# in5omnia/Image_Segmentation

Hardware: AMD Instinct MI355X
Metric: images/sec (fwd+bwd) U-Net 3-class 256x256; IoU parity vs CPU ref (higher is better)
Workload: dtype bf16; 1 GPU; unet(3,3) train step (fwd + ce + bwd + grad all-reduce + AdamW), B=32/GPU 3x256x256, BASELINE config 2; global_batch=32, parallelism=dp1, rccl_ranks=0, rehearsal=False

## Files before the change

image_segmentation_amd/_lib.py:

```python
import ctypes as C
import os

_HERE = os.path.dirname(os.path.abspath(__file__))
LIB_PATH = os.path.join(_HERE, "csrc", "libsegk.so")

F32, BF16 = 0, 1
ABI_VERSION = 318
MAX_CLASSES = 8
MAX_VIEWS = 16
MSE_PART_FLOATS = 1024

_vp, _fp, _i, _l, _f, _d = C.c_void_p, C.c_void_p, C.c_int, C.c_long, C.c_float, C.c_double

SIGNATURES = {
    "segk_version": (_i, []),
    "segk_entry_count": (_i, []),
    "segk_clock_probe": (_i, [_vp, _i, _i, _i, _vp]),
    "segk_debug_poison_tickets": (_i, [C.c_uint64, _vp]),
    "segk_build_id": (C.c_char_p, []),
    "segk_last_error": (C.c_char_p, []),
    "segk_nchw_to_nhwc": (_i, [_fp, _vp, _i, _i, _i, _i, _i, _i, _vp]),
    "segk_nhwc_to_nchw": (_i, [_vp, _fp, _i, _i, _i, _i, _i, _i, _vp]),
    "segk_pack_conv_weight": (_i, [_fp, _vp, _i, _i, _i, _i, _i, _i, _i, _i, _i, _vp]),
    "segk_pack_conv3x3_both": (_i, [_fp, _vp, _vp, _i, _i, _i, _i, _i, _i, _i, _vp]),
    "segk_pack_multi": (_i, [_vp, _i, _i, _i, _vp]),
    "segk_pack_convt_chunk": (_i, []),
    "segk_pack_convt_weight": (_i, [_fp, _vp, _i, _i, _i, _i, _i, _i, _vp]),
    "segk_conv_tiles": (_i, [_i, _i, _i, _i, _i, _i]),
    "segk_bn_stats_floats": (_i, [_i, _i]),
    "segk_conv3x3": (_i, [_vp, _vp, _vp, _fp, _fp, _fp, _vp, _vp, _fp, _i, _i, _i, _i, _i, _i, _i, _i, _vp]),
    "segk_conv_writes_act_q": (_i, [_i, _i, _i]),
    "segk_conv3x3_act": (_i, [_vp, _vp, _fp, _fp, _vp, _vp, _fp, _i, _i, _i, _i, _i, _i, _vp]),
    "segk_stem3x3_rows": (_i, [_i, _i, _i, _i, _i, _i]),
    "segk_stem3x3": (_i, [_fp, _fp, _vp, _vp, _fp, _i, _i, _i, _i, _i, _i, _vp]),
    "segk_stem3x3_wgrad_slabs": (_i, [_i, _i, _i, _i, _i, _i]),
    "segk_stem3x3_wgrad": (_i, [_fp, _vp, _fp, _i, _i, _i, _i, _i, _i, _vp]),
    "segk_conv1x1": (_i, [_vp, _vp, _fp, _vp, _i, _i, _i, _i, _i, _i, _vp]),
    "segk_convt2x2_fwd": (_i, [_vp, _vp, _fp, _vp, _i, _i, _i, _i, _i, _i, _vp]),
    "segk_convt2x2_dgrad": (_i, [_vp, _vp, _vp, _i, _i, _i, _i, _i, _i, _vp]),
    "segk_wgrad_tiles": (_i, [_i, _i, _i, _i, _i]),
    "segk_wgrad_split": (_i, [_i, _i, _i, _i, _i, _i]),
    "segk_wgrad": (_i, [_vp, _vp, _vp, _fp, _fp, _fp, _vp, _i, _i, _i, _i, _i, _i, _i, _i, _i, _vp]),
    "segk_wgrad_reduce": (_i, [_fp, _i, _fp, _i, _i, _i, _i, _i, _i, _i, _vp]),
    "segk_wgrad_reduce_multi": (_i, [_vp, _i, _vp]),
    "segk_bn_finalize": (_i, [_fp, _i, _i, _i, _d, _fp, _fp, _fp, _fp, _fp, _f, _f, _i, _fp, _fp, _fp, _fp, _vp]),
    "segk_bn_relu_apply": (_i, [_vp, _vp, _fp, _fp, _l, _i, _i, _vp]),
    "segk_bn_relu_apply_pool": (_i, [_vp, _vp, _vp, _fp, _fp, _i, _i, _i, _i, _i, _vp]),
    "segk_bn_bwd_blocks": (_i, [_l, _i, _i]),
    "segk_bn_relu_bwd": (_i, [_vp, _vp, _vp, _fp, _fp, _fp, _fp, _l, _i, _i, _fp, _fp, _fp, _fp, _i, _vp]),
    "segk_channel_sum": (_i, [_vp, _l, _i, _i, _fp, _fp, _i, _vp]),
    "segk_maxpool2x2_fwd": (_i, [_vp, _vp, _i, _i, _i, _i, _i, _vp]),
    "segk_maxpool2x2_bwd": (_i, [_vp, _vp, _vp, _i, _i, _i, _i, _i, _i, _vp]),
    "segk_maxpool_bwd_stat_blocks": (_i, [_i, _i, _i, _i, _i]),
    "segk_maxpool2x2_bwd_bnstat": (_i, [_vp, _vp, _vp, _i, _i, _i, _i, _i, _fp, _fp, _fp, _fp, _fp, _vp, _i, _vp]),
    "segk_bn_relu_bwd_from_part": (_i, [_vp, _vp, _vp, _fp, _fp, _fp, _fp, _l, _i, _i, _fp, _i, _fp, _fp, _fp, _i, _vp]),
    "segk_bilinear_fwd": (_i, [_vp, _vp, _i, _i, _i, _i, _i, _i, _i, _vp]),
    "segk_bilinear_bwd": (_i, [_vp, _vp, _fp, _i, _i, _i, _i, _i, _i, _i, _vp]),
    "segk_linear": (_i, [_vp, _vp, _fp, _vp, _l, _i, _i, _i, _i, _vp]),
    "segk_vit_patchify": (_i, [_fp, _vp, _i, _i, _i, _i, _i, _i, _i, _vp]),
    "segk_vit_embed_ln": (_i, [_vp, _fp, _fp, _fp, _fp, _f, _fp, _i, _i, _i, _i, _i, _vp]),
    "segk_add_layernorm": (_i, [_fp, _vp, _fp, _fp, _f, _vp, _l, _i, _i, _i, _vp]),
    "segk_linear_splitk": (_i, [_vp, _vp, _fp, _vp, _l, _i, _i, _i, _i, _vp]),
    "segk_add_layernorm_parts": (_i, [_fp, _vp, _i, _l, _fp, _fp, _f, _vp, _l, _i, _i, _i, _vp]),
    "segk_attention": (_i, [_vp, _vp, _i, _i, _i, _i, _i, _i, _f, _i, _vp]),
    "segk_vit_tokens_to_grid": (_i, [_fp, _vp, _i, _i, _i, _i, _i, _vp]),
    "segk_resize_pad": (_i, [_vp, _vp, _i, _i, _i, _i, _i, _i, _i, _i, _i, _i, _vp]),
    "segk_crop_resize": (_i, [_fp, _fp, _i, _i, _i, _i, _i, _i, _i, _i, _i, _vp]),
    "segk_resize_pad_u8": (_i, [_vp, _fp, _i, _i, _i, _i, _i, _i, _i, _i, _i, _vp]),
    "segk_predict_mask": (_i, [_vp, _vp, _vp, _vp, _vp, _vp, _vp, _i, _i, _i, _i, _i, _i, _i, _i, _i, _vp]),
    "segk_resize_pad_flip": (_i, [_vp, _vp, _i, _i, _i, _i, _i, _i, _i, _i, _i, _i, _i, _vp]),
    "segk_resize_pad_u8_flip": (_i, [_vp, _fp, _i, _i, _i, _i, _i, _i, _i, _i, _i, _i, _vp]),
    "segk_predict_merge": (_i, [_vp, _i, _i, _i, _i, _i, _i, _vp, _vp, _vp, _vp, _vp, _vp, _vp, _fp, _vp]),
    "segk_tile_gather_u8": (_i, [_vp, _fp, _i, _i, _i, _i, _i, _i, _i, _i, _vp]),
    "segk_tile_gather": (_i, [_fp, _fp, _i, _i, _i, _i, _i, _i, _i, _i, _vp]),
    "segk_predict_tiles": (_i, [_fp, _i, _i, _i, _i, _i, _i, _i, _i, _vp, _vp, _vp, _vp, _vp, _vp, _vp, _fp, _vp]),
    "segk_cc_label": (_i, [_vp, _vp, _vp, _vp, _vp, _vp, _vp, _vp, _i, _i, _i, _i, _i, _vp]),
    "segk_cc_clean": (_i, [_vp, _vp, _vp, _vp, _vp, _i, _i, _i, _i, _i, _vp]),
    "segk_mask_finish": (_i, [_vp, _vp, _vp, _vp, _vp, _vp, _i, _i, _i, _vp]),
    "segk_head_fwd": (_i, [_vp, _fp, _fp, _fp, _i, _i, _i, _i, _i, _i, _i, _vp]),
    "segk_head_fwd_bn": (_i, [_vp, _fp, _fp, _fp, _fp, _fp, _i, _i, _i, _i, _i, _i, _i, _vp]),
    "segk_head_bwd_bn": (_i, [_fp, _vp, _fp, _vp, _fp, _fp, _fp, _i, _i, _i, _i, _i, _i, _fp, _fp, _fp, _fp, _fp, _i, _vp]),
    "segk_head_part_floats": (_i, [_l, _i]),
    "segk_head_bwd": (_i, [_fp, _vp, _fp, _vp, _fp, _fp, _fp, _i, _i, _i, _i, _i, _i, _i, _vp]),
    "segk_head_bwd_blocks": (_i, [_l]),
    "segk_head_bwd_bnstat": (_i, [_fp, _vp, _fp, _vp, _fp, _fp, _fp, _i, _i, _i, _i, _i, _i, _fp, _fp, _fp, _fp, _fp, _i, _vp]),
    "segk_loss_part_floats": (_i, [_l]),
    "segk_loss_state_floats": (_i, []),
    "segk_loss_fwd": (_i, [_fp, _vp, _fp, _i, _i, _l, _i, _f, _f, _f, _fp, _fp, _fp, _vp]),
    "segk_loss_bwd": (_i, [_fp, _vp, _fp, _fp, _fp, _i, _i, _l, _i, _f, _f, _fp, _vp]),
    "segk_prompt_mix_fwd": (_i, [_fp, _fp, _fp, _i, _l, _vp]),
    "segk_prompt_mix_bwd": (_i, [_fp, _fp, _fp, _fp, _i, _l, _vp]),
    "segk_prob_loss_fwd": (_i, [_fp, _vp, _fp, _i, _i, _l, _i, _f, _f, _f, _i, _f, _fp, _fp, _fp, _vp]),
    "segk_prob_loss_bwd": (_i, [_fp, _vp, _fp, _fp, _fp, _i, _i, _l, _i, _f, _f, _i, _f, _fp, _vp]),
    "segk_confusion": (_i, [_fp, _vp, _i, _i, _l, _vp, _vp]),
    "segk_recon_head_fwd": (_i, [_vp, _fp, _fp, _fp, _i, _i, _i, _i, _i, _i, _i, _vp]),
    "segk_recon_sigmoid_bwd": (_i, [_fp, _fp, _vp, _i, _i, _i, _i, _i, _i, _vp]),
    "segk_mse_fwd": (_i, [_fp, _fp, _fp, _i, _fp, _l, _i, _vp]),
    "segk_mse_bwd": (_i, [_fp, _fp, _fp, _fp, _fp, _l, _i, _vp]),
    "segk_prompt_scores": (_i, [_vp, _vp, _vp, _vp, _i, _i, _vp, _vp, _i, _i, _i, _i, _vp]),
    "segk_prompt_make": (_i, [_vp, _vp, _vp, _vp, _vp, _i, _fp, _vp, _vp, _vp, _vp, _i, _i, _i, _i, _i, _vp]),
    "segk_prompt_heatmap": (_i, [_vp, _i, _vp, _i, _fp, _i, _i, _vp]),
    "segk_aug_prefilter": (_i, [_vp, _i, _i, _vp]),
    "segk_aug_resample": (_i, [_vp, _i, _i, _vp, _vp, _i, _vp, _i, _vp, _i, _vp, _fp, _vp, _vp, _vp]),
    "segk_aug_merge": (_i, [_vp, _vp, _i, _i, _vp, _fp, _vp, _vp, _vp]),
    "segk_label_hist": (_i, [_vp, _l, _i, _i, _i, _l, _vp, _vp]),
    "segk_rgb_label_to_classes": (_i, [_vp, _vp, _l, _vp]),
    "segk_perturb_point": (_i, [_vp, _i, _i, _i, _vp, _vp]),
    "segk_perturb_blur": (_i, [_vp, _i, _i, _i, _vp]),
}



class ReduceJob(C.Structure):
    _fields_ = [("src", C.c_void_p), ("dst", C.c_void_p), ("kind", C.c_int), ("S", C.c_int), ("N", C.c_int), ("CA", C.c_int),
                ("CB", C.c_int), ("Np", C.c_int), ("CAp", C.c_int), ("CBp", C.c_int), ("taps", C.c_int), ("pad_", C.c_int)]


_lib = None


def load():
    global _lib, LIB_PATH
    if _lib is None:
        if os.environ.get("SEGK_LIB"):
            LIB_PATH = os.path.abspath(os.environ["SEGK_LIB"])
        if not os.path.exists(LIB_PATH):
            raise RuntimeError(
                f"{LIB_PATH} not found: the HIP extension is required (no CPU/eager fallback exists). "
                "Build it with `python -m image_segmentation_amd.build`.")
        lib = C.CDLL(LIB_PATH)
        for name, (res, args) in SIGNATURES.items():
            try:
                fn = getattr(lib, name)
            except AttributeError:
                raise RuntimeError(f"{LIB_PATH} does not export {name}: it was built from another include/segk.h than "
                                   "this binding (rebuild with `python -m image_segmentation_amd.build`)") from None
            fn.restype = res
            fn.argtypes = args
        ver, nent = lib.segk_version(), lib.segk_entry_count()
        if ver != ABI_VERSION or nent != len(SIGNATURES):
            raise RuntimeError(f"{LIB_PATH}: ABI version {ver} with {nent} entries, this binding expects version "
                               f"{ABI_VERSION} with {len(SIGNATURES)} entries -- refusing to drive a library built from "
                               "another include/segk.h")
        _lib = lib
    return _lib


def call(name, *args):
    lib = load()
    rc = getattr(lib, name)(*args)
    if rc != 0:
        raise RuntimeError(f"{name} failed ({rc}): {lib.segk_last_error().decode()}")


def build_id():
    return load().segk_build_id().decode()


def query(name, *args):
    return getattr(load(), name)(*args)
```

image_segmentation_amd/build.py:

```python
import os
import subprocess
import sys
from concurrent.futures import ThreadPoolExecutor

CSRC = os.path.join(os.path.dirname(os.path.abspath(__file__)), "csrc")
SOURCES = ["api.hip", "conv_igemm.hip", "conv_rs.hip", "convt_stream.hip", "stem.hip", "wgrad.hip", "bn_pool.hip", "pack.hip", "head_loss.hip", "recon.hip", "prompt.hip", "augment.hip", "perturb.hip", "components.hip", "resize.hip", "tiles.hip", "vit.hip", "gemm.hip", "probe.hip"]
LIB = os.path.join(CSRC, "libsegk.so")
FLAGS = ["--offload-arch=gfx950", "-O3", "-fPIC", "-std=c++17", "-ffp-contract=off", "-Wall", "-Wno-unused-function"]


def _hipcc():
    for c in (os.environ.get("HIPCC"), "/opt/rocm/bin/hipcc", "hipcc"):
        if c and (os.path.isabs(c) and os.path.exists(c) or not os.path.isabs(c)):
            return c
    raise RuntimeError("hipcc not found")


def source_hash() -> str:
    import hashlib
    h = hashlib.sha256()
    files = sorted(f for f in os.listdir(CSRC) if f.endswith((".hip", ".hpp", ".h")))
    paths = [os.path.join(CSRC, f) for f in files] + \
            [os.path.join(os.path.dirname(os.path.dirname(CSRC)), "include", "segk.h")]
    for path in paths:
        h.update(os.path.basename(path).encode() + b"\0")
        h.update(open(path, "rb").read())
    return h.hexdigest()[:16]


def _stale(obj, src):
    if not os.path.exists(obj):
        return True
    t = os.path.getmtime(obj)
    deps = [src] + [os.path.join(CSRC, h) for h in ("common.hpp", "segk_internal.h")] + \
           [os.path.join(os.path.dirname(os.path.dirname(CSRC)), "include", "segk.h")]
    return any(os.path.getmtime(d) > t for d in deps)


def build(force: bool = False, verbose: bool = True) -> str:
    hipcc = _hipcc()
    objs, jobs = [], []
    bid = source_hash()
    stamp = os.path.join(CSRC, ".build_id")
    id_changed = not os.path.exists(stamp) or open(stamp).read().strip() != bid
    for s in SOURCES:
        src = os.path.join(CSRC, s)
        obj = os.path.join(CSRC, s.replace(".hip", ".o"))
        objs.append(obj)
        extra = [f'-DSEGK_BUILD_ID="{bid}"'] if s == "api.hip" else []
        if force or _stale(obj, src) or (extra and id_changed):
            jobs.append([hipcc, *FLAGS, *extra, "-c", src, "-o", obj])

    def run(cmd):
        if verbose:
            print(" ".join(cmd), flush=True)
        r = subprocess.run(cmd, capture_output=True, text=True)
        if r.returncode != 0:
            raise RuntimeError(f"hipcc failed: {' '.join(cmd)}\n{r.stdout}\n{r.stderr}")
        if verbose and r.stderr.strip():
            print(r.stderr, file=sys.stderr)

    with ThreadPoolExecutor(max_workers=6) as ex:
        list(ex.map(run, jobs))
    if jobs or not os.path.exists(LIB):
        run([hipcc, "--offload-arch=gfx950", "-shared", "-fPIC", "-o", LIB, *objs])
    with open(stamp, "w") as f:
        f.write(bid + "\n")
    return LIB


def build_sanitized(verbose: bool = False) -> str:
    hipcc = _hipcc()
    out = os.path.join(CSRC, ".asan")
    os.makedirs(out, exist_ok=True)
    lib = os.path.join(out, "libsegk_asan.so")
    stamp = os.path.join(out, ".build_id")
    bid = source_hash()
    if os.path.exists(lib) and os.path.exists(stamp) and open(stamp).read().strip() == bid:
        return lib
    flags = ["--offload-arch=gfx950", "-O1", "-g", "-fPIC", "-std=c++17", "-ffp-contract=off", "-fno-omit-frame-pointer",
             "-fsanitize=address,undefined", "-fno-sanitize-recover=undefined", "-fno-gpu-sanitize"]
    objs, jobs = [], []
    for s in SOURCES:
        obj = os.path.join(out, s.replace(".hip", ".o"))
        objs.append(obj)
        extra = [f'-DSEGK_BUILD_ID="{bid}"'] if s == "api.hip" else []
        jobs.append([hipcc, *flags, *extra, "-c", os.path.join(CSRC, s), "-o", obj])

    def run(cmd):
        if verbose:
            print(" ".join(cmd), flush=True)
        r = subprocess.run(cmd, capture_output=True, text=True)
        if r.returncode != 0:
            raise RuntimeError(f"hipcc failed: {' '.join(cmd)}\n{r.stdout}\n{r.stderr}")
    with ThreadPoolExecutor(max_workers=6) as ex:
        list(ex.map(run, jobs))
    run([hipcc, "--offload-arch=gfx950", "-shared", "-fPIC", "-fsanitize=address,undefined", "-shared-libsan", "-o", lib, *objs])
    with open(stamp, "w") as f:
        f.write(bid + "\n")
    return lib


def asan_runtime() -> str:
    import glob
    hits = sorted(glob.glob("/opt/rocm/lib/llvm/lib/clang/*/lib/linux/libclang_rt.asan-x86_64.so"))
    if not hits:
        raise RuntimeError("libclang_rt.asan-x86_64.so not found under /opt/rocm/lib/llvm")
    return hits[-1]


if __name__ == "__main__":
    print(build(force="--force" in sys.argv))
```

image_segmentation_amd/csrc/bn_pool.hip:

```cpp
#include <atomic>
#include "common.hpp"
#include "segk_internal.h"
#include "ticket.hpp"
#include "../../include/segk.h"

namespace {
__device__ unsigned g_tickets[TICKET_SLOTS * TICKET_GROUPS];

struct Lanes {
  int cx, ry, cv;
  bool active;
};
__device__ __forceinline__ Lanes lanes(int cvb, int cvec) {
  Lanes l;
  l.cx = threadIdx.x % cvb;
  l.ry = threadIdx.x / cvb;
  l.cv = blockIdx.y * cvb + l.cx;
  l.active = l.cv < cvec;
  return l;
}

constexpr int NCH = 32;
__device__ __forceinline__ void stats_chunk(const float* __restrict__ part, int MT, int C, double* __restrict__ out,
                                            double (&sh)[8][32][2]) {
// ... 459 lines not shown
        o[j] = accumulate ? o[j] + r : r;
        if (STAT) {
          const float gg = v[k][j] > 0.f ? o[j] : 0.f;
          sg[j] += gg;
          sgx[j] = fmaf(gg, fmaf(v[k][j], xa[j], xb[j]), sgx[j]);
        }
      }
      *(uint4*)(dx + off[k]) = pack16<T>(o);
    }
  }
  if (STAT) {
    __shared__ float red[256][2 * E::VEC + 1];
    if (from_z) {
#pragma unroll
      for (int j = 0; j < E::VEC; ++j) sgx[j] = 0.f;
      for (unsigned i = blockIdx.x * 256u + threadIdx.x; i < (unsigned)total; i += gridDim.x * 256u) {
        const Idx4 ix = split4(i, (unsigned)CV, (unsigned)Wc, (unsigned)Hc);
        const int cv = ix.cv, xo = ix.x, yo = ix.y, b = ix.b;
        for (int k = 0; k < 4; ++k) {
          const int yy = 2 * yo + (k >> 1), xx = 2 * xo + (k & 1);
          if (yy >= H || xx >= W) continue;
          const size_t off = (((size_t)(b * H + yy)) * W + xx) * C + cv * E::VEC;
          float fy[E::VEC], fd[E::VEC], fz[E::VEC];
          unpack16<T>(*(const uint4*)(x + off), fy);
          unpack16<T>(*(const uint4*)(dx + off), fd);
          unpack16<T>(*(const uint4*)(z + off), fz);
#pragma unroll
          for (int j = 0; j < E::VEC; ++j) {
            const int c = cv * E::VEC + j;
            const float gg = fy[j] > 0.f ? fd[j] : 0.f;
            sgx[j] = fmaf(gg, (fz[j] - mean[c]) * rstd[c], sgx[j]);
          }
        }
      }
    }
#pragma unroll
    for (int j = 0; j < E::VEC; ++j) { red[threadIdx.x][j] = sg[j]; red[threadIdx.x][E::VEC + j] = sgx[j]; }
    __syncthreads();
    for (int q = threadIdx.x; q < CV * E::VEC; q += 256) {
      const int cv = q / E::VEC, j = q - cv * E::VEC;
      float a = 0.f, bsum = 0.f;
      for (int t = cv; t < 256; t += CV) {
        a += red[t][j];
        bsum += red[t][E::VEC + j];
      }
      ((float2*)part)[(size_t)blockIdx.x * C + q] = make_float2(a, bsum);
    }
  }
}

template <typename T>
__global__ __launch_bounds__(256) void channel_sum_kernel(const T* __restrict__ x, long P, int C, int cvb, int rows,
                                                          float* part) {
  using E = ET<T>;
  extern __shared__ __attribute__((aligned(16))) char smem[];
  float* red = (float*)smem;
  const Lanes l = lanes(cvb, C / E::VEC);
  float s[E::VEC];
#pragma unroll
  for (int j = 0; j < E::VEC; ++j) s[j] = 0.f;
  if (l.active && l.ry < rows) {
    auto one = [&](const uint4 raw) {
      float f[E::VEC];
      unpack16<T>(raw, f);
#pragma unroll
      for (int j = 0; j < E::VEC; ++j) s[j] += f[j];
    };
    const long step = (long)gridDim.x * rows;
    const size_t cofs = (size_t)l.cv * E::VEC;
    long p = (long)blockIdx.x * rows + l.ry;
    for (; p + 3 * step < P; p += 4 * step) {
      uint4 r[4];
#pragma unroll
      for (int u = 0; u < 4; ++u) r[u] = *(const uint4*)(x + (size_t)(p + u * step) * C + cofs);
      __builtin_amdgcn_sched_barrier(0);
#pragma unroll
      for (int u = 0; u < 4; ++u) one(r[u]);
    }
    for (; p < P; p += step) one(*(const uint4*)(x + (size_t)p * C + cofs));
  }
  if (l.ry < rows) {
    float* r = red + ((size_t)l.ry * cvb + l.cx) * E::VEC;
#pragma unroll
    for (int j = 0; j < E::VEC; ++j) r[j] = s[j];
  }
  __syncthreads();
  if (l.ry == 0 && l.active)
#pragma unroll
    for (int j = 0; j < E::VEC; ++j) {
      float a = 0.f;
      for (int r = 0; r < rows; ++r) a += red[((size_t)r * cvb + l.cx) * E::VEC + j];
      part[(size_t)blockIdx.x * C + l.cv * E::VEC + j] = a;
    }
}
__global__ __launch_bounds__(1024) void channel_sum_finalize_kernel(const float* __restrict__ part, int NB, int C,
                                                                    int C_real, float* out) {
  __shared__ double sh[32][32];
  const int cx = threadIdx.x & 31, ry = threadIdx.x >> 5;
  const int c = blockIdx.x * 32 + cx;
  double s = 0.0;
  if (c < C) {
    for (int m = ry; m < NB; m += 512) {
      float v[16];
#pragma unroll
      for (int u = 0; u < 16; ++u) {
        const int r = m + 32 * u < NB ? m + 32 * u : NB - 1;
        v[u] = part[(unsigned)r * (unsigned)C + (unsigned)c];
      }
#pragma unroll
      for (int u = 0; u < 16; ++u) s += (m + 32 * u < NB) ? (double)v[u] : 0.0;
    }
  }
  sh[ry][cx] = s;
  __syncthreads();
  if (ry != 0 || c >= C_real) return;
  s = 0.0;
#pragma unroll 8
  for (int r = 0; r < 32; ++r) s += sh[r][cx];
  out[c] = (float)s;
}

static inline void lane_geometry(int C, int vec, int* cvb, int* rows, int* gy) {
  const int cvec = C / vec;
  *cvb = cvec < 128 ? cvec : 128;
  *rows = 256 / *cvb;
  *gy = cdiv(cvec, *cvb);
}

}

unsigned* segk_ticket_slot(int groups, hipStream_t st) {
  static std::atomic<unsigned> n{0};
  static unsigned* base[SEGK_MAX_DEVICES] = {};
  const int dev = segk_device_index();
  if (groups < 1 || groups > TICKET_GROUPS) return nullptr;
  if (!base[dev] && hipGetSymbolAddress((void**)&base[dev], HIP_SYMBOL(g_tickets)) != hipSuccess) return nullptr;
  unsigned* const p = base[dev] + (size_t)(n.fetch_add(1, std::memory_order_relaxed) % TICKET_SLOTS) * TICKET_GROUPS;
  if (hipMemsetAsync(p, 0, (size_t)groups * sizeof(unsigned), st) != hipSuccess) return nullptr;
  return p;
}

extern "C" int segk_debug_poison_tickets(uint64_t pattern, segk_stream_t s) {
  hipStream_t st = (hipStream_t)s;
  unsigned* base = nullptr;
  SEGK_REQUIRE(hipGetSymbolAddress((void**)&base, HIP_SYMBOL(g_tickets)) == hipSuccess, "poison_tickets: no ticket array");
  static unsigned host[TICKET_SLOTS * TICKET_GROUPS];
  for (int i = 0; i < TICKET_SLOTS * TICKET_GROUPS; ++i) host[i] = (unsigned)pattern;
  SEGK_REQUIRE(hipMemcpyAsync(base, host, sizeof(host), hipMemcpyHostToDevice, st) == hipSuccess, "poison_tickets: copy failed");
  SEGK_REQUIRE(hipStreamSynchronize(st) == hipSuccess, "poison_tickets: sync failed");
  return 0;
}

extern "C" int segk_bn_finalize(const float* part, int MT, int C, int C_real, double count, const float* conv_bias,
                                const float* gamma, const float* beta, float* rmean, float* rvar, float momentum, float eps,
                                int training, float* scale, float* shift, float* mean, float* rstd, segk_stream_t s) {
  hipStream_t st = (hipStream_t)s;
  SEGK_REQUIRE(C > 0 && C % 32 == 0 && C_real > 0 && C_real <= C, "bn_finalize: bad channels C=%d real=%d", C, C_real);
  SEGK_REQUIRE(gamma && beta && scale && shift, "bn_finalize: null pointer");
  if (training) SEGK_REQUIRE(part && MT > 0 && count > 0 && mean && rstd, "bn_finalize: training needs partials");
  else SEGK_REQUIRE(rmean && rvar, "bn_finalize: eval needs running statistics");
  double* scratch = part ? (double*)(const_cast<float*>(part) + (size_t)MT * C * 2) : nullptr;
  if (training && MT <= 1024) {
    hipLaunchKernelGGL(bn_stats_finalize_small_kernel, dim3(C / 32), dim3(1024), 0, st, part, MT, C, C_real, count, conv_bias,
                       gamma, beta, rmean, rvar, momentum, eps, scale, shift, mean, rstd);
    SEGK_CHECK_LAUNCH("bn_stats_finalize_small");
    return 0;
  }
  if (training) {
    SEGK_REQUIRE(C / 32 <= TICKET_GROUPS, "bn_finalize: at most %d channels", 32 * TICKET_GROUPS);
    unsigned* const tickets = segk_ticket_slot(C / 32, st);
    SEGK_REQUIRE(tickets != nullptr, "bn_finalize: no ticket array");
    hipLaunchKernelGGL(bn_stats_finalize_kernel, dim3(C / 32, NCH), dim3(256), 0, st, part, MT, C, C_real, count, conv_bias,
                       gamma, beta, rmean, rvar, momentum, eps, scale, shift, mean, rstd, scratch, tickets);
    SEGK_CHECK_LAUNCH("bn_stats_finalize");
    return 0;
  }
  hipLaunchKernelGGL(bn_finalize_kernel, dim3(C / 32), dim3(256), 0, st, scratch, NCH, C, C_real, count, conv_bias,
                     gamma, beta, rmean, rvar, momentum, eps, training, scale, shift, mean, rstd);
  SEGK_CHECK_LAUNCH("bn_finalize");
  return 0;
}
int segk_bn_stats_floats(int tiles, int Cp) {
  if (tiles <= 0 || Cp <= 0) return 0;
  const long long n = (long long)tiles * Cp * 2 + (long long)NCH * Cp * 4;
  return n > 0x7fffffffLL ? 0 : (int)n;
}

template <typename T>
static int bn_relu_apply_t(const void* z, void* y, const float* scale, const float* shift, long P, int C, hipStream_t st) {
  int cvb, rows, gy;
  lane_geometry(C, ET<T>::VEC, &cvb, &rows, &gy);
  long gx = (P + rows - 1) / rows;
  if (gx > 4096) gx = 4096;
  hipLaunchKernelGGL(bn_relu_apply_kernel<T>, dim3((int)gx, gy), dim3(256), 0, st, (const T*)z, (T*)y, scale, shift, P,
                     C, cvb, rows);
  SEGK_CHECK_LAUNCH("bn_relu_apply");
  return 0;
}
extern "C" int segk_bn_relu_apply(const void* z, void* y, const float* scale, const float* shift, long P, int C, int dtype,
                                  segk_stream_t s) {
  SEGK_REQUIRE_DTYPE("bn_relu_apply", dtype);
  hipStream_t st = (hipStream_t)s;
  SEGK_REQUIRE(z && y && scale && shift && P > 0 && C > 0 && C % 32 == 0, "bn_relu_apply: bad arguments");
  return dtype == SEGK_DT_BF16 ? bn_relu_apply_t<bf16_t>(z, y, scale, shift, P, C, st)
                               : bn_relu_apply_t<float>(z, y, scale, shift, P, C, st);
}

extern "C" int segk_bn_relu_apply_pool(const void* z, void* y, void* pooled, const float* scale, const float* shift, int B,
                                       int H, int W, int C, int dtype, segk_stream_t s) {
  SEGK_REQUIRE_DTYPE("bn_relu_apply_pool", dtype);
  hipStream_t st = (hipStream_t)s;
  SEGK_REQUIRE(z && y && pooled && scale && shift && B > 0 && H >= 2 && W >= 2 && C > 0 && C % 32 == 0,
               "bn_relu_apply_pool: bad arguments");
  const int vec = dtype == SEGK_DT_BF16 ? 8 : 4;
  long total = (long)B * ((H + 1) / 2) * ((W + 1) / 2) * (C / vec);
  SEGK_REQUIRE(total < (1L << 31), "bn_relu_apply_pool: more than 2^31 windows x channel vectors");
  long g = (total + 255) / 256;
  if (g > 8192) g = 8192;
  if (dtype == SEGK_DT_BF16)
    hipLaunchKernelGGL(bn_relu_apply_pool_kernel<bf16_t>, dim3((int)g), dim3(256), 0, st, (const bf16_t*)z, (bf16_t*)y,
                       (bf16_t*)pooled, scale, shift, B, H, W, C);
  else
    hipLaunchKernelGGL(bn_relu_apply_pool_kernel<float>, dim3((int)g), dim3(256), 0, st, (const float*)z, (float*)y,
                       (float*)pooled, scale, shift, B, H, W, C);
  SEGK_CHECK_LAUNCH("bn_relu_apply_pool");
  return 0;
}

int segk_bn_bwd_blocks(long P, int C, int dtype) {
  if (P <= 0 || C <= 0 || C % 32 != 0) return 0;
  const int vec = dtype == SEGK_DT_BF16 ? 8 : 4;
  int cvb, rows, gy;
  lane_geometry(C, vec, &cvb, &rows, &gy);
  long gx = (P + rows - 1) / rows;
  if (gx > 512) gx = 512;
  return (int)gx;
}

template <typename T>
static int bn_bwd_t(const void* dy, const void* z, void* dz, const float* scale, const float* shift, const float* mean,
                    const float* rstd, long P, int C, int C_real, float* part, float* dgamma, float* dbeta,
                    float* coef, hipStream_t st) {
  using E = ET<T>;
  int cvb, rows, gy;
  lane_geometry(C, E::VEC, &cvb, &rows, &gy);
  const int gx = segk_bn_bwd_blocks(P, C, sizeof(T) == 2 ? SEGK_DT_BF16 : SEGK_DT_F32);
  const size_t lds = (size_t)rows * cvb * 2 * E::VEC * sizeof(float);
  hipLaunchKernelGGL(bn_bwd_reduce_kernel<T>, dim3(gx, gy), dim3(256), lds, st, (const T*)dy, (const T*)z, scale, shift,
                     mean, rstd, P, C, cvb, rows, part);
  SEGK_CHECK_LAUNCH("bn_bwd_reduce");
  hipLaunchKernelGGL(bn_bwd_finalize_kernel, dim3(C / 32), dim3(1024), 0, st, part, gx, C, C_real, (double)P, dgamma,
                     dbeta, coef);
  SEGK_CHECK_LAUNCH("bn_bwd_finalize");
  long ga = (P + rows - 1) / rows;
  if (ga > 4096) ga = 4096;
  hipLaunchKernelGGL(bn_bwd_apply_kernel<T>, dim3((int)ga, gy), dim3(256), 0, st, (const T*)dy, (const T*)z, (T*)dz,
                     scale, shift, mean, rstd, coef, P, C, cvb, rows);
  SEGK_CHECK_LAUNCH("bn_bwd_apply");
  return 0;
}
template <typename T>
static int bn_bwd_from_part_t(const void* dy, const void* z, void* dz, const float* scale, const float* shift, const float* mean,
                              const float* rstd, long P, int C, int C_real, const float* part, int nb, float* dgamma,
                              float* dbeta, float* coef, hipStream_t st) {
  using E = ET<T>;
  int cvb, rows, gy;
  lane_geometry(C, E::VEC, &cvb, &rows, &gy);
  hipLaunchKernelGGL(bn_bwd_finalize_kernel, dim3(C / 32), dim3(1024), 0, st, part, nb, C, C_real, (double)P, dgamma,
                     dbeta, coef);
  SEGK_CHECK_LAUNCH("bn_bwd_finalize");
  long ga = (P + rows - 1) / rows;
  if (ga > 4096) ga = 4096;
  hipLaunchKernelGGL(bn_bwd_apply_kernel<T>, dim3((int)ga, gy), dim3(256), 0, st, (const T*)dy, (const T*)z, (T*)dz,
                     scale, shift, mean, rstd, coef, P, C, cvb, rows);
  SEGK_CHECK_LAUNCH("bn_bwd_apply");
  return 0;
}
extern "C" int segk_bn_relu_bwd_from_part(const void* dy, const void* z, void* dz, const float* scale, const float* shift,
                                          const float* mean, const float* rstd, long P, int C, int C_real, const float* part,
                                          int nb, float* dgamma, float* dbeta, float* coef, int dtype, segk_stream_t s) {
  SEGK_REQUIRE_DTYPE("bn_relu_bwd_from_part", dtype);
  hipStream_t st = (hipStream_t)s;
  SEGK_REQUIRE(dy && z && dz && scale && shift && mean && rstd && part && dgamma && dbeta && coef && nb > 0,
               "bn_bwd_from_part: bad arguments");
  SEGK_REQUIRE(P > 0 && C > 0 && C % 32 == 0 && C_real > 0 && C_real <= C, "bn_bwd_from_part: bad shape");
  return dtype == SEGK_DT_BF16
             ? bn_bwd_from_part_t<bf16_t>(dy, z, dz, scale, shift, mean, rstd, P, C, C_real, part, nb, dgamma, dbeta, coef, st)
             : bn_bwd_from_part_t<float>(dy, z, dz, scale, shift, mean, rstd, P, C, C_real, part, nb, dgamma, dbeta, coef, st);
}

extern "C" int segk_bn_relu_bwd(const void* dy, const void* z, void* dz, const float* scale, const float* shift,
                                const float* mean, const float* rstd, long P, int C, int C_real, float* part, float* dgamma,
                                float* dbeta, float* coef, int dtype, segk_stream_t s) {
  SEGK_REQUIRE_DTYPE("bn_relu_bwd", dtype);
  hipStream_t st = (hipStream_t)s;
  SEGK_REQUIRE(dy && z && dz && scale && shift && mean && rstd && part && dgamma && dbeta && coef,
               "bn_bwd: null pointer");
  SEGK_REQUIRE(P > 0 && C > 0 && C % 32 == 0 && C_real > 0 && C_real <= C, "bn_bwd: bad shape");
  return dtype == SEGK_DT_BF16
             ? bn_bwd_t<bf16_t>(dy, z, dz, scale, shift, mean, rstd, P, C, C_real, part, dgamma, dbeta, coef, st)
             : bn_bwd_t<float>(dy, z, dz, scale, shift, mean, rstd, P, C, C_real, part, dgamma, dbeta, coef, st);
}

extern "C" int segk_maxpool2x2_fwd(const void* x, void* y, int B, int H, int W, int C, int dtype, segk_stream_t s) {
  SEGK_REQUIRE_DTYPE("maxpool2x2_fwd", dtype);
  hipStream_t st = (hipStream_t)s;
  SEGK_REQUIRE(x && y && B > 0 && H >= 2 && W >= 2 && C > 0 && C % 32 == 0, "maxpool_fwd: bad arguments");
  const int vec = dtype == SEGK_DT_BF16 ? 8 : 4;
  long total = (long)B * (H / 2) * (W / 2) * (C / vec);
  SEGK_REQUIRE(total < (1L << 31), "maxpool_fwd: more than 2^31 windows x channel vectors");
  long g = (total + 255) / 256;
  if (g > 8192) g = 8192;
  if (dtype == SEGK_DT_BF16)
    hipLaunchKernelGGL(maxpool_fwd_kernel<bf16_t>, dim3((int)g), dim3(256), 0, st, (const bf16_t*)x, (bf16_t*)y, B, H, W, C);
  else
    hipLaunchKernelGGL(maxpool_fwd_kernel<float>, dim3((int)g), dim3(256), 0, st, (const float*)x, (float*)y, B, H, W, C);
  SEGK_CHECK_LAUNCH("maxpool_fwd");
  return 0;
}

extern "C" int segk_maxpool2x2_bwd(const void* x, const void* dy, void* dx, int B, int H, int W, int C, int accumulate,
                                   int dtype, segk_stream_t s) {
  SEGK_REQUIRE_DTYPE("maxpool2x2_bwd", dtype);
  hipStream_t st = (hipStream_t)s;
  SEGK_REQUIRE(x && dy && dx && B > 0 && H >= 2 && W >= 2 && C > 0 && C % 32 == 0, "maxpool_bwd: bad arguments");
  const int vec = dtype == SEGK_DT_BF16 ? 8 : 4;
  long total = (long)B * ((H + 1) / 2) * ((W + 1) / 2) * (C / vec);
  SEGK_REQUIRE(total < (1L << 31), "maxpool_bwd: more than 2^31 windows x channel vectors");
  long g = (total + 255) / 256;
  if (g > 8192) g = 8192;
  if (dtype == SEGK_DT_BF16)
    hipLaunchKernelGGL((maxpool_bwd_kernel<bf16_t, false>), dim3((int)g), dim3(256), 0, st, (const bf16_t*)x, (const bf16_t*)dy,
                       (bf16_t*)dx, B, H, W, C, accumulate, nullptr, nullptr, nullptr, nullptr, nullptr, nullptr);
  else
    hipLaunchKernelGGL((maxpool_bwd_kernel<float, false>), dim3((int)g), dim3(256), 0, st, (const float*)x, (const float*)dy,
                       (float*)dx, B, H, W, C, accumulate, nullptr, nullptr, nullptr, nullptr, nullptr, nullptr);
  SEGK_CHECK_LAUNCH("maxpool_bwd");
  return 0;
}

int segk_maxpool_bwd_stat_blocks(int B, int H, int W, int C, int dtype) {
  const int vec = dtype == SEGK_DT_BF16 ? 8 : 4;
  if (B <= 0 || H < 2 || W < 2 || C <= 0 || C % 32 != 0) return 0;
  const int cv = C / vec;
  if ((cv & (cv - 1)) != 0 || cv > 256) return 0;
  long total = (long)B * ((H + 1) / 2) * ((W + 1) / 2) * cv;
  if (total >= (1L << 31)) return 0;
  long g = (total + 255) / 256;
  return (int)(g > 1024 ? 1024 : g);
}

extern "C" int segk_maxpool2x2_bwd_bnstat(const void* x, const void* dy, void* dx, int B, int H, int W, int C, int accumulate,
                                          const float* scale, const float* shift, const float* mean, const float* rstd,
                                          float* part, const void* z, int dtype, segk_stream_t s) {
  SEGK_REQUIRE_DTYPE("maxpool2x2_bwd_bnstat", dtype);
  hipStream_t st = (hipStream_t)s;
  SEGK_REQUIRE(x && dy && dx && scale && shift && mean && rstd && part, "maxpool_bwd_bnstat: null pointer");
  const int g = segk_maxpool_bwd_stat_blocks(B, H, W, C, dtype);
  SEGK_REQUIRE(g > 0, "maxpool_bwd_bnstat: shape not served (channel vectors must be a power of two)");
  if (dtype == SEGK_DT_BF16)
    hipLaunchKernelGGL((maxpool_bwd_kernel<bf16_t, true>), dim3(g), dim3(256), 0, st, (const bf16_t*)x, (const bf16_t*)dy,
                       (bf16_t*)dx, B, H, W, C, accumulate, scale, shift, mean, rstd, part, (const bf16_t*)z);
  else
    hipLaunchKernelGGL((maxpool_bwd_kernel<float, true>), dim3(g), dim3(256), 0, st, (const float*)x, (const float*)dy,
                       (float*)dx, B, H, W, C, accumulate, scale, shift, mean, rstd, part, (const float*)z);
  SEGK_CHECK_LAUNCH("maxpool_bwd_bnstat");
  return 0;
}

extern "C" int segk_channel_sum(const void* x, long P, int C, int C_real, float* part, float* out, int dtype, segk_stream_t s) {
  SEGK_REQUIRE_DTYPE("channel_sum", dtype);
  hipStream_t st = (hipStream_t)s;
  SEGK_REQUIRE(x && part && out && P > 0 && C > 0 && C % 32 == 0 && C_real > 0 && C_real <= C, "channel_sum: bad arguments");
  const int vec = dtype == SEGK_DT_BF16 ? 8 : 4;
  int cvb, rows, gy;
  lane_geometry(C, vec, &cvb, &rows, &gy);
  const int gx = segk_bn_bwd_blocks(P, C, dtype);
  const size_t lds = (size_t)rows * cvb * vec * sizeof(float);
  if (dtype == SEGK_DT_BF16)
    hipLaunchKernelGGL(channel_sum_kernel<bf16_t>, dim3(gx, gy), dim3(256), lds, st, (const bf16_t*)x, P, C, cvb, rows, part);
  else
    hipLaunchKernelGGL(channel_sum_kernel<float>, dim3(gx, gy), dim3(256), lds, st, (const float*)x, P, C, cvb, rows, part);
  SEGK_CHECK_LAUNCH("channel_sum");
  hipLaunchKernelGGL(channel_sum_finalize_kernel, dim3(C / 32), dim3(1024), 0, st, part, gx, C, C_real, out);
  SEGK_CHECK_LAUNCH("channel_sum_finalize");
  return 0;
}
```

image_segmentation_amd/csrc/head_loss.hip:

```cpp
#include <type_traits>
#include "common.hpp"
#include "segk_internal.h"
#include "ticket.hpp"
#include "../../include/segk.h"

namespace {
constexpr int MAXC = 8;
constexpr int HT = 256;
constexpr int HCH = 64;

__device__ __forceinline__ void split_hw(long p, long HW, long& b, long& r) {
  const unsigned bb = (unsigned)p / (unsigned)HW;
  b = (long)bb;
  r = p - (long)bb * HW;
}

template <typename T, int NC>
__global__ __launch_bounds__(256) void head_fwd_kernel(const T* __restrict__ y, const float* __restrict__ w,
                                                       const float* __restrict__ bias, float* __restrict__ logits,
                                                       long P, long HW, int Cp, int C, int ncls,
                                                       const float* __restrict__ zsc, const float* __restrict__ zsh) {
  using E = ET<T>;
  constexpr int PITCH = HCH * E::ES + 16;
  extern __shared__ __attribute__((aligned(16))) char tile[];
// ... 303 lines not shown
      v[u] = part[(unsigned)r * LP + cx];
    }
#pragma unroll
    for (int u = 0; u < FL; ++u) acc += (ry + RG * u < NB) ? (double)v[u] : 0.0;
  }
  sh[ry][cx] = acc;
  __syncthreads();
  if (t < LP) {
    double s = 0.0;
    for (int r = 0; r < RG; ++r) s += sh[r][t];
    tot[t] = s;
  }
  __syncthreads();
  if (t != 0) return;
  const double ce = tot[1] > 0.0 ? tot[0] / tot[1] : NAN;
  double wsum = 0.0, dsum = 0.0;
  int nvalid = 0;
  for (int k = 0; k < C; ++k) {
    const double den_raw = tot[2 + MAXC + k] + tot[2 + 2 * MAXC + k] + (double)smooth;
    const double den = den_raw < 1e-8 ? 1e-8 : den_raw;
    const double dc = (2.0 * tot[2 + k] + (double)smooth) / den;
    state[4 + k] = (float)dc;
    state[4 + MAXC + k] = (float)den_raw;
    const bool valid = !(ignore_index >= 0 && ignore_index < C && k == ignore_index);
    if (valid) {
      const double wk = cw ? (double)cw[k] : 1.0;
      wsum += wk; dsum += dc * wk; ++nvalid;
    }
  }
  if (cw && wsum < 1e-8) wsum = 1e-8;
  const double dice = -(dsum / wsum);
  for (int k = 0; k < C; ++k) {
    const bool valid = !(ignore_index >= 0 && ignore_index < C && k == ignore_index);
    state[4 + 2 * MAXC + k] = valid ? (float)((cw ? (double)cw[k] : 1.0) / wsum) : 0.f;
  }
  state[0] = (float)((double)dice_weight * dice + (ce_weight != 0.f ? (double)ce_weight * ce : 0.0));
  if (loss_out) *loss_out = state[0];
  state[1] = (float)ce;
  state[2] = (float)dice;
  state[3] = (float)tot[1];
  (void)nvalid;
}

template <bool PROB, int NC>
__global__ __launch_bounds__(LT) void loss_fwd_kernel(const float* __restrict__ logits,
                                                       const long long* __restrict__ labels,
                                                       const float* __restrict__ cw, long P, long HW, int C,
                                                       int ignore_index, float* __restrict__ part, int nll_log, float eps,
                                                       float smooth, float dice_weight, float ce_weight,
                                                       float* __restrict__ state, float* __restrict__ loss_out,
                                                       unsigned* __restrict__ ticket) {
  __shared__ float sh[LT / 64][LP];
  __shared__ int last;
  float a0 = 0.f, a1 = 0.f, aI[NC], aP[NC], aG[NC];
#pragma unroll
  for (int k = 0; k < NC; ++k) { aI[k] = 0.f; aP[k] = 0.f; aG[k] = 0.f; }
  auto fetch = [&](long p, float (&raw)[NC], long long& y) {
    long b, r; split_hw(p, HW, b, r);
#pragma unroll
    for (int k = 0; k < NC; ++k) {
      const float v = logits[(b * C + (k < C ? k : C - 1)) * HW + r];
      raw[k] = (k < C) ? v : -INFINITY;
    }
    y = labels[p];
  };
  auto pixel = [&](const float (&raw)[NC], const long long y) {
    float l[NC], m = -INFINITY;
#pragma unroll
    for (int k = 0; k < NC; ++k) m = fmaxf(m, raw[k]);
    float se = 0.f;
#pragma unroll
    for (int k = 0; k < NC; ++k) {
      if constexpr (PROB) l[k] = (k < C) ? raw[k] : 0.f;
      else l[k] = (k < C) ? expf(raw[k] - m) : 0.f;
      se += l[k];
    }
    const float inv = PROB ? 1.f : 1.f / se, lse = PROB ? 0.f : logf(se);
#pragma unroll
    for (int k = 0; k < NC; ++k) {
      const float pk = l[k] * inv;
      const float oh = (y == k) ? 1.f : 0.f;
      aI[k] += pk * oh;
      aP[k] += pk;
      aG[k] += oh;
      if (y == k && k < C && y != ignore_index) {
        const float wy = cw ? cw[k] : 1.f;
        if constexpr (PROB) a0 += wy * (nll_log ? -logf(raw[k] + eps) : -raw[k]);
        else a0 += wy * (lse - (raw[k] - m));
        a1 += wy;
      }
    }
  };
  const long step = (long)gridDim.x * LT;
  long p = (long)blockIdx.x * LT + threadIdx.x;
  for (; p + 3 * step < P; p += 4 * step) {
    float r0[NC], r1[NC], r2[NC], r3[NC];
    long long y0, y1, y2, y3;
    fetch(p, r0, y0);
    fetch(p + step, r1, y1);
    fetch(p + 2 * step, r2, y2);
    fetch(p + 3 * step, r3, y3);
    pixel(r0, y0);
    pixel(r1, y1);
    pixel(r2, y2);
    pixel(r3, y3);
  }
  for (; p < P; p += step) {
    float r0[NC];
    long long y0;
    fetch(p, r0, y0);
    pixel(r0, y0);
  }
  float v[LP];
#pragma unroll
  for (int i = 0; i < LP; ++i) v[i] = 0.f;
  v[0] = a0; v[1] = a1;
#pragma unroll
  for (int k = 0; k < NC; ++k) { v[2 + k] = aI[k]; v[2 + MAXC + k] = aP[k]; v[2 + 2 * MAXC + k] = aG[k]; }
#pragma unroll
  for (int i = 0; i < LP; ++i) {
    if (i >= 2 && ((i - 2) % MAXC) >= NC) continue;
#pragma unroll
    for (int o = 32; o > 0; o >>= 1) v[i] += __shfl_xor(v[i], o);
  }
  if ((threadIdx.x & 63) == 0) {
#pragma unroll
    for (int i = 0; i < LP; ++i) sh[threadIdx.x >> 6][i] = v[i];
  }
  __syncthreads();
  if (threadIdx.x < LP) {
    const int i = threadIdx.x;
    float s2 = 0.f;
#pragma unroll
    for (int w = 0; w < LT / 64; ++w) s2 += sh[w][i];
    part[(size_t)blockIdx.x * LP + i] = s2;
  }
  if (last_arriver(ticket, gridDim.x, &last))
    loss_finalize_block(part, (int)gridDim.x, C, cw, ignore_index, smooth, dice_weight, ce_weight, state, loss_out);
}


template <bool PROB, int NC>
__global__ __launch_bounds__(256) void loss_bwd_kernel(const float* __restrict__ logits,
                                                       const long long* __restrict__ labels,
                                                       const float* __restrict__ cw, const float* __restrict__ state,
                                                       const float* __restrict__ gout, long P, long HW, int C,
                                                       int ignore_index, float dice_weight, float ce_weight,
                                                       float* __restrict__ dlogits, int nll_log, float eps) {
  const float go = gout[0];
  const float ce_den = state[3];
  float G0[NC], G1[NC];
#pragma unroll
  for (int k = 0; k < NC; ++k) {
    G0[k] = 0.f; G1[k] = 0.f;
    if (k < C) {
      const float dc = state[4 + k], den_raw = state[4 + MAXC + k], ak = state[4 + 2 * MAXC + k];
      if (den_raw < 1e-8f) { G1[k] = -ak * 2.f / 1e-8f; }
      else { G0[k] = ak * dc / den_raw; G1[k] = -ak * 2.f / den_raw; }
    }
  }
  for (long p = (long)blockIdx.x * 256 + threadIdx.x; p < P; p += (long)gridDim.x * 256) {
    long b, r; split_hw(p, HW, b, r);
    float l[NC], m = -INFINITY;
#pragma unroll
    for (int k = 0; k < NC; ++k) {
      const float v = logits[(b * C + (k < C ? k : C - 1)) * HW + r];
      l[k] = (k < C) ? v : -INFINITY;
      m = fmaxf(m, l[k]);
    }
    const long long y = labels[p];
    const bool ce_valid = (ce_weight != 0.f && y >= 0 && y < C && y != ignore_index);
    float wy = 0.f;
    if (ce_valid) wy = (cw ? cw[y] : 1.f) / ce_den;
    if constexpr (PROB) {
#pragma unroll
      for (int k = 0; k < NC; ++k)
        if (k < C) {
          const bool hit = (y == k);
          const float dd = G0[k] + (hit ? G1[k] : 0.f);
          const float dn = hit ? (nll_log ? -wy / (l[k] + eps) : -wy) : 0.f;
          dlogits[(b * C + k) * HW + r] = go * (dice_weight * dd + ce_weight * dn);
        }
      continue;
    }
    float se = 0.f;
#pragma unroll
    for (int k = 0; k < NC; ++k) { l[k] = (k < C) ? expf(l[k] - m) : 0.f; se += l[k]; }
    const float inv = 1.f / se;
    float dot = 0.f;
#pragma unroll
    for (int k = 0; k < NC; ++k) {
      l[k] *= inv;
      dot += l[k] * (G0[k] + ((y == k) ? G1[k] : 0.f));
    }
#pragma unroll
    for (int k = 0; k < NC; ++k)
      if (k < C) {
        const float gk = G0[k] + ((y == k) ? G1[k] : 0.f);
        const float dd = l[k] * (gk - dot);
        const float dce = wy * (l[k] - ((y == k) ? 1.f : 0.f));
        dlogits[(b * C + k) * HW + r] = go * (dice_weight * dd + ce_weight * dce);
      }
  }
}

__global__ __launch_bounds__(256) void confusion_kernel(const float* __restrict__ logits,
                                                        const long long* __restrict__ labels, long P, long HW, int C,
                                                        unsigned long long* __restrict__ M) {
  __shared__ unsigned int hist[MAXC * MAXC];
  if (threadIdx.x < MAXC * MAXC) hist[threadIdx.x] = 0;
  __syncthreads();
  for (long p = (long)blockIdx.x * 256 + threadIdx.x; p < P; p += (long)gridDim.x * 256) {
    long b, r; split_hw(p, HW, b, r);
    int best = 0;
    float bv = logits[(b * C) * HW + r];
    for (int k = 1; k < C; ++k) {
      const float v = logits[(b * C + k) * HW + r];
      if (v > bv || (v != v && bv == bv)) { bv = v; best = k; }
    }
    const long long y = labels[p];
    if (y >= 0 && y < C) atomicAdd(&hist[best * MAXC + (int)y], 1u);
  }
  __syncthreads();
  if (threadIdx.x < MAXC * MAXC && hist[threadIdx.x])
    atomicAdd(&M[threadIdx.x], (unsigned long long)hist[threadIdx.x]);
}

}

template <typename T> static size_t head_lds() { return (size_t)HT * (HCH * ET<T>::ES + 16); }

#ifndef SEGK_HEAD_BLOCKS_CAP
#define SEGK_HEAD_BLOCKS_CAP 1024
#endif
int segk_head_blocks(long P) {
  if (P <= 0) return 0;
  long g = (P + 31) / 32;
  return (int)(g > SEGK_HEAD_BLOCKS_CAP ? SEGK_HEAD_BLOCKS_CAP : g);
}
int segk_head_part_floats(long P, int Cp) {
  if (P <= 0 || Cp <= 0) return 0;
  const long long n = (long long)segk_head_blocks(P) * MAXC * ((long long)Cp + 1);
  return n > 0x7fffffffLL ? 0 : (int)n;
}

static int head_fwd(const void* y, const float* w, const float* bias, float* logits, int B, int H, int W, int Cp, int C, int ncls,
                    const float* zsc, const float* zsh, int dtype, hipStream_t st) {
  SEGK_REQUIRE(y && w && bias && logits && B > 0 && H > 0 && W > 0, "head_fwd: bad arguments");
  SEGK_REQUIRE((zsc == nullptr) == (zsh == nullptr), "head_fwd: scale and shift come together");
  SEGK_REQUIRE_DTYPE("head_fwd", dtype);
  SEGK_REQUIRE(ncls >= 1 && ncls <= MAXC, "head_fwd: 1..%d classes supported, got %d", MAXC, ncls);
  SEGK_REQUIRE(Cp % 32 == 0 && C > 0 && C <= Cp, "head_fwd: bad channels");
  const long P = (long)B * H * W, HW = (long)H * W;
  SEGK_REQUIRE(P < (1L << 31), "head / loss kernels index pixels with 32 bits: %ld pixels", P);
  long g = (P + HT - 1) / HT;
  if (g > 4096) g = 4096;
  auto launch = [&](auto Tc, auto NCc) {
    using T = decltype(Tc);
    constexpr int NC = decltype(NCc)::value;
    return segk_launch_lds<head_fwd_kernel<T, NC>>("head_fwd", 96 * 1024, dim3((int)g), dim3(256), head_lds<T>(), st, (const T*)y, w,
                                                   bias, logits, P, HW, Cp, C, ncls, zsc, zsh);
  };
  auto by_nc = [&](auto Tc) {
    if (ncls <= 2) return launch(Tc, std::integral_constant<int, 2>{});
    if (ncls == 3) return launch(Tc, std::integral_constant<int, 3>{});
    if (ncls == 4) return launch(Tc, std::integral_constant<int, 4>{});
    return launch(Tc, std::integral_constant<int, MAXC>{});
  };
  return dtype == SEGK_DT_BF16 ? by_nc(bf16_t{}) : by_nc(float{});
}
extern "C" int segk_head_fwd(const void* y, const float* w, const float* bias, float* logits, int B, int H, int W, int Cp, int C,
                             int ncls, int dtype, segk_stream_t s) {
  SEGK_REQUIRE_DTYPE("head_fwd", dtype);
  return head_fwd(y, w, bias, logits, B, H, W, Cp, C, ncls, nullptr, nullptr, dtype, (hipStream_t)s);
}
extern "C" int segk_head_fwd_bn(const void* z, const float* scale, const float* shift, const float* w, const float* bias,
                                float* logits, int B, int H, int W, int Cp, int C, int ncls, int dtype, segk_stream_t s) {
  SEGK_REQUIRE(scale && shift, "head_fwd_bn: null scale/shift");
  return head_fwd(z, w, bias, logits, B, H, W, Cp, C, ncls, scale, shift, dtype, (hipStream_t)s);
}

template <typename T>
static int head_bwd_t(const float* dlog, const void* y, const float* w, void* dy, float* part, float* dw, float* db,
                      long P, long HW, int Cp, int C, int ncls, const float* const* bn, float* bnpart, bool zin,
                      hipStream_t st) {
  constexpr int HV = HeadVec<T>::HV;
  const int cvec = Cp / HV;
  const int cvb = cvec < 64 ? cvec : 64;
  const int rows = 256 / cvb, gy = cdiv(cvec, cvb);
  const int nb = segk_head_blocks(P);
  const size_t lds = (size_t)rows * cvb * (MAXC * HV + MAXC) * sizeof(float);
  auto launch_z = [&](auto NCc, auto ZINc) {
    constexpr int NC = decltype(NCc)::value;
    return segk_launch_lds<head_bwd_kernel<T, NC, decltype(ZINc)::value>>(
        "head_bwd", 96 * 1024, dim3(nb, gy), dim3(256), lds, st, dlog, (const T*)y, w, (T*)dy, part, P, HW, Cp, C, ncls, cvb, rows,
        bn ? bn[0] : nullptr, bn ? bn[1] : nullptr, bn ? bn[2] : nullptr, bn ? bn[3] : nullptr, bnpart);
  };
  auto launch = [&](auto NCc) { return zin ? launch_z(NCc, std::true_type{}) : launch_z(NCc, std::false_type{}); };
  const int rc = ncls <= 2 ? launch(std::integral_constant<int, 2>{})
               : ncls == 3 ? launch(std::integral_constant<int, 3>{})
               : ncls == 4 ? launch(std::integral_constant<int, 4>{})
                           : launch(std::integral_constant<int, MAXC>{});
  if (rc) return rc;
  hipLaunchKernelGGL(head_bwd_finalize_kernel, dim3(cdiv(ncls * (C + 1), 4)), dim3(256), 0, st, part, nb, Cp, C, ncls, dw, db);
  SEGK_CHECK_LAUNCH("head_bwd_finalize");
  return 0;
}

static int head_bwd(const float* dlog, const void* y, const float* w, void* dy, float* part, float* dw, float* db, int B, int H,
                    int W, int Cp, int C, int ncls, const float* bn_scale, const float* bn_shift, const float* bn_mean,
                    const float* bn_rstd, float* bnpart, int zin, int dtype, hipStream_t st) {
  SEGK_REQUIRE(dlog && y && w && dy && part && dw && db && B > 0 && H > 0 && W > 0, "head_bwd: bad arguments");
  SEGK_REQUIRE(ncls >= 1 && ncls <= MAXC && Cp % 32 == 0 && C > 0 && C <= Cp, "head_bwd: bad channels/classes");
  SEGK_REQUIRE_DTYPE("head_bwd", dtype);
  SEGK_REQUIRE(!(bnpart || zin) || (bn_scale && bn_shift && bn_mean && bn_rstd),
               "head_bwd: BatchNorm reductions / a pre-activation input need scale, shift, mean and rstd");
  const long P = (long)B * H * W, HW = (long)H * W;
  SEGK_REQUIRE(P < (1L << 31), "head / loss kernels index pixels with 32 bits: %ld pixels", P);
  const float* bn[4] = {bn_scale, bn_shift, bn_mean, bn_rstd};
  const float* const* bnp = (bnpart || zin) ? bn : nullptr;
  return dtype == SEGK_DT_BF16 ? head_bwd_t<bf16_t>(dlog, y, w, dy, part, dw, db, P, HW, Cp, C, ncls, bnp, bnpart, zin != 0, st)
                               : head_bwd_t<float>(dlog, y, w, dy, part, dw, db, P, HW, Cp, C, ncls, bnp, bnpart, zin != 0, st);
}
extern "C" int segk_head_bwd(const float* dlogits, const void* y, const float* w, void* dy, float* part, float* dw, float* db,
                             int B, int H, int W, int Cp, int C, int ncls, int dtype, segk_stream_t s) {
  SEGK_REQUIRE_DTYPE("head_bwd", dtype);
  return head_bwd(dlogits, y, w, dy, part, dw, db, B, H, W, Cp, C, ncls, nullptr, nullptr, nullptr, nullptr, nullptr, 0, dtype,
                  (hipStream_t)s);
}
extern "C" int segk_head_bwd_blocks(long P) { return segk_head_blocks(P); }
extern "C" int segk_head_bwd_bnstat(const float* dlogits, const void* y, const float* w, void* dy, float* part, float* dw,
                                    float* db, int B, int H, int W, int Cp, int C, int ncls, const float* scale,
                                    const float* shift, const float* mean, const float* rstd, float* bnpart, int dtype,
                                    segk_stream_t s) {
  SEGK_REQUIRE_DTYPE("head_bwd_bnstat", dtype);
  SEGK_REQUIRE(bnpart, "head_bwd_bnstat: null partials");
  return head_bwd(dlogits, y, w, dy, part, dw, db, B, H, W, Cp, C, ncls, scale, shift, mean, rstd, bnpart, 0, dtype,
                  (hipStream_t)s);
}
extern "C" int segk_head_bwd_bn(const float* dlogits, const void* z, const float* w, void* dy, float* part, float* dw, float* db,
                                int B, int H, int W, int Cp, int C, int ncls, const float* scale, const float* shift,
                                const float* mean, const float* rstd, float* bnpart, int dtype, segk_stream_t s) {
  SEGK_REQUIRE(scale && shift && mean && rstd, "head_bwd_bn: null BatchNorm vectors");
  return head_bwd(dlogits, z, w, dy, part, dw, db, B, H, W, Cp, C, ncls, scale, shift, mean, rstd, bnpart, 1, dtype,
                  (hipStream_t)s);
}

__global__ __launch_bounds__(256) void prompt_mix_fwd_kernel(const float* __restrict__ clip, const float* __restrict__ mask,
                                                             float* __restrict__ out, long P, long HW) {
  for (long p = (long)blockIdx.x * 256 + threadIdx.x; p < P; p += (long)gridDim.x * 256) {
    long b, r; split_hw(p, HW, b, r);
    float l[4], mx = -INFINITY;
#pragma unroll
    for (int k = 0; k < 4; ++k) { l[k] = clip[(b * 4 + k) * HW + r]; mx = fmaxf(mx, l[k]); }
    float se = 0.f;
#pragma unroll
    for (int k = 0; k < 4; ++k) { l[k] = expf(l[k] - mx); se += l[k]; }
    const float inv = 1.f / se;
    const float m = 1.f / (1.f + expf(-mask[p]));
    float sel[4];
#pragma unroll
    for (int k = 0; k < 4; ++k) sel[k] = m * (l[k] * inv);
    out[(b * 4 + 0) * HW + r] = 1.0f - m;
    out[(b * 4 + 1) * HW + r] = sel[0] + sel[3];
    out[(b * 4 + 2) * HW + r] = sel[1];
    out[(b * 4 + 3) * HW + r] = sel[2];
  }
}
__global__ __launch_bounds__(256) void prompt_mix_bwd_kernel(const float* __restrict__ clip, const float* __restrict__ mask,
                                                             const float* __restrict__ dout, float* __restrict__ dmask,
                                                             long P, long HW) {
  for (long p = (long)blockIdx.x * 256 + threadIdx.x; p < P; p += (long)gridDim.x * 256) {
    long b, r; split_hw(p, HW, b, r);
    float l[4], mx = -INFINITY;
#pragma unroll
    for (int k = 0; k < 4; ++k) { l[k] = clip[(b * 4 + k) * HW + r]; mx = fmaxf(mx, l[k]); }
    float se = 0.f;
#pragma unroll
    for (int k = 0; k < 4; ++k) { l[k] = expf(l[k] - mx); se += l[k]; }
    const float inv = 1.f / se;
    const float m = 1.f / (1.f + expf(-mask[p]));
    const float d0 = dout[(b * 4 + 0) * HW + r], d1 = dout[(b * 4 + 1) * HW + r];
    const float d2 = dout[(b * 4 + 2) * HW + r], d3 = dout[(b * 4 + 3) * HW + r];
    const float dm = -d0 + d1 * ((l[0] + l[3]) * inv) + d2 * (l[1] * inv) + d3 * (l[2] * inv);
    dmask[p] = dm * m * (1.f - m);
  }
}

static int prompt_mix(const float* clip, const float* mask, const float* dout, float* out, int N, long HW, hipStream_t st) {
  SEGK_REQUIRE(clip && mask && out && N > 0 && HW > 0, "prompt_mix: bad arguments");
  const long P = (long)N * HW;
  SEGK_REQUIRE(P < (1L << 31), "head / loss kernels index pixels with 32 bits: %ld pixels", P);
  long g = (P + 255) / 256;
  if (g > 4096) g = 4096;
  if (dout) hipLaunchKernelGGL(prompt_mix_bwd_kernel, dim3((int)g), dim3(256), 0, st, clip, mask, dout, out, P, HW);
  else hipLaunchKernelGGL(prompt_mix_fwd_kernel, dim3((int)g), dim3(256), 0, st, clip, mask, out, P, HW);
  SEGK_CHECK_LAUNCH("prompt_mix");
  return 0;
}
extern "C" int segk_prompt_mix_fwd(const float* clip_logits, const float* mask_logit, float* final_probs, int N, long HW,
                                   segk_stream_t s) {
  return prompt_mix(clip_logits, mask_logit, nullptr, final_probs, N, HW, (hipStream_t)s);
}
extern "C" int segk_prompt_mix_bwd(const float* clip_logits, const float* mask_logit, const float* dfinal, float* dmask_logit,
                                   int N, long HW, segk_stream_t s) {
  SEGK_REQUIRE(dfinal, "prompt_mix_bwd: null gradient");
  return prompt_mix(clip_logits, mask_logit, dfinal, dmask_logit, N, HW, (hipStream_t)s);
}

int segk_loss_blocks(long P) {
  if (P <= 0) return 0;
  long g = (P + 4 * LT - 1) / (4 * LT);
  return (int)(g > LROWS ? LROWS : g < 1 ? 1 : g);
}
int segk_loss_part_floats(long P) { return segk_loss_blocks(P) * LP; }
int segk_loss_state_floats(void) { return LS; }

static int loss_fwd(const float* logits, const int64_t* labels64, const float* cw, int N, int C, long HW, int ignore_index,
                    float smooth, float dice_weight, float ce_weight, float* part, float* state, float* loss_out, int prob,
                    int nll_log, float eps, segk_stream_t s) {
  const long long* labels = (const long long*)labels64;
  hipStream_t st = (hipStream_t)s;
  SEGK_REQUIRE(logits && labels && part && state && N > 0 && HW > 0, "loss_fwd: bad arguments");
  SEGK_REQUIRE(C >= 1 && C <= MAXC, "loss_fwd: 1..%d classes supported, got %d", MAXC, C);
  const long P = (long)N * HW;
  SEGK_REQUIRE(P < (1L << 31), "head / loss kernels index pixels with 32 bits: %ld pixels", P);
  const int nb = segk_loss_blocks(P);
  unsigned* const ticket = segk_ticket_slot(1, st);
  SEGK_REQUIRE(ticket != nullptr, "loss_fwd: no ticket array");
  auto launch = [&](auto PROBc, auto NCc) {
    constexpr bool PR = decltype(PROBc)::value;
    constexpr int NC = decltype(NCc)::value;
    hipLaunchKernelGGL((loss_fwd_kernel<PR, NC>), dim3(nb), dim3(LT), 0, st, logits, labels, cw, P, HW, C, ignore_index, part,
                       PR ? nll_log : 0, PR ? eps : 0.f, smooth, dice_weight, ce_weight, state, loss_out, ticket);
  };
  auto by_nc = [&](auto PROBc) {
    if (C <= 2) launch(PROBc, std::integral_constant<int, 2>{});
    else if (C <= 4) launch(PROBc, std::integral_constant<int, 4>{});
    else launch(PROBc, std::integral_constant<int, MAXC>{});
  };
  if (prob) by_nc(std::true_type{});
  else by_nc(std::false_type{});
  SEGK_CHECK_LAUNCH("loss_fwd");
  return 0;
}
extern "C" int segk_loss_fwd(const float* logits, const int64_t* labels, const float* cw, int N, int C, long HW, int ignore_index,
                             float smooth, float dice_weight, float ce_weight, float* part, float* state, float* loss_out,
                             segk_stream_t s) {
  return loss_fwd(logits, labels, cw, N, C, HW, ignore_index, smooth, dice_weight, ce_weight, part, state, loss_out, 0, 0, 0.f, s);
}
extern "C" int segk_prob_loss_fwd(const float* probs, const int64_t* labels, const float* cw, int N, int C, long HW,
                                  int ignore_index, float smooth, float dice_weight, float nll_weight, int nll_log, float eps,
                                  float* part, float* state, float* loss_out, segk_stream_t s) {
  return loss_fwd(probs, labels, cw, N, C, HW, ignore_index, smooth, dice_weight, nll_weight, part, state, loss_out, 1, nll_log,
                  eps, s);
}

static int loss_bwd(const float* logits, const int64_t* labels64, const float* cw, const float* state, const float* gout, int N,
                    int C, long HW, int ignore_index, float dice_weight, float ce_weight, float* dlogits, int prob, int nll_log,
                    float eps, segk_stream_t s) {
  const long long* labels = (const long long*)labels64;
  hipStream_t st = (hipStream_t)s;
  SEGK_REQUIRE(logits && labels && state && gout && dlogits && N > 0 && HW > 0 && C >= 1 && C <= MAXC, "loss_bwd: bad arguments");
  const long P = (long)N * HW;
  SEGK_REQUIRE(P < (1L << 31), "head / loss kernels index pixels with 32 bits: %ld pixels", P);
  long g = (P + 255) / 256;
  if (g > 4096) g = 4096;
  auto launch = [&](auto PROBc, auto NCc) {
    constexpr bool PR = decltype(PROBc)::value;
    constexpr int NC = decltype(NCc)::value;
    hipLaunchKernelGGL((loss_bwd_kernel<PR, NC>), dim3((int)g), dim3(256), 0, st, logits, labels, cw, state, gout, P, HW, C,
                       ignore_index, dice_weight, ce_weight, dlogits, PR ? nll_log : 0, PR ? eps : 0.f);
  };
  auto by_nc = [&](auto PROBc) {
    if (C <= 2) launch(PROBc, std::integral_constant<int, 2>{});
    else if (C <= 4) launch(PROBc, std::integral_constant<int, 4>{});
    else launch(PROBc, std::integral_constant<int, MAXC>{});
  };
  if (prob) by_nc(std::true_type{});
  else by_nc(std::false_type{});
  SEGK_CHECK_LAUNCH("loss_bwd");
  return 0;
}
extern "C" int segk_loss_bwd(const float* logits, const int64_t* labels, const float* cw, const float* state, const float* gout,
                             int N, int C, long HW, int ignore_index, float dice_weight, float ce_weight, float* dlogits,
                             segk_stream_t s) {
  return loss_bwd(logits, labels, cw, state, gout, N, C, HW, ignore_index, dice_weight, ce_weight, dlogits, 0, 0, 0.f, s);
}
extern "C" int segk_prob_loss_bwd(const float* probs, const int64_t* labels, const float* cw, const float* state,
                                  const float* gout, int N, int C, long HW, int ignore_index, float dice_weight,
                                  float nll_weight, int nll_log, float eps, float* dprobs, segk_stream_t s) {
  return loss_bwd(probs, labels, cw, state, gout, N, C, HW, ignore_index, dice_weight, nll_weight, dprobs, 1, nll_log, eps, s);
}

extern "C" int segk_confusion(const float* logits, const int64_t* labels, int N, int C, long HW, uint64_t* M, segk_stream_t s) {
  hipStream_t st = (hipStream_t)s;
  SEGK_REQUIRE(logits && labels && M && N > 0 && HW > 0 && C >= 1 && C <= MAXC, "confusion: bad arguments");
  const long P = (long)N * HW;
  SEGK_REQUIRE(P < (1L << 31), "head / loss kernels index pixels with 32 bits: %ld pixels", P);
  long g = (P + 255) / 256;
  if (g > 1024) g = 1024;
  hipLaunchKernelGGL(confusion_kernel, dim3((int)g), dim3(256), 0, st, logits, (const long long*)labels, P, HW, C, (unsigned long long*)M);
  SEGK_CHECK_LAUNCH("confusion");
  return 0;
}
```

image_segmentation_amd/csrc/segk_internal.h:

```cpp
#pragma once
#include <hip/hip_runtime.h>
#include <stdint.h>
#include "common.hpp"

struct ConvArgs {
  const void* srcA;
  const void* srcB;
  const void* w;
  const float* bias;
  const float* scale;
  const float* shift;
  void* out;
  void* out2;
  float* stats;
  void* act_out;
  int B, H, W;
  int CA, CB;
  int Ntot, CO1, CO2;
  int twl, tiles_x, tiles_y;
  int unshuf, shuffle;
  int persistent;
  int act;
};
int segk_conv_igemm_launch(const ConvArgs& a, int geo, int dtype, hipStream_t st);

#define SEGK_MAX_DEVICES 64
int segk_device_index();
int segk_num_cus();

int segk_conv_use_rs(int cin_p, int n_p, int dtype, int W);
int segk_conv_rs_rows(int B, int H, int W, int n_p);
void segk_conv_rs_grid(int MT, int NT, int* gw_out, int* GW_out);
struct ConvPlan;
int segk_conv_rs_launch(const ConvArgs& a, const ConvPlan& p, hipStream_t st);
int segk_stem_rows(int B, int H, int W, int Cin, int Cout, int dtype);
int segk_stem_launch(const float* x, const float* w, void* z, void* xn, float* stats, int B, int H, int W, int Cin, int Cout,
                     hipStream_t st);
int segk_stem_wgrad_slabs(int B, int H, int W, int Cin, int Cout, int dtype);
int segk_stem_wgrad_launch(const float* x, const void* dz, float* slabs, int B, int H, int W, int Cin, int Cout,
                           hipStream_t st);
int segk_convt_stream_ok(int B, int H, int W, int Cin, int Cout, int dtype);
int segk_convt_stream_launch(const void* x, const void* wp, const float* bias4, void* out, int B, int H, int W, int Cin,
                             int Cout, hipStream_t st);
int segk_convt_stream_dgrad_ok(int B, int H, int W, int Cin, int Cout, int dtype);
int segk_convt_stream_dgrad_launch(const void* dout, const void* wd, void* din, int B, int H, int W, int Cin, int Cout,
                                   hipStream_t st);
int segk_conv_writes_act(int cin_p, int n_p, int dtype);

enum ConvForm {
  CONV_RS,
  CONV_WS,
  CONV_PIPE,
  CONV_GEMM_DMA,
  CONV_GENERIC,
};
struct ConvPlan {
  ConvForm form;
  bool wide;
  int bm, twl;
  int bn;
  int wm, wn, mf, nf, pbuf;
  int unit;
  bool rs_rows;
};
ConvPlan segk_conv_plan(int geo, int dtype, int cin_p, int n_p, int W, bool has_bias, bool gemm_dma);

template <auto Kern>
int segk_raise_lds(const char* name, int limit) {
  static bool attr_set[SEGK_MAX_DEVICES] = {};
  const int dev = segk_device_index();
  if (!attr_set[dev]) {
    if (hipFuncSetAttribute((const void*)Kern, hipFuncAttributeMaxDynamicSharedMemorySize, limit) != hipSuccess)
      SEGK_FAIL(-3, "%s: cannot raise dynamic LDS limit", name);
    attr_set[dev] = true;
  }
  return 0;
}
template <auto Kern, typename... Args>
int segk_launch_lds(const char* name, int limit, dim3 grid, dim3 block, size_t lds, hipStream_t st, Args... args) {
  if (const int rc = segk_raise_lds<Kern>(name, limit)) return rc;
  hipLaunchKernelGGL(Kern, grid, block, lds, st, args...);
  SEGK_CHECK_LAUNCH(name);
  return 0;
}

struct SegkPackEntry {
  const float* w;
  void* dst_fwd;
  void* dst_dgrad;
  int Cout, CA, CB, Coutp, CAp, CBp;
  int block0;
  int kind;
  int pad_[2];
};
static_assert(sizeof(SegkPackEntry) == 64, "SegkPackEntry is 64 bytes");

struct WgradArgs {
  const void* dz;
  const void* srcA;
  const void* srcB;
  const float* scale;
  const float* shift;
  float* slabs;
  const void* zeros;
  int B, H, W;
  int CD, CA, CB;
  int S;
};
int segk_wgrad_launch(const WgradArgs& a, int geo, int dtype, hipStream_t st);
int segk_wgrad_wc(int CD, int CA, int CB, int geo, int dtype);

struct GemmArgs {
  const void* A;
  const char* w;
  const float* bias;
  void* out;
  long M;
  int N;
  int nchunks;
  int nchA;
  int lda;
  int H, W;
  int Cout;
  int act;
  int ksplit;
  long split_stride;
};
int segk_gemm_dma_ok(long M, int nchunks, int nchA, int N, int cout_shuffle, int lda, int mode);
int segk_gemm_dma_launch(const GemmArgs& g, int mode, hipStream_t st);
```

image_segmentation_amd/ops.py:

```python
import os
import sys
import weakref

import torch

from . import _lib

_DT = {torch.float32: _lib.F32, torch.bfloat16: _lib.BF16}
_compute_dtype = torch.bfloat16


def set_compute_dtype(dtype):
    global _compute_dtype
    if dtype not in _DT:
        raise ValueError("compute dtype must be torch.float32 or torch.bfloat16")
    _compute_dtype = dtype


def get_compute_dtype():
    return _compute_dtype


def pad32(c):
    return (c + 31) // 32 * 32


_raw_stream = getattr(torch._C, "_cuda_getCurrentRawStream", None)
_raw_device = getattr(torch._C, "_cuda_getDevice", None)


def _stream():
    if _raw_stream is not None and _raw_device is not None:
        return _raw_stream(_raw_device())
    return torch.cuda.current_stream().cuda_stream


def _require_cuda(t, what):
    if not t.is_cuda:
        raise RuntimeError(f"{what}: expected a CUDA/HIP tensor -- image_segmentation_amd has no CPU path "
                           "(the CPU oracle lives in oracle/ and is test infrastructure only)")


def _p(t):
    return 0 if t is None else t.data_ptr()


def new_act(B, C, H, W, dtype, device):
    Cp = pad32(C)
    buf = torch.empty((B, H, W, Cp), dtype=dtype, device=device)
    if Cp != C:
        buf[..., C:].zero_()
    return buf.permute(0, 3, 1, 2)[:, :C]


def act_view(buf, C):
    return buf.permute(0, 3, 1, 2)[:, :C]


def act_info(t, dtype):
    if t.dim() != 4 or t.dtype != dtype or not t.is_cuda:
        return None
    B, C, H, W = t.shape
    sb, sc, sh, sw = t.stride()
    Cp = sw if W > 1 else (sh if H > 1 else pad32(C))
    if sc != 1 or Cp < C or Cp % 32 != 0 or Cp != pad32(C):
        return None
    if (W > 1 and sw != Cp) or (H > 1 and sh != W * Cp) or (B > 1 and sb != H * W * Cp):
        return None
    if (t.storage_offset() * t.element_size()) % 16 != 0:
        return None
    return t.data_ptr(), Cp


def to_act(x, dtype):
    _require_cuda(x, "to_act")
    if act_info(x, dtype) is not None:
        return x
    B, C, H, W = x.shape
    src = x.detach()
    if C % 32 == 0 and src.stride(1) == 1 and src.permute(0, 2, 3, 1).is_contiguous():
        return act_view(src.permute(0, 2, 3, 1).to(dtype), C)
    if src.dtype != torch.float32 or not src.is_contiguous():
        src = src.float().contiguous()
    out = torch.empty((B, H, W, pad32(C)), dtype=dtype, device=x.device)
    _lib.call("segk_nchw_to_nhwc", src.data_ptr(), out.data_ptr(), B, C, H, W, pad32(C), _DT[dtype], _stream())
    return act_view(out, C)


def act_to_nchw(t):
    info = act_info(t, t.dtype)
    if info is None:
        return t.float().contiguous()
    B, C, H, W = t.shape
    out = torch.empty((B, C, H, W), dtype=torch.float32, device=t.device)
    _lib.call("segk_nhwc_to_nchw", info[0], out.data_ptr(), B, C, H, W, info[1], _DT[t.dtype], _stream())
    return out


def _private_act_copy(t, dtype):
    ptr, Cp = act_info(t, dtype)
    B, C, H, W = t.shape
    n = B * H * W * Cp
    out = torch.empty((B, H, W, Cp), dtype=dtype, device=t.device)
    out.view(-1).copy_(torch.as_strided(t, (n,), (1,), t.storage_offset()))
    return out


def _raw(t, dtype):
    t = to_act(t, dtype)
    ptr, Cp = act_info(t, dtype)
    return t, ptr, Cp


INPLACE_SKIP_GRAD = True
FUSE_BN_REDUCE = True
HEAD_ON_Z = os.environ.get("SEGK_HEAD_ON_Z", "1") != "0"
_OPT_EPOCH = [0]


def _on_optimizer_step(optimizer, args, kwargs):
    _OPT_EPOCH[0] += 1


from torch.optim.optimizer import register_optimizer_step_post_hook as _register_step_hook

_register_step_hook(_on_optimizer_step)


def invalidate_packed_weights():
    _OPT_EPOCH[0] += 1


class PackCache:

    def __init__(self):
        self._c = {}
        self.multi = {}

    def get_pair(self, key_a, key_b, param, builder, meta=None):
        ver = (param._version, param.data_ptr(), param.device, _OPT_EPOCH[0] if param.requires_grad else -1)
        hit = self._c.get(key_a)
        if hit is None or hit[0] != ver:
            a, b = builder()
            hit = (ver, a)
            self._c[key_a] = hit
            self._c[key_b] = (ver, b)
            if meta is not None:
                self.multi[key_a] = (meta[0], key_b, param) + tuple(meta[1:])
        return hit[1]

    def get_registered(self, key, param, builder, meta):
        self.multi[key] = (meta[0], None, param) + tuple(meta[1:])
        return self.get(key, param, builder)

    def get(self, key, param, builder):
        ver = (param._version, param.data_ptr(), param.device, _OPT_EPOCH[0] if param.requires_grad else -1)
        hit = self._c.get(key)
        if hit is None or hit[0] != ver:
            hit = (ver, builder())
            self._c[key] = hit
        return hit[1]


def pack_conv(w, CA, CB, dtype, mode, taps=9):
    Cout = w.shape[0]
    Coutp, CAp, CBp = pad32(Cout), pad32(CA), (pad32(CB) if CB else 0)
    dst = torch.empty(((CAp + CBp) * taps * Coutp,), dtype=dtype, device=w.device)
    wf = w.detach()
    if wf.dtype != torch.float32 or not wf.is_contiguous():
        wf = wf.float().contiguous()
    _lib.call("segk_pack_conv_weight", wf.data_ptr(), dst.data_ptr(), Cout, CA, CB, Coutp, CAp, CBp, taps, mode,
              _DT[dtype], _stream())
    return dst


def pack_conv_both(w, CA, CB, dtype):
    Cout = w.shape[0]
    Coutp, CAp, CBp = pad32(Cout), pad32(CA), (pad32(CB) if CB else 0)
    n = (CAp + CBp) * 9 * Coutp
    both = torch.empty((2 * n,), dtype=dtype, device=w.device)
    wf = w.detach()
    if wf.dtype != torch.float32 or not wf.is_contiguous():
        wf = wf.float().contiguous()
    _lib.call("segk_pack_conv3x3_both", wf.data_ptr(), both.data_ptr(), both[n:].data_ptr(), Cout, CA, CB, Coutp, CAp, CBp,
              _DT[dtype], _stream())
    return both[:n], both[n:]


_PACK_CONVT_CHUNK = [0]


def _entry_geometry(kind, param, d0, d1):
    if kind == 0:
        Cout = param.shape[0]
        Coutp, CAp, CBp = pad32(Cout), pad32(d0), (pad32(d1) if d1 else 0)
        return (CAp + CBp) * 9 * Coutp, (Cout, d0, d1, Coutp, CAp, CBp), (CAp + CBp) // 32 * (Coutp // 32)
    if kind == 1:
        Cin, Cout = param.shape[0], param.shape[1]
        Cinp, Coutp = pad32(Cin), pad32(Cout)
        if not _PACK_CONVT_CHUNK[0]:
            _PACK_CONVT_CHUNK[0] = _lib.query("segk_pack_convt_chunk")
        n = Cinp * 4 * Coutp
        return n, (Cout, Cin, 0, Coutp, Cinp, 0), (n + _PACK_CONVT_CHUNK[0] - 1) // _PACK_CONVT_CHUNK[0]
    if kind == 3:
        Cout = param.shape[0]
        Coutp, CAp = pad32(Cout), pad32(d0)
        if not _PACK_CONVT_CHUNK[0]:
            _PACK_CONVT_CHUNK[0] = _lib.query("segk_pack_convt_chunk")
        n = CAp * Coutp
        return n, (Cout, d0, 0, Coutp, CAp, 0), (n + _PACK_CONVT_CHUNK[0] - 1) // _PACK_CONVT_CHUNK[0]
    Cout = param.shape[0]
    reps = d0 if d0 > 0 else 4
    return reps * pad32(Cout), (Cout, d0, 0, pad32(Cout), 0, 0), 1


def _pack_caches(model):
    seen, out, stack = set(), [], list(model.modules())
    while stack:
        m = stack.pop()
        if id(m) in seen:
            continue
        seen.add(id(m))
        c = getattr(m, "cache", None)
        if isinstance(c, PackCache):
            out.append(c)
        for v in vars(m).values():
            if isinstance(v, torch.nn.Module) and id(v) not in seen:
                stack.extend(v.modules())
    return out


def repack_stale(model):
    st = model.__dict__.get("_segk_pack_state")
    if st is None:
        st = model.__dict__["_segk_pack_state"] = {"epoch": _OPT_EPOCH[0], "caches": None, "tables": {}}
        return
    if st["epoch"] == _OPT_EPOCH[0]:
        return
    st["epoch"] = _OPT_EPOCH[0]
    if st["caches"] is None:
        st["caches"] = _pack_caches(model)
    groups = {}
    for cache in st["caches"]:
        for key_a, (kind, key_b, param, d0, d1, dtype) in cache.multi.items():
            ha = cache._c.get(key_a)
            hb = cache._c.get(key_b) if key_b is not None else None
            if ha is None or (key_b is not None and hb is None):
                continue
            if not param.is_cuda or param.dtype != torch.float32 or not param.is_contiguous():
                continue
            ver = (param._version, param.data_ptr(), param.device, _OPT_EPOCH[0] if param.requires_grad else -1)
            if ha[0] == ver and (hb is None or hb[0] == ver):
                continue
            n, _, _ = _entry_geometry(kind, param, d0, d1)
            want = torch.float32 if kind == 2 else dtype
            if ha[1].numel() != n or ha[1].dtype != want or not ha[1].is_contiguous():
                continue
            if hb is not None and (hb[1].numel() != n or hb[1].dtype != want or not hb[1].is_contiguous()):
                continue
            groups.setdefault((dtype, param.device), []).append(
                (cache, key_a, key_b, ver, param, ha[1], None if hb is None else hb[1], kind, d0, d1))
    for (dtype, dev), items in groups.items():
        if len(items) < 2:
            continue
        for c0 in range(0, len(items), 64):
            chunk = items[c0:c0 + 64]
            sig = tuple((it[4].data_ptr(), it[5].data_ptr(), 0 if it[6] is None else it[6].data_ptr(), it[7], it[8], it[9])
                        for it in chunk)
            tab = st["tables"].get((dtype, dev, c0))
            if tab is None or tab[0] != sig:
                import numpy as np
                words = np.zeros((len(chunk), 8), dtype=np.int64)
                ints = words.view(np.int32).reshape(len(chunk), 16)
                blk = 0
                for i, (_, _, _, _, param, a, b, kind, d0, d1) in enumerate(chunk):
                    _, dims, nblk = _entry_geometry(kind, param, d0, d1)
                    words[i, 0], words[i, 1], words[i, 2] = param.data_ptr(), a.data_ptr(), 0 if b is None else b.data_ptr()
                    ints[i, 6:12] = dims
                    ints[i, 12], ints[i, 13] = blk, kind
                    blk += nblk
                tab = (sig, torch.from_numpy(words).to(dev), blk)
                st["tables"][(dtype, dev, c0)] = tab
            with torch.cuda.device(dev):
                _lib.call("segk_pack_multi", tab[1].data_ptr(), len(chunk), tab[2], _DT[dtype], _stream())
            for cache, key_a, key_b, ver, _, a, b, _, _, _ in chunk:
                cache._c[key_a] = (ver, a)
                if key_b is not None:
                    cache._c[key_b] = (ver, b)


def pack_convt(w, dtype, mode):
    Cin, Cout = w.shape[0], w.shape[1]
    dst = torch.empty((pad32(Cin) * 4 * pad32(Cout),), dtype=dtype, device=w.device)
    wf = w.detach()
    if wf.dtype != torch.float32 or not wf.is_contiguous():
        wf = wf.float().contiguous()
    _lib.call("segk_pack_convt_weight", wf.data_ptr(), dst.data_ptr(), Cin, Cout, pad32(Cin), pad32(Cout), mode,
              _DT[dtype], _stream())
    return dst


class KernelTimer:

    def __init__(self):
        self.rows = {}
        self.levels = {}

    def span(self, tag, flops=0.0, nbytes=0.0):
        return _Span(self, tag, flops, nbytes)

    @staticmethod
    def _sum(rows):
        out = {}
        for key, r in rows.items():
            ms = sum(a.elapsed_time(b) for a, b in r["ev"])
            out[key] = {"launches": len(r["ev"]), "ms": ms, "flops": r["flops"], "bytes": r["bytes"]}
        return out

    def summary(self):
        torch.cuda.synchronize()
        return self._sum(self.rows)

    def level_summary(self):
        torch.cuda.synchronize()
        return self._sum(self.levels)


class _Span:
    def __init__(self, timer, tag, flops, nbytes):
        self.t, self.tag, self.flops, self.nbytes = timer, tag, flops, nbytes

    def __enter__(self):
        self.a = torch.cuda.Event(enable_timing=True)
        self.a.record()

    def __exit__(self, *exc):
        b = torch.cuda.Event(enable_timing=True)
        b.record()
        r = self.t.rows.setdefault(self.tag, {"ev": [], "flops": 0.0, "bytes": 0.0})
        r["ev"].append((self.a, b))
        r["flops"] += self.flops
        r["bytes"] += self.nbytes
        if _LEVEL is not None:
            phase = {"conv3x3_igemm": "dgrad" if _LEVEL[1] else "fwd", "wgrad3x3": "wgrad"}.get(self.tag, "other")
            r = self.t.levels.setdefault((_LEVEL[0], phase), {"ev": [], "flops": 0.0, "bytes": 0.0})
            r["ev"].append((self.a, b))
            r["flops"] += self.flops
            r["bytes"] += self.nbytes


class _NoSpan:
    def __enter__(self):
        return None

    def __exit__(self, *exc):
        return False


_NOSPAN = _NoSpan()
TIMER = None
_LEVEL = None


def name_levels(model):
    for name, m in model.named_modules():
        if hasattr(m, "bn_modules") and hasattr(m, "cache"):
            m.__dict__["_segk_level"] = name or "block"


class _level_scope:
    def __init__(self, mod, backward):
        self.v = (mod.__dict__.get("_segk_level"), backward) if TIMER is not None else None

    def __enter__(self):
        global _LEVEL
        self.prev = _LEVEL
        if self.v is not None and self.v[0] is not None:
            _LEVEL = self.v

    def __exit__(self, *exc):
        global _LEVEL
        _LEVEL = self.prev
        return False


def clock_probe(launches=4, blocks=256, iters=20000, device=None):
    dev = torch.device("cuda", torch.cuda.current_device()) if device is None else torch.device(device)
    res = {"method": f"s_memtime / s_memrealtime (100 MHz) around {iters} rounds of 16 v_mfma_f32_32x32x16_bf16 (or 32 "
                     f"v_mfma_f32_16x16x32_bf16: the same matrix work) per wave, one wave per SIMD on {blocks} workgroups, "
                     f"launch {launches} of {launches} back to back; pseudo-random register operands"}
    for shape, name in ((0, "mfma_32x32x16"), (1, "mfma_16x16x32")):
        out = torch.zeros((blocks * 4 * 2,), dtype=torch.int64, device=dev)
        with torch.cuda.device(dev):
            for _ in range(launches):
                _lib.call("segk_clock_probe", out.data_ptr(), blocks, iters, shape, _stream())
            torch.cuda.synchronize(dev)
        t = out.view(-1, 2).double().cpu()
        ghz = (t[:, 0] / t[:, 1].clamp(min=1.0)) * 0.1
        ms = float(t[:, 1].median()) / 1e5
        res[name] = {"median_ghz": round(float(ghz.median()), 4), "min_ghz": round(float(ghz.min()), 4),
                     "max_ghz": round(float(ghz.max()), 4), "probe_ms": round(ms, 3),
                     "probe_pflops": round(blocks * 4 * iters * 16 * 32768.0 / (ms * 1e-3) / 1e15, 3)}
    res["median_ghz"] = res["mfma_32x32x16"]["median_ghz"]
    return res


def _span(tag, flops=0.0, nbytes=0.0):
    return _NOSPAN if TIMER is None else TIMER.span(tag, flops, nbytes)


def _es(dtype):
    return 2 if dtype == torch.bfloat16 else 4


def _f32(n, dev):
    return torch.empty((n,), dtype=torch.float32, device=dev)


_ZERO_PAGES = {}


def _zero_page(dev):
    key = torch.device(dev)
    if key.type == "cuda" and key.index is None:
        key = torch.device("cuda", torch.cuda.current_device())
    z = _ZERO_PAGES.get(key)
    if z is None:
        z = torch.zeros(256, dtype=torch.uint8, device=key)
        _ZERO_PAGES[key] = z
    return z


def conv3x3(srcA, ptrA, CAp, ptrB, CBp, wpacked, out_ptr, CO1p, out2_ptr, CO2p, B, H, W, dtype, scale=None,
            shift=None, stats=None, alg=None, tag="conv3x3_igemm"):
    cin, cout = alg if alg else (CAp + CBp, CO1p + CO2p)
    P, e = B * H * W, _es(dtype)
    with _span(tag, 2.0 * P * 9 * cin * cout, P * (cin + cout) * e + 9.0 * cin * cout * e):
        _lib.call("segk_conv3x3", ptrA, ptrB, wpacked.data_ptr(), 0, _p(scale), _p(shift), out_ptr, out2_ptr,
                  _p(stats), B, H, W, CAp, CBp, CO1p, CO2p, _DT[dtype], _stream())


def wgrad(dz_ptr, CDp, ptrA, CAp, ptrB, CBp, B, H, W, geo, dtype, dev, scale=None, shift=None, alg=None):
    taps = {0: 9, 1: 1, 2: 4}[geo]
    cd, ck = alg if alg else (CDp, CAp + CBp)
    P, e = B * H * W, _es(dtype)
    pk = P * (4 if geo == 2 else 1)
    tiles = _lib.query("segk_wgrad_tiles", B, H, W, geo, _DT[dtype])
    S = _lib.query("segk_wgrad_split", tiles, CDp, CAp, CBp, geo, _DT[dtype])
    slabs = _f32(S * CDp * taps * (CAp + CBp), dev)
    tag = {0: "wgrad3x3", 1: "wgrad1x1", 2: "wgrad_convt"}[geo]
    with _span(tag, 2.0 * P * taps * cd * ck, (P * cd + pk * ck) * e + 4.0 * taps * cd * ck):
        _lib.call("segk_wgrad", dz_ptr, ptrA, ptrB, _p(scale), _p(shift), slabs.data_ptr(), _zero_page(dev).data_ptr(),
                  S, B, H, W, CDp, CAp, CBp, geo, _DT[dtype], _stream())
    return slabs, S


_GRAD_DEST = None
_GRAD_DEST_USED = set()


def grad_destination_begin(callback):
    global _GRAD_DEST
    _GRAD_DEST = callback
    _GRAD_DEST_USED.clear()


def grad_destination_end():
    global _GRAD_DEST
    _GRAD_DEST = None
    _GRAD_DEST_USED.clear()


def _grad_buffer(param, shape, dev):
    if _GRAD_DEST is not None and param is not None and param.data_ptr() not in _GRAD_DEST_USED:
        d = _GRAD_DEST(param)
        if d is not None and tuple(d.shape) == tuple(shape) and d.dtype == torch.float32:
            _GRAD_DEST_USED.add(param.data_ptr())
            return d
    return torch.empty(shape, dtype=torch.float32, device=dev)


def wgrad_to_param(slabs, S, shape, N, CA, CB, taps, dev, param=None):
    grad = _grad_buffer(param, shape, dev)
    with _span("wgrad_reduce", 0.0, 4.0 * (S + 1) * grad.numel()):
        _lib.call("segk_wgrad_reduce", slabs.data_ptr(), S, grad.data_ptr(), N, CA, CB, pad32(N), pad32(CA),
                  pad32(CB) if CB else 0, taps, _stream())
    return grad


class ReduceBatch:

    def __init__(self, dev):
        self.dev, self.jobs, self.keep, self.nbytes = dev, [], [], 0.0

    def add_weight(self, slabs, S, shape, N, CA, CB, taps, param=None):
        grad = _grad_buffer(param, shape, self.dev)
        self.jobs.append(_lib.ReduceJob(slabs.data_ptr(), grad.data_ptr(), 0, S, N, CA, CB, pad32(N), pad32(CA),
                                        pad32(CB) if CB else 0, taps, 0))
        self.keep.append(slabs)
        self.nbytes += 4.0 * (S + 1) * grad.numel()
        return grad

    def add_colsum(self, part, rows, ntot, col0, ncols):
        out = _f32(ncols, self.dev)
        self.jobs.append(_lib.ReduceJob(part.data_ptr(), out.data_ptr(), 1, rows, ntot, col0, ncols, 0, 0, 0, 0, 0))
        self.keep.append(part)
        self.nbytes += 8.0 * rows * ncols
        return out

    def flush(self):
        for i in range(0, len(self.jobs), 4):
            chunk = self.jobs[i:i + 4]
            arr = (_lib.ReduceJob * len(chunk))(*chunk)
            with _span("wgrad_reduce", 0.0, self.nbytes * len(chunk) / len(self.jobs)):
                _lib.call("segk_wgrad_reduce_multi", arr, len(chunk), _stream())
        self.jobs, self.keep, self.nbytes = [], [], 0.0


def bn_finalize(stats, tiles, C, count, conv_bias, bn_w, bn_b, rmean, rvar, momentum, eps, training, dev):
    Cp = pad32(C)
    scale, shift = _f32(Cp, dev), _f32(Cp, dev)
    mean, rstd = _f32(Cp, dev), _f32(Cp, dev)
    with _span("bn_finalize", 0.0, 8.0 * tiles * Cp if training else 0.0):
        _lib.call("segk_bn_finalize", _p(stats), tiles, Cp, C, float(count), _p(conv_bias), bn_w.data_ptr(),
                  bn_b.data_ptr(), _p(rmean), _p(rvar), float(momentum), float(eps), int(training), scale.data_ptr(),
                  shift.data_ptr(), mean.data_ptr(), rstd.data_ptr(), _stream())
    return scale, shift, mean, rstd


def bn_relu_bwd(dy_ptr, z_ptr, dz_ptr, scale, shift, mean, rstd, P, C, dtype, dev, ready=None, frozen=False):
    Cp = pad32(C)
    dgamma, dbeta = _f32(C, dev), _f32(C, dev)
    if frozen:
        nb = _lib.query("segk_bn_bwd_blocks", P, Cp, _DT[dtype])
        part, coef = _f32(nb * Cp * 2, dev), _f32(2 * Cp, dev)
        scratch = torch.empty((P * Cp,), dtype=dtype, device=dev)
        _lib.call("segk_bn_relu_bwd", dy_ptr, z_ptr, scratch.data_ptr(), scale.data_ptr(), shift.data_ptr(), mean.data_ptr(),
                  rstd.data_ptr(), P, Cp, C, part.data_ptr(), dgamma.data_ptr(), dbeta.data_ptr(), coef.data_ptr(),
                  _DT[dtype], _stream())
        zero_part = torch.zeros((Cp * 2,), dtype=torch.float32, device=dev)
        unused_g, unused_b = _f32(C, dev), _f32(C, dev)
        _lib.call("segk_bn_relu_bwd_from_part", dy_ptr, z_ptr, dz_ptr, scale.data_ptr(), shift.data_ptr(),
                  mean.data_ptr(), rstd.data_ptr(), P, Cp, C, zero_part.data_ptr(), 1, unused_g.data_ptr(), unused_b.data_ptr(),
                  coef.data_ptr(), _DT[dtype], _stream())
        return dgamma, dbeta
    if ready is not None:
        part, nb = ready
        coef = _f32(2 * Cp, dev)
        with _span("bn_relu_bwd", 0.0, 3.0 * P * C * _es(dtype)):
            _lib.call("segk_bn_relu_bwd_from_part", dy_ptr, z_ptr, dz_ptr, scale.data_ptr(), shift.data_ptr(),
                      mean.data_ptr(), rstd.data_ptr(), P, Cp, C, part.data_ptr(), nb, dgamma.data_ptr(), dbeta.data_ptr(),
                      coef.data_ptr(), _DT[dtype], _stream())
        return dgamma, dbeta
    nb = _lib.query("segk_bn_bwd_blocks", P, Cp, _DT[dtype])
    part, coef = _f32(nb * Cp * 2, dev), _f32(2 * Cp, dev)
    with _span("bn_relu_bwd", 0.0, 5.0 * P * C * _es(dtype)):
        _lib.call("segk_bn_relu_bwd", dy_ptr, z_ptr, dz_ptr, scale.data_ptr(), shift.data_ptr(), mean.data_ptr(),
                  rstd.data_ptr(), P, Cp, C, part.data_ptr(), dgamma.data_ptr(), dbeta.data_ptr(), coef.data_ptr(),
                  _DT[dtype], _stream())
    return dgamma, dbeta


def channel_sum(ptr, P, C, dtype, dev):
    Cp = pad32(C)
    nb = _lib.query("segk_bn_bwd_blocks", P, Cp, _DT[dtype])
    part, out = _f32(nb * Cp, dev), _f32(C, dev)
    _lib.call("segk_channel_sum", ptr, P, Cp, C, part.data_ptr(), out.data_ptr(), _DT[dtype], _stream())
    return out


_ZERO_POOL = {}


def _zero_grad_like(n, dev):
    key = torch.device(dev)
    if key.type == "cuda" and key.index is None:
        key = torch.device("cuda", torch.cuda.current_device())
    pool = _ZERO_POOL.get(key)
    if pool is None or pool[0] != _OPT_EPOCH[0] or pool[2] + n > pool[1].numel():
        pool = [_OPT_EPOCH[0], torch.zeros(max(16384, 4 * n), dtype=torch.float32, device=key), 0]
        _ZERO_POOL[key] = pool
    off = pool[2]
    pool[2] = off + (n + 3) // 4 * 4
    return pool[1][off:off + n]


_NBT_DEFER = None


class defer_batch_counters:

    def __enter__(self):
        global _NBT_DEFER
        self.prev, _NBT_DEFER = _NBT_DEFER, []
        return self

    def __exit__(self, *exc):
        global _NBT_DEFER
        pending, _NBT_DEFER = _NBT_DEFER, self.prev
        if pending and exc[0] is None:
            torch._foreach_add_(pending, 1)
        return False


def _bump_batch_counters(*bns):
    for bn in bns:
        if bn.num_batches_tracked is None:
            continue
        if _NBT_DEFER is not None:
            _NBT_DEFER.append(bn.num_batches_tracked)
        else:
            bn.num_batches_tracked.add_(1)


def _param_f32(p):
    t = p.detach()
    if t.dtype != torch.float32 or not t.is_contiguous():
        t = t.float().contiguous()
    return t


def _bn_momentum(bn):
    if bn.momentum is None:
        raise NotImplementedError("BatchNorm2d(momentum=None) (cumulative moving average) is not supported by the fused "
                                  "DoubleConv kernels; the reference uses the default momentum 0.1 (unet/unet.py:17,20)")
    return bn.momentum


def _convt_fwd(mod, x_t, px, w, b, B, H, W, Cin, Cout, dtype, dev, both=False):
    Cinp, Coutp = pad32(Cin), pad32(Cout)
    if both:
        wp = mod.cache.get_pair(("tf", dtype), ("td", dtype), w, lambda: (pack_convt(w, dtype, 0), pack_convt(w, dtype, 1)),
                                meta=(1, 0, 0, dtype))
    else:
        wp = mod.cache.get(("tf", dtype), w, lambda: pack_convt(w, dtype, 0))

    def bias4():
        t = torch.zeros((4, Coutp), dtype=torch.float32, device=dev)
        t[:, :Cout] = _param_f32(b)
        return t
    b4 = None if b is None else mod.cache.get_registered(("tb", dtype), b, bias4, meta=(2, 0, 0, dtype))
    out = torch.empty((B, 2 * H, 2 * W, Coutp), dtype=dtype, device=dev)
    with _span("convt_fwd", 2.0 * B * H * W * Cin * 4 * Cout, B * H * W * (Cin + 4 * Cout) * _es(dtype)):
        _lib.call("segk_convt2x2_fwd", px, wp.data_ptr(), _p(b4), out.data_ptr(), B, H, W, Cinp, Coutp, _DT[dtype],
                  _stream())
    return out


def _convt_bwd(mod, x_t, w, pd, B, H, W, Cin, Cout, dtype, dev, need_dx, has_bias, chan_sum=None, batch=None):
    Cinp, Coutp = pad32(Cin), pad32(Cout)
    px = act_info(x_t, dtype)[0]
    dx = None
    if need_dx:
        wd = mod.cache.get(("td", dtype), w, lambda: pack_convt(w, dtype, 1))
        dxb = torch.empty((B, H, W, Cinp), dtype=dtype, device=dev)
        with _span("convt_dgrad", 2.0 * B * H * W * Cin * 4 * Cout, B * H * W * (Cin + 4 * Cout) * _es(dtype)):
            _lib.call("segk_convt2x2_dgrad", pd, wd.data_ptr(), dxb.data_ptr(), B, H, W, Cinp, Coutp, _DT[dtype],
                      _stream())
        dx = act_view(dxb, Cin)
    slabs, S = wgrad(px, Cinp, pd, Coutp, 0, 0, B, H, W, 2, dtype, dev, alg=(Cin, Cout))
    if batch is not None:
        dw = batch.add_weight(slabs, S, w.shape, Cin, Cout, 0, 4, param=w)
    else:
        dw = wgrad_to_param(slabs, S, w.shape, Cin, Cout, 0, 4, dev, param=w)
    db = None
    if has_bias:
        db = chan_sum if chan_sum is not None else channel_sum(pd, B * 4 * H * W, Cout, dtype, dev)
    return dx, dw, db


def _head_fwd(px, Cp, w, b, B, C, H, W, dtype, dev, bn=None):
    ncls = w.shape[0]
    if ncls > _lib.MAX_CLASSES:
        raise RuntimeError(f"output head supports up to {_lib.MAX_CLASSES} classes, got {ncls}")
    w2 = _param_f32(w).reshape(ncls, C)
    logits = torch.empty((B, ncls, H, W), dtype=torch.float32, device=dev)
    with _span("head_fwd", 2.0 * B * H * W * C * ncls, B * H * W * (C * _es(dtype) + 4 * ncls)):
        if bn is not None:
            _lib.call("segk_head_fwd_bn", px, bn[0].data_ptr(), bn[1].data_ptr(), w2.data_ptr(), _param_f32(b).data_ptr(),
                      logits.data_ptr(), B, H, W, Cp, C, ncls, _DT[dtype], _stream())
        else:
            _lib.call("segk_head_fwd", px, w2.data_ptr(), _param_f32(b).data_ptr(), logits.data_ptr(), B, H, W, Cp, C,
                      ncls, _DT[dtype], _stream())
    return logits


def _head_bwd(dlogits, px, Cp, w, B, C, H, W, dtype, dev, bn=None, on_z=False):
    ncls = w.shape[0]
    dl = dlogits
    if dl.dtype != torch.float32 or not dl.is_contiguous():
        dl = dl.float().contiguous()
    w2 = _param_f32(w).reshape(ncls, C)
    dy = torch.empty((B, H, W, Cp), dtype=dtype, device=dev)
    part = _f32(_lib.query("segk_head_part_floats", B * H * W, Cp), dev)
    dw = _grad_buffer(w, w.shape, dev)
    db = _f32(ncls, dev)
    ready = None
    with _span("head_bwd", 4.0 * B * H * W * C * ncls, B * H * W * (2 * C * _es(dtype) + 4 * ncls)):
        if on_z:
            sc, sh, mu, rs = bn
            bnpart, nb = None, 0
            if FUSE_BN_REDUCE:
                nb = _lib.query("segk_head_bwd_blocks", B * H * W)
                bnpart = _f32(nb * Cp * 2, dev)
                ready = (bnpart, nb)
            _lib.call("segk_head_bwd_bn", dl.data_ptr(), px, w2.data_ptr(), dy.data_ptr(), part.data_ptr(),
                      dw.data_ptr(), db.data_ptr(), B, H, W, Cp, C, ncls, sc.data_ptr(), sh.data_ptr(), mu.data_ptr(),
                      rs.data_ptr(), _p(bnpart), _DT[dtype], _stream())
        elif bn is not None and FUSE_BN_REDUCE:
            sc, sh, mu, rs = bn
            nb = _lib.query("segk_head_bwd_blocks", B * H * W)
            bnpart = _f32(nb * Cp * 2, dev)
            _lib.call("segk_head_bwd_bnstat", dl.data_ptr(), px, w2.data_ptr(), dy.data_ptr(), part.data_ptr(),
                      dw.data_ptr(), db.data_ptr(), B, H, W, Cp, C, ncls, sc.data_ptr(), sh.data_ptr(), mu.data_ptr(),
                      rs.data_ptr(), bnpart.data_ptr(), _DT[dtype], _stream())
            ready = (bnpart, nb)
        else:
            _lib.call("segk_head_bwd", dl.data_ptr(), px, w2.data_ptr(), dy.data_ptr(), part.data_ptr(), dw.data_ptr(),
                      db.data_ptr(), B, H, W, Cp, C, ncls, _DT[dtype], _stream())
    return dy, dw, db, ready


class BlockCfg:
    __slots__ = ("mod", "up_mod", "emit_pool")

    def __init__(self, mod, up_mod=None, emit_pool=False):
        self.mod, self.up_mod, self.emit_pool = mod, up_mod, emit_pool


class DoubleConvFn(torch.autograd.Function):

    @staticmethod
    def forward(ctx, cfg, xa, xb, w1, b1, g1, be1, w2, b2, g2, be2, up_x, up_w, up_b, head_w, head_b):
        with _level_scope(cfg.mod, False):
            return DoubleConvFn._forward(ctx, cfg, xa, xb, w1, b1, g1, be1, w2, b2, g2, be2, up_x, up_w, up_b, head_w, head_b)

    @staticmethod
    def _forward(ctx, cfg, xa, xb, w1, b1, g1, be1, w2, b2, g2, be2, up_x, up_w, up_b, head_w, head_b):
        mod = cfg.mod
        dtype = mod.compute_dtype or _compute_dtype
        _require_cuda(xa, "DoubleConvReLU")
        dev = xa.device
        B, CA, H, W = xa.shape
        up_t, up_dims = None, None
        if up_x is not None:
            if xb is not None:
                raise ValueError("DoubleConvFn: give either xb or up_x")
            _require_cuda(up_x, "ConvTranspose2d")
            Bu, Cin_u, Hu, Wu = up_x.shape
            Cout_u = up_w.shape[1]
            if (2 * Hu, 2 * Wu) != (H, W):
                raise RuntimeError(f"Sizes of tensors must match except in dimension 1: {tuple(xa.shape)} vs "
                                   f"{(Bu, Cout_u, 2 * Hu, 2 * Wu)} (H and W must be multiples of 16)")
            up_t, pux, _ = _raw(up_x, dtype)
            ubuf = _convt_fwd(cfg.up_mod, up_t, pux, up_w, up_b, Bu, Hu, Wu, Cin_u, Cout_u, dtype, dev,
                              both=any(ctx.needs_input_grad))
            xb = act_view(ubuf, Cout_u)
            up_dims = (Bu, Hu, Wu, Cin_u, Cout_u)
        CB = 0 if xb is None else xb.shape[1]
        Cout = w1.shape[0]
        Coutp = pad32(Cout)
        training = mod.training
        bn1, bn2 = mod.bn_modules()
        want_grad = any(ctx.needs_input_grad)
        stem_rows = 0
        if (xb is None and act_info(xa, dtype) is None and xa.dtype == torch.float32 and xa.is_contiguous()
                and w1.dtype == torch.float32 and w1.is_contiguous()):
            stem_rows = _lib.query("segk_stem3x3_rows", B, H, W, CA, Cout, _DT[dtype])
        stem_raw = False
        if stem_rows:
            xa_t, pA, CAp = None, 0, pad32(CA)
            if want_grad and _lib.query("segk_stem3x3_wgrad_slabs", B, H, W, CA, Cout, _DT[dtype]):
                xa_t, stem_raw = xa.detach(), True
            elif want_grad:
                xbuf = torch.empty((B, H, W, CAp), dtype=dtype, device=dev)
                xa_t, pA = act_view(xbuf, CA), xbuf.data_ptr()
        else:
            xa_t, pA, CAp = _raw(xa, dtype)
        xb_t, pB, CBp = (None, 0, 0) if xb is None else _raw(xb, dtype)
        if training and want_grad:
            w1p = mod.cache.get_pair(("w1f", dtype), ("w1d", dtype), w1, lambda: pack_conv_both(w1, CA, CB, dtype),
                                     meta=(0, CA, CB, dtype))
            w2p = mod.cache.get_pair(("w2f", dtype), ("w2d", dtype), w2, lambda: pack_conv_both(w2, Cout, 0, dtype),
                                     meta=(0, Cout, 0, dtype))
        else:
            w1p = mod.cache.get(("w1f", dtype), w1, lambda: pack_conv(w1, CA, CB, dtype, 0))
            w2p = mod.cache.get(("w2f", dtype), w2, lambda: pack_conv(w2, Cout, 0, dtype, 0))
        tiles1 = stem_rows or _lib.query("segk_conv_tiles", B, H, W, CAp + CBp, Coutp, _DT[dtype])
        tiles2 = _lib.query("segk_conv_tiles", B, H, W, Coutp, Coutp, _DT[dtype])
        P = B * H * W

        z1 = torch.empty((B, H, W, Coutp), dtype=dtype, device=dev)
        st1 = _f32(_lib.query("segk_bn_stats_floats", tiles1, Coutp), dev) if training else None
        if stem_rows:
            e = _es(dtype)
            with _span("conv3x3_igemm", 2.0 * P * 9 * CA * Cout, P * (4 * CA + Cout * e) + 9.0 * CA * Cout * 4):
                _lib.call("segk_stem3x3", xa.data_ptr(), w1.data_ptr(), z1.data_ptr(), pA, _p(st1), B, H, W, CA, Cout,
                          _DT[dtype], _stream())
        else:
            conv3x3(xa_t, pA, CAp, pB, CBp, w1p, z1.data_ptr(), Coutp, 0, 0, B, H, W, dtype, stats=st1, alg=(CA + CB, Cout))
        sc1, sh1, mu1, rs1 = bn_finalize(st1, tiles1, Cout, P, None if b1 is None else _param_f32(b1), _param_f32(g1),
                                         _param_f32(be1), bn1.running_mean, bn1.running_var, _bn_momentum(bn1), bn1.eps,
                                         training, dev)
        z2 = torch.empty((B, H, W, Coutp), dtype=dtype, device=dev)
        st2 = _f32(_lib.query("segk_bn_stats_floats", tiles2, Coutp), dev) if training else None
        a1 = None
        if training and want_grad and _lib.query("segk_conv_writes_act_q", Coutp, Coutp, _DT[dtype]):
            a1 = torch.empty((B, H, W, Coutp), dtype=dtype, device=dev)
            with _span("conv3x3_igemm", 2.0 * P * 9 * Cout * Cout, (P * 2 * Cout + 9.0 * Cout * Cout) * _es(dtype)):
                _lib.call("segk_conv3x3_act", z1.data_ptr(), w2p.data_ptr(), sc1.data_ptr(), sh1.data_ptr(), z2.data_ptr(),
                          a1.data_ptr(), _p(st2), B, H, W, Coutp, Coutp, _DT[dtype], _stream())
        else:
            conv3x3(z1, z1.data_ptr(), Coutp, 0, 0, w2p, z2.data_ptr(), Coutp, 0, 0, B, H, W, dtype, scale=sc1,
                    shift=sh1, stats=st2, alg=(Cout, Cout))
        sc2, sh2, mu2, rs2 = bn_finalize(st2, tiles2, Cout, P, None if b2 is None else _param_f32(b2), _param_f32(g2),
                                         _param_f32(be2), bn2.running_mean, bn2.running_var, _bn_momentum(bn2), bn2.eps,
                                         training, dev)
        if training:
            _bump_batch_counters(bn1, bn2)
        head_on_z = head_w is not None and HEAD_ON_Z
        y = None if head_on_z else torch.empty((B, H, W, Coutp), dtype=dtype, device=dev)
        pooled = None
        if head_on_z:
            pass
        elif cfg.emit_pool:
            if H < 2 or W < 2:
                raise RuntimeError("MaxPool2d(2,2): input smaller than the window")
            pooled = torch.empty((B, H // 2, W // 2, Coutp), dtype=dtype, device=dev)
            with _span("bn_relu_apply", 0.0, 2.25 * P * Cout * _es(dtype)):
                _lib.call("segk_bn_relu_apply_pool", z2.data_ptr(), y.data_ptr(), pooled.data_ptr(), sc2.data_ptr(),
                          sh2.data_ptr(), B, H, W, Coutp, _DT[dtype], _stream())
        else:
            with _span("bn_relu_apply", 0.0, 2.0 * P * Cout * _es(dtype)):
                _lib.call("segk_bn_relu_apply", z2.data_ptr(), y.data_ptr(), sc2.data_ptr(), sh2.data_ptr(), P, Coutp,
                          _DT[dtype], _stream())
        logits = None
        if head_on_z:
            logits = _head_fwd(z2.data_ptr(), Coutp, head_w, head_b, B, Cout, H, W, dtype, dev, bn=(sc2, sh2))
        elif head_w is not None:
            logits = _head_fwd(y.data_ptr(), Coutp, head_w, head_b, B, Cout, H, W, dtype, dev)

        ctx.cfg, ctx.dtype, ctx.dims = cfg, dtype, (B, H, W, CA, CB, Cout)
        ctx.training = training
        ctx.has_bias = (b1 is not None, b2 is not None)
        ctx.up_dims = up_dims
        ctx.has_head = head_w is not None
        ctx.head_on_z = head_on_z
        ctx.stem_raw = stem_raw
        ctx.save_for_backward(xa_t, xb_t, z1, z2, sc1, sh1, mu1, rs1, sc2, sh2, mu2, rs2, w1, w2, a1,
                              y if (cfg.emit_pool or head_w is not None) else None, up_t, up_w, head_w)
        if logits is not None:
            return logits
        if pooled is not None:
            y_out = act_view(y, Cout)
            ctx.y_ref = weakref.ref(y_out)
            return y_out, act_view(pooled, Cout)
        return act_view(y, Cout)

    @staticmethod
    def backward(ctx, *grads):
        with _level_scope(ctx.cfg.mod, True):
            return DoubleConvFn._backward(ctx, *grads)

    @staticmethod
    def _backward(ctx, *grads):
        frozen = not ctx.training
        (xa_t, xb_t, z1, z2, sc1, sh1, mu1, rs1, sc2, sh2, mu2, rs2, w1, w2, a1, y, up_t, up_w, head_w) = ctx.saved_tensors
        cfg, dtype = ctx.cfg, ctx.dtype
        mod = cfg.mod
        B, H, W, CA, CB, Cout = ctx.dims
        dev = z1.device
        Coutp, CAp, CBp = pad32(Cout), pad32(CA), (pad32(CB) if CB else 0)
        P = B * H * W
        pA = 0 if ctx.stem_raw else act_info(xa_t, dtype)[0]
        pB = 0 if xb_t is None else act_info(xb_t, dtype)[0]
        need = ctx.needs_input_grad

        ready = None
        d_head_w = d_head_b = None
        keep = None
        if ctx.has_head:
            src = z2 if ctx.head_on_z else y
            dy_buf, d_head_w, d_head_b, ready = _head_bwd(grads[0], src.data_ptr(), Coutp, head_w, B, Cout, H, W, dtype, dev,
                                                          bn=(sc2, sh2, mu2, rs2), on_z=ctx.head_on_z)
            pdy, keep = dy_buf.data_ptr(), dy_buf
        elif cfg.emit_pool:
            dy, dpool = grads
            rc_skip, rc_pool = sys.getrefcount(dy), sys.getrefcount(dpool)
            if dpool is None:
                keep, pdy, _ = _raw(dy, dtype)
            else:
                dp_t, pdp, _ = _raw(dpool, dtype)
                if dy is None:
                    keep = torch.empty((B, H, W, Coutp), dtype=dtype, device=dev)
                    pdy, acc, nbytes = keep.data_ptr(), 0, 2.25
                else:
                    yo = getattr(ctx, "y_ref", lambda: None)()
                    uc = getattr(dy, "_use_count", None)
                    shared = uc is None or uc() > 2 or rc_skip > rc_pool
                    hooked = INPLACE_SKIP_GRAD is False or shared or (yo is not None and bool(yo._backward_hooks))
                    keep, pdy, _ = _raw(dy, dtype)
                    if hooked and keep.data_ptr() == dy.data_ptr():
                        keep = _private_act_copy(keep, dtype)
                        pdy = keep.data_ptr()
                    acc, nbytes = 1, 3.25
                nb = _lib.query("segk_maxpool_bwd_stat_blocks", B, H, W, Coutp, _DT[dtype]) if FUSE_BN_REDUCE else 0
                with _span("maxpool_bwd", 0.0, nbytes * P * Cout * _es(dtype)):
                    if nb > 0:
                        part = _f32(nb * Coutp * 2, dev)
                        _lib.call("segk_maxpool2x2_bwd_bnstat", y.data_ptr(), pdp, pdy, B, H, W, Coutp, acc,
                                  sc2.data_ptr(), sh2.data_ptr(), mu2.data_ptr(), rs2.data_ptr(), part.data_ptr(),
                                  z2.data_ptr(), _DT[dtype], _stream())
                        ready = (part, nb)
                    else:
                        _lib.call("segk_maxpool2x2_bwd", y.data_ptr(), pdp, pdy, B, H, W, Coutp, acc, _DT[dtype],
                                  _stream())
        else:
            keep, pdy, _ = _raw(grads[0], dtype)

        dz2 = torch.empty((B, H, W, Coutp), dtype=dtype, device=dev)
        dg2, dbe2 = bn_relu_bwd(pdy, z2.data_ptr(), dz2.data_ptr(), sc2, sh2, mu2, rs2, P, Cout, dtype, dev, ready=ready,
                                frozen=frozen)
        del keep
        w2d = mod.cache.get(("w2d", dtype), w2, lambda: pack_conv(w2, Cout, 0, dtype, 1))
        da1 = torch.empty((B, H, W, Coutp), dtype=dtype, device=dev)
        conv3x3(dz2, dz2.data_ptr(), Coutp, 0, 0, w2d, da1.data_ptr(), Coutp, 0, 0, B, H, W, dtype, alg=(Cout, Cout))
        if a1 is not None:
            slabs, S = wgrad(dz2.data_ptr(), Coutp, a1.data_ptr(), Coutp, 0, 0, B, H, W, 0, dtype, dev, alg=(Cout, Cout))
        else:
            slabs, S = wgrad(dz2.data_ptr(), Coutp, z1.data_ptr(), Coutp, 0, 0, B, H, W, 0, dtype, dev, scale=sc1,
                             shift=sh1, alg=(Cout, Cout))
        dw2 = wgrad_to_param(slabs, S, w2.shape, Cout, Cout, 0, 9, dev, param=w2)
        rb = ReduceBatch(dev)
        del slabs, dz2

        dg1, dbe1 = bn_relu_bwd(da1.data_ptr(), z1.data_ptr(), da1.data_ptr(), sc1, sh1, mu1, rs1, P, Cout, dtype, dev,
                                frozen=frozen)
        dz1 = da1
        dxa = dxb = None
        dxb_buf, chan_sum = None, None
        has_up = ctx.up_dims is not None
        if need[1] or need[2] or has_up:
            w1d = mod.cache.get(("w1d", dtype), w1, lambda: pack_conv(w1, CA, CB, dtype, 1))
            dxa_buf = torch.empty((B, H, W, CAp), dtype=dtype, device=dev)
            dxb_buf = torch.empty((B, H, W, CBp), dtype=dtype, device=dev) if CB else None
            std = None
            if has_up:
                tiles_d = _lib.query("segk_conv_tiles", B, H, W, Coutp, CAp + CBp, _DT[dtype])
                std = _f32(_lib.query("segk_bn_stats_floats", tiles_d, CAp + CBp), dev)
            conv3x3(dz1, dz1.data_ptr(), Coutp, 0, 0, w1d, dxa_buf.data_ptr(), CAp, _p(dxb_buf), CBp, B, H, W, dtype,
                    stats=std, alg=(Cout, CA + CB))
            dxa = act_view(dxa_buf, CA)
            dxb = act_view(dxb_buf, CB) if CB else None
            if has_up:
                chan_sum = rb.add_colsum(std, tiles_d, CAp + CBp, CAp, CB)
        if ctx.stem_raw:
            S = _lib.query("segk_stem3x3_wgrad_slabs", B, H, W, CA, Cout, _DT[dtype])
            slabs = _f32(S * 64 * 32, dev)
            with _span("wgrad3x3", 2.0 * P * 9 * CA * Cout, P * (Cout * _es(dtype) + 4 * CA) + 4.0 * 9 * CA * Cout):
                _lib.call("segk_stem3x3_wgrad", xa_t.data_ptr(), dz1.data_ptr(), slabs.data_ptr(), B, H, W, CA, Cout,
                          _DT[dtype], _stream())
            dw1 = wgrad_to_param(slabs, S, w1.shape, Cout, 9 * CA, 0, 1, dev, param=w1)
        else:
            slabs, S = wgrad(dz1.data_ptr(), Coutp, pA, CAp, pB, CBp, B, H, W, 0, dtype, dev, alg=(Cout, CA + CB))
            dw1 = wgrad_to_param(slabs, S, w1.shape, Cout, CA, CB, 9, dev, param=w1)
        del slabs
        if frozen:
            db1 = sc1[:Cout] * dbe1 if ctx.has_bias[0] else None
            db2 = sc2[:Cout] * dbe2 if ctx.has_bias[1] else None
        else:
            db1 = _zero_grad_like(Cout, dev) if ctx.has_bias[0] else None
            db2 = _zero_grad_like(Cout, dev) if ctx.has_bias[1] else None

        d_up_x = d_up_w = d_up_b = None
        if has_up:
            Bu, Hu, Wu, Cin_u, Cout_u = ctx.up_dims
            d_up_x, d_up_w, d_up_b = _convt_bwd(cfg.up_mod, up_t, up_w, dxb_buf.data_ptr(), Bu, Hu, Wu, Cin_u, Cout_u, dtype,
                                                dev, need[11], cfg.up_mod.upsample.bias is not None, chan_sum=chan_sum,
                                                batch=rb)
            dxb = None
        rb.flush()
        return (None, dxa, dxb, dw1, db1, dg1, dbe1, dw2, db2, dg2, dbe2, d_up_x, d_up_w, d_up_b, d_head_w, d_head_b)


def double_conv(mod, xa, xb, params, emit_pool=False, head=None, up_mod=None, up_x=None):
    cfg = BlockCfg(mod, up_mod, emit_pool and head is None)
    uw = ub = None
    if up_mod is not None:
        uw, ub = up_mod.upsample.weight, up_mod.upsample.bias
    hw = hb = None
    if head is not None:
        hw, hb = head.weight, head.bias
    return DoubleConvFn.apply(cfg, xa, xb, *params, up_x, uw, ub, hw, hb)


class MaxPoolFn(torch.autograd.Function):

    @staticmethod
    def forward(ctx, x, dtype):
        _require_cuda(x, "MaxPool2d")
        x_t, px, Cp = _raw(x, dtype)
        B, C, H, W = x.shape
        y = torch.empty((B, H // 2, W // 2, Cp), dtype=dtype, device=x.device)
        with _span("maxpool_fwd", 0.0, 1.25 * B * H * W * C * _es(dtype)):
            _lib.call("segk_maxpool2x2_fwd", px, y.data_ptr(), B, H, W, Cp, _DT[dtype], _stream())
        ctx.save_for_backward(x_t)
        ctx.dtype = dtype
        return act_view(y, C)

    @staticmethod
    def backward(ctx, dy):
        (x_t,) = ctx.saved_tensors
        dtype = ctx.dtype
        B, C, H, W = x_t.shape
        px, Cp = act_info(x_t, dtype)
        dy_t, pdy, _ = _raw(dy, dtype)
        dx = torch.empty((B, H, W, Cp), dtype=dtype, device=x_t.device)
        with _span("maxpool_bwd", 0.0, 2.25 * B * H * W * C * _es(dtype)):
            _lib.call("segk_maxpool2x2_bwd", px, pdy, dx.data_ptr(), B, H, W, Cp, 0, _DT[dtype], _stream())
        return act_view(dx, C), None


class ConvT2x2Fn(torch.autograd.Function):

    @staticmethod
    def forward(ctx, mod, x, w, b):
        dtype = mod.compute_dtype or _compute_dtype
        _require_cuda(x, "ConvTranspose2d")
        B, Cin, H, W = x.shape
        Cout = w.shape[1]
        x_t, px, _ = _raw(x, dtype)
        out = _convt_fwd(mod, x_t, px, w, b, B, H, W, Cin, Cout, dtype, x.device, both=any(ctx.needs_input_grad))
        ctx.mod, ctx.dtype, ctx.dims = mod, dtype, (B, H, W, Cin, Cout)
        ctx.has_bias = b is not None
        ctx.save_for_backward(x_t, w)
        return act_view(out, Cout)

    @staticmethod
    def backward(ctx, dout):
        x_t, w = ctx.saved_tensors
        B, H, W, Cin, Cout = ctx.dims
        d_t, pd, _ = _raw(dout, ctx.dtype)
        dx, dw, db = _convt_bwd(ctx.mod, x_t, w, pd, B, H, W, Cin, Cout, ctx.dtype, x_t.device, ctx.needs_input_grad[1],
                                ctx.has_bias)
        return None, dx, dw, db


class Conv1x1Fn(torch.autograd.Function):

    @staticmethod
    def forward(ctx, mod, x, w, b):
        dtype = mod.compute_dtype or _compute_dtype
        _require_cuda(x, "Conv2d 1x1")
        dev = x.device
        B, Cin, H, W = x.shape
        Cout = w.shape[0]
        Cinp, Coutp = pad32(Cin), pad32(Cout)
        x_t, px, _ = _raw(x, dtype)
        wp = mod.cache.get_registered(("cf", dtype), w, lambda: pack_conv(w, Cin, 0, dtype, 0, taps=1), meta=(3, Cin, 0, dtype))

        def biasp():
            t = torch.zeros((Coutp,), dtype=torch.float32, device=dev)
            t[:Cout] = _param_f32(b)
            return t
        bp = None if b is None else mod.cache.get_registered(("cb", dtype), b, biasp, meta=(2, 1, 0, dtype))
        out = torch.empty((B, H, W, Coutp), dtype=dtype, device=dev)
        _lib.call("segk_conv1x1", px, wp.data_ptr(), _p(bp), out.data_ptr(), B, H, W, Cinp, Coutp, _DT[dtype], _stream())
        ctx.mod, ctx.dtype, ctx.dims = mod, dtype, (B, H, W, Cin, Cout)
        ctx.has_bias = b is not None
        ctx.save_for_backward(x_t, w)
        return act_view(out, Cout)

    @staticmethod
    def backward(ctx, dout):
        x_t, w = ctx.saved_tensors
        mod, dtype = ctx.mod, ctx.dtype
        B, H, W, Cin, Cout = ctx.dims
        dev = x_t.device
        Cinp, Coutp = pad32(Cin), pad32(Cout)
        d_t, pd, _ = _raw(dout, dtype)
        px = act_info(x_t, dtype)[0]
        dx = None
        if ctx.needs_input_grad[1]:
            wd = mod.cache.get(("cd", dtype), w, lambda: pack_conv(w, Cin, 0, dtype, 1, taps=1))
            dxb = torch.empty((B, H, W, Cinp), dtype=dtype, device=dev)
            _lib.call("segk_conv1x1", pd, wd.data_ptr(), 0, dxb.data_ptr(), B, H, W, Coutp, Cinp, _DT[dtype], _stream())
            dx = act_view(dxb, Cin)
        slabs, S = wgrad(pd, Coutp, px, Cinp, 0, 0, B, H, W, 1, dtype, dev)
        dw = wgrad_to_param(slabs, S, w.shape, Cout, Cin, 0, 1, dev, param=w)
        db = channel_sum(pd, B * H * W, Cout, dtype, dev) if ctx.has_bias else None
        return None, dx, dw, db


class ReconHeadFn(torch.autograd.Function):

    @staticmethod
    def forward(ctx, mod, x, w, b):
        dtype = mod.compute_dtype or _compute_dtype
        _require_cuda(x, "reconstruction head")
        dev = x.device
        B, Cin, H, W = x.shape
        Cout = w.shape[0]
        x_t, px, Cp = _raw(x, dtype)
        rec = torch.empty((B, Cout, H, W), dtype=torch.float32, device=dev)
        P = B * H * W
        with _span("recon_head_fwd", 2.0 * P * 9 * Cin * Cout, P * (Cin * _es(dtype) + 4 * Cout)):
            _lib.call("segk_recon_head_fwd", px, _param_f32(w).data_ptr(), 0 if b is None else _param_f32(b).data_ptr(),
                      rec.data_ptr(), B, H, W, Cp, Cin, Cout, _DT[dtype], _stream())
        ctx.mod, ctx.dtype, ctx.dims = mod, dtype, (B, H, W, Cin, Cout)
        ctx.has_bias = b is not None
        ctx.save_for_backward(x_t, w, rec)
        return rec

    @staticmethod
    def backward(ctx, drec):
        x_t, w, rec = ctx.saved_tensors
        mod, dtype = ctx.mod, ctx.dtype
        B, H, W, Cin, Cout = ctx.dims
        dev = x_t.device
        Cinp, Coutp = pad32(Cin), pad32(Cout)
        g = drec.detach()
        if g.dtype != torch.float32 or not g.is_contiguous():
            g = g.float().contiguous()
        dzb = torch.empty((B, H, W, Coutp), dtype=dtype, device=dev)
        P = B * H * W
        with _span("recon_sigmoid_bwd", 0.0, P * (8.0 * Cout + Coutp * _es(dtype))):
            _lib.call("segk_recon_sigmoid_bwd", g.data_ptr(), rec.data_ptr(), dzb.data_ptr(), B, H, W, Cout, Coutp,
                      _DT[dtype], _stream())
        pd = dzb.data_ptr()
        px = act_info(x_t, dtype)[0]
        dx = dw = db = None
        if ctx.needs_input_grad[1]:
            wd = mod.cache.get(("c3d", dtype), w, lambda: pack_conv(w, Cin, 0, dtype, 1))
            dxb = torch.empty((B, H, W, Cinp), dtype=dtype, device=dev)
            conv3x3(dzb, pd, Coutp, 0, 0, wd, dxb.data_ptr(), Cinp, 0, 0, B, H, W, dtype, alg=(Cout, Cin))
            dx = act_view(dxb, Cin)
        if ctx.needs_input_grad[2]:
            slabs, S = wgrad(pd, Coutp, px, Cinp, 0, 0, B, H, W, 0, dtype, dev, alg=(Cout, Cin))
            dw = wgrad_to_param(slabs, S, w.shape, Cout, Cin, 0, 9, dev, param=w)
        if ctx.has_bias and ctx.needs_input_grad[3]:
            db = channel_sum(pd, P, Cout, dtype, dev)
        return None, dx, dw, db


def _mse_operand(t, what):
    _require_cuda(t, what)
    t = t.detach()
    if t.dtype != torch.float32 or not t.is_contiguous():
        t = t.float().contiguous()
    return t


class MSELossFn(torch.autograd.Function):

    @staticmethod
    def forward(ctx, input, target, mean):
        if input.shape != target.shape:
            raise ValueError(f"MSELoss: input {tuple(input.shape)} and target {tuple(target.shape)} differ in shape")
        a, b = _mse_operand(input, "MSELoss input"), _mse_operand(target, "MSELoss target")
        n = a.numel()
        if n == 0:
            raise ValueError("MSELoss of empty tensors")
        dev = a.device
        part, out = _f32(_lib.MSE_PART_FLOATS, dev), _f32(1, dev)
        with _span("mse_fwd", 0.0, 8.0 * n):
            _lib.call("segk_mse_fwd", a.data_ptr(), b.data_ptr(), part.data_ptr(), part.numel(), out.data_ptr(), n, int(mean),
                      _stream())
        ctx.mean = int(mean)
        ctx.save_for_backward(a, b)
        return out.view(())

    @staticmethod
    def backward(ctx, gout):
        a, b = ctx.saved_tensors
        go = gout.detach().float().reshape(1).contiguous()
        da = torch.empty_like(a)
        db = torch.empty_like(b) if ctx.needs_input_grad[1] else None
        n = a.numel()
        with _span("mse_bwd", 0.0, (12.0 if db is None else 16.0) * n):
            _lib.call("segk_mse_bwd", a.data_ptr(), b.data_ptr(), go.data_ptr(), da.data_ptr(), _p(db), n, ctx.mean,
                      _stream())
        return da, db, None


class BilinearFn(torch.autograd.Function):

    @staticmethod
    def forward(ctx, x, size, dtype):
        _require_cuda(x, "bilinear resize")
        x_t, px, Cp = _raw(x, dtype)
        B, C, IH, IW = x.shape
        OH, OW = int(size[0]), int(size[1])
        y = torch.empty((B, OH, OW, Cp), dtype=dtype, device=x.device)
        with _span("bilinear_fwd", 0.0, B * (IH * IW + OH * OW) * C * _es(dtype)):
            _lib.call("segk_bilinear_fwd", px, y.data_ptr(), B, IH, IW, OH, OW, Cp, _DT[dtype], _stream())
        ctx.cfg = (B, C, IH, IW, OH, OW, Cp, dtype)
        return act_view(y, C)

    @staticmethod
    def backward(ctx, dy):
        B, C, IH, IW, OH, OW, Cp, dtype = ctx.cfg
        d_t, pd, _ = _raw(dy, dtype)
        dx = torch.empty((B, IH, IW, Cp), dtype=dtype, device=dy.device)
        with _span("bilinear_bwd", 0.0, B * (IH * IW + OH * OW) * C * _es(dtype)):
            tmp = _f32(B * OH * IW * Cp, dy.device) if OH * OW > 4 * IH * IW else None
            _lib.call("segk_bilinear_bwd", pd, dx.data_ptr(), _p(tmp), B, IH, IW, OH, OW, Cp, _DT[dtype], _stream())
        return act_view(dx, C), None, None


class HeadFn(torch.autograd.Function):

    @staticmethod
    def forward(ctx, mod, x, w, b):
        dtype = mod.compute_dtype or _compute_dtype
        _require_cuda(x, "output Conv2d")
        B, C, H, W = x.shape
        x_t, px, Cp = _raw(x, dtype)
        logits = _head_fwd(px, Cp, w, b, B, C, H, W, dtype, x.device)
        ctx.dtype, ctx.dims = dtype, (B, C, H, W)
        ctx.save_for_backward(x_t, w)
        return logits

    @staticmethod
    def backward(ctx, dlogits):
        x_t, w = ctx.saved_tensors
        dtype = ctx.dtype
        B, C, H, W = ctx.dims
        px, Cp = act_info(x_t, dtype)
        dy, dw, db, _ = _head_bwd(dlogits, px, Cp, w, B, C, H, W, dtype, x_t.device)
        return None, act_view(dy, C), dw, db


class SegLossFn(torch.autograd.Function):

    @staticmethod
    def forward(ctx, logits, target, class_weights, ignore_index, smooth, dice_weight, ce_weight):
        _require_cuda(logits, "segmentation loss")
        if logits.dim() != 4:
            raise ValueError(f"expected logits [N,C,H,W], got {tuple(logits.shape)}")
        N, C, H, W = logits.shape
        if C > _lib.MAX_CLASSES:
            raise RuntimeError(f"fused loss supports up to {_lib.MAX_CLASSES} classes, got {C}")
        lg = logits.detach()
        if lg.dtype != torch.float32 or not lg.is_contiguous():
            lg = lg.float().contiguous()
        tg = target.detach()
        if tg.dtype != torch.int64 or not tg.is_contiguous():
            tg = tg.long().contiguous()
        if tg.numel() != N * H * W:
            raise ValueError(f"target shape {tuple(target.shape)} does not match logits {tuple(logits.shape)}")
        dev = logits.device
        cw = None
        if class_weights is not None:
            cw = class_weights.detach().to(device=dev, dtype=torch.float32).contiguous()
            if cw.numel() != C:
                raise ValueError("class_weights must have one entry per class")
        ign = -1 if ignore_index is None else int(ignore_index)
        part = _f32(_lib.query("segk_loss_part_floats", N * H * W), dev)
        state = _f32(_lib.query("segk_loss_state_floats"), dev)
        out = _f32(1, dev)
        with _span("loss_fwd", 0.0, N * H * W * (4.0 * C + 8)):
            _lib.call("segk_loss_fwd", lg.data_ptr(), tg.data_ptr(), _p(cw), N, C, H * W, ign, float(smooth),
                      float(dice_weight), float(ce_weight), part.data_ptr(), state.data_ptr(), out.data_ptr(), _stream())
        ctx.cfg = (N, C, H, W, ign, float(dice_weight), float(ce_weight))
# ... 113 lines not shown
```

include/segk.h:

```cpp
#ifndef SEGK_H
#define SEGK_H
#include <stddef.h>
#include <stdint.h>
#ifdef __cplusplus
extern "C" {
#endif

#define SEGK_F32 0
#define SEGK_BF16 1
#define SEGK_MAX_CLASSES 8

typedef void* segk_stream_t;

#define SEGK_ABI_VERSION 318
#define SEGK_ENTRY_COUNT 94
int segk_version(void);
int segk_entry_count(void);
const char* segk_build_id(void);
const char* segk_last_error(void);

int segk_nchw_to_nhwc(const float* src, void* dst, int B, int C, int H, int W, int Cp, int dtype, segk_stream_t s);
int segk_nhwc_to_nchw(const void* src, float* dst, int B, int C, int H, int W, int Cp, int dtype, segk_stream_t s);

int segk_pack_conv_weight(const float* w, void* dst, int Cout, int CA, int CB, int Coutp, int CAp, int CBp,
                          int taps, int mode, int dtype, segk_stream_t s);
int segk_pack_conv3x3_both(const float* w, void* dst_fwd, void* dst_dgrad, int Cout, int CA, int CB, int Coutp, int CAp,
                           int CBp, int dtype, segk_stream_t s);
int segk_pack_multi(const void* table, int n, int total_blocks, int dtype, segk_stream_t s);
int segk_pack_convt_chunk(void);
int segk_pack_convt_weight(const float* w, void* dst, int Cin, int Cout, int Cinp, int Coutp, int mode, int dtype,
                           segk_stream_t s);

int segk_conv_writes_act_q(int Cin, int Cout, int dtype);
int segk_conv3x3_act(const void* srcA, const void* wpacked, const float* scale, const float* shift, void* out,
                     void* act_out, float* stats, int B, int H, int W, int CA, int CO, int dtype, segk_stream_t s);

int segk_stem3x3_rows(int B, int H, int W, int Cin, int Cout, int dtype);
int segk_stem3x3(const float* x_nchw, const float* w_oihw, void* z, void* x_nhwc, float* stats, int B, int H, int W, int Cin,
                 int Cout, int dtype, segk_stream_t s);
int segk_stem3x3_wgrad_slabs(int B, int H, int W, int Cin, int Cout, int dtype);
int segk_stem3x3_wgrad(const float* x_nchw, const void* dz, float* slabs, int B, int H, int W, int Cin, int Cout, int dtype,
                       segk_stream_t s);
int segk_conv_tiles(int B, int H, int W, int Cin, int Cout, int dtype);
int segk_bn_stats_floats(int tiles, int Cp);
int segk_conv3x3(const void* srcA, const void* srcB, const void* wpacked, const float* bias, const float* scale,
                 const float* shift, void* out, void* out2, float* stats, int B, int H, int W, int CA, int CB,
                 int CO1, int CO2, int dtype, segk_stream_t s);
int segk_conv1x1(const void* srcA, const void* wpacked, const float* bias, void* out, int B, int H, int W, int CA,
                 int CO, int dtype, segk_stream_t s);
int segk_convt2x2_fwd(const void* in, const void* wpacked, const float* bias4, void* out, int B, int H, int W,
                      int Cin, int Cout, int dtype, segk_stream_t s);
int segk_convt2x2_dgrad(const void* dout, const void* wpacked, void* din, int B, int H, int W, int Cin, int Cout,
                        int dtype, segk_stream_t s);

int segk_wgrad_tiles(int B, int H, int W, int geo, int dtype);
int segk_wgrad_split(int tiles, int CD, int CA, int CB, int geo, int dtype);
int segk_wgrad(const void* dz, const void* srcA, const void* srcB, const float* scale, const float* shift,
               float* slabs, const void* zeros64, int S, int B, int H, int W, int CD, int CA, int CB, int geo,
               int dtype, segk_stream_t s);
int segk_wgrad_reduce(const float* slabs, int S, float* grad, int N, int CA, int CB, int Np, int CAp, int CBp,
                      int taps, segk_stream_t s);
typedef struct segk_reduce_job {
  const float* src;
  float* dst;
  int kind, S, N, CA, CB, Np, CAp, CBp, taps, pad_;
} segk_reduce_job;
int segk_wgrad_reduce_multi(const segk_reduce_job* jobs, int n, segk_stream_t s);

int segk_bn_finalize(const float* stats, int tiles, int Cp, int C, double count, const float* conv_bias,
                     const float* gamma, const float* beta, float* running_mean, float* running_var, float momentum,
                     float eps, int training, float* scale, float* shift, float* mean, float* rstd, segk_stream_t s);
int segk_bn_relu_apply(const void* z, void* y, const float* scale, const float* shift, long P, int Cp, int dtype,
                       segk_stream_t s);
int segk_bn_relu_apply_pool(const void* z, void* y, void* pooled, const float* scale, const float* shift, int B, int H, int W,
                            int Cp, int dtype, segk_stream_t s);
int segk_bn_bwd_blocks(long P, int Cp, int dtype);
int segk_bn_relu_bwd(const void* dy, const void* z, void* dz, const float* scale, const float* shift,
                     const float* mean, const float* rstd, long P, int Cp, int C, float* part, float* dgamma,
                     float* dbeta, float* coef, int dtype, segk_stream_t s);

int segk_channel_sum(const void* x, long P, int Cp, int C, float* part, float* out, int dtype, segk_stream_t s);

int segk_maxpool2x2_fwd(const void* x, void* y, int B, int H, int W, int Cp, int dtype, segk_stream_t s);
int segk_maxpool2x2_bwd(const void* x, const void* dy, void* dx, int B, int H, int W, int Cp, int accumulate,
                        int dtype, segk_stream_t s);

int segk_maxpool_bwd_stat_blocks(int B, int H, int W, int Cp, int dtype);
int segk_maxpool2x2_bwd_bnstat(const void* x, const void* dy, void* dx, int B, int H, int W, int Cp, int accumulate,
                               const float* scale, const float* shift, const float* mean, const float* rstd, float* part,
                               const void* z, int dtype, segk_stream_t s);
int segk_bn_relu_bwd_from_part(const void* dy, const void* z, void* dz, const float* scale, const float* shift,
                               const float* mean, const float* rstd, long P, int Cp, int C, const float* part, int nb,
                               float* dgamma, float* dbeta, float* coef, int dtype, segk_stream_t s);

int segk_bilinear_fwd(const void* x, void* y, int B, int IH, int IW, int OH, int OW, int Cp, int dtype,
                      segk_stream_t s);
int segk_bilinear_bwd(const void* dy, void* dx, float* scratch, int B, int IH, int IW, int OH, int OW, int Cp, int dtype,
                      segk_stream_t s);

int segk_linear(const void* rows, const void* wpacked, const float* bias, void* out, long M, int K, int N, int act,
                int dtype, segk_stream_t s);
int segk_vit_patchify(const float* x, void* rows, int B, int C, int H, int W, int ps, int Kp, int dtype, segk_stream_t s);
int segk_vit_embed_ln(const void* proj, const float* cls, const float* pos, const float* gamma, const float* beta,
                      float eps, float* h, int B, int T, int D, int Dp, int dtype, segk_stream_t s);
int segk_add_layernorm(float* h, const void* delta, const float* gamma, const float* beta, float eps, void* out, long M,
                       int D, int Dp, int dtype, segk_stream_t s);
int segk_linear_splitk(const void* rows, const void* wpacked, const float* bias, void* out_parts, long M, int K, int N,
                       int ksplit, int dtype, segk_stream_t s);
int segk_add_layernorm_parts(float* h, const void* delta, int nparts, long part_stride, const float* gamma,
                             const float* beta, float eps, void* out, long M, int D, int Dp, int dtype, segk_stream_t s);
int segk_attention(const void* qkv, void* ctx, int B, int T, int heads, int head_dim, int ldq, int ldo, float scale,
                   int dtype, segk_stream_t s);
int segk_vit_tokens_to_grid(const float* h, void* out, int B, int T, int D, int Dp, int dtype, segk_stream_t s);

int segk_resize_pad(const void* img, void* out, int C, int H, int W, int nh, int nw, int T, int pad_top, int pad_left,
                    int mode, int elem, segk_stream_t s);
int segk_crop_resize(const float* slot, float* out, int C, int T, int pad_top, int pad_left, int nh, int nw, int oh,
                     int ow, int mode, segk_stream_t s);
int segk_resize_pad_u8(const uint8_t* img_hwc, float* out, int Cin, int H, int W, int nh, int nw, int T, int pad_top,
                       int pad_left, int mode, segk_stream_t s);
int segk_predict_mask(const float* slot, uint8_t* mask, uint8_t* color, const uint8_t* palette, uint64_t* counts,
                      const int64_t* labels, uint64_t* M, int C, int T, int pad_top, int pad_left, int nh, int nw, int oh,
                      int ow, int mode, segk_stream_t s);

int segk_resize_pad_flip(const void* img, void* out, int C, int H, int W, int nh, int nw, int T, int pad_top, int pad_left,
                         int mode, int elem, int flip, segk_stream_t s);
int segk_resize_pad_u8_flip(const uint8_t* img_hwc, float* out, int Cin, int H, int W, int nh, int nw, int T, int pad_top,
                            int pad_left, int mode, int flip, segk_stream_t s);

#define SEGK_MAX_VIEWS 16
#define SEGK_MERGE_PROB 0
#define SEGK_MERGE_LOGIT 1
typedef struct segk_view_desc {
  uint64_t slot;
  int32_t T, pad_top, pad_left, nh, nw;
  int32_t flip;
  int32_t kind;
  float weight;
  int32_t pad_[2];
} segk_view_desc;
int segk_predict_merge(const void* views_dev, int V, int C, int merge, int mode, int oh, int ow, uint8_t* mask,
                       uint8_t* color, const uint8_t* palette, uint64_t* counts, const int64_t* labels, uint64_t* M,
                       uint8_t* conf, float* scores, segk_stream_t s);

#define SEGK_TILE_PAD_ZERO 0
#define SEGK_TILE_PAD_REFLECT 1
#define SEGK_TILE_WINDOW_FLAT 0
#define SEGK_TILE_WINDOW_TRIANGLE 1
int segk_tile_gather_u8(const uint8_t* img_hwc, float* out, int Cin, int H, int W, int T, int overlap, int pad, int tile0,
                        int ntiles, segk_stream_t s);
int segk_tile_gather(const float* img_chw, float* out, int C, int H, int W, int T, int overlap, int pad, int tile0, int ntiles,
                     segk_stream_t s);
int segk_predict_tiles(const float* Y, int C, int kind, int merge, int window, int H, int W, int T, int overlap, uint8_t* mask,
                       uint8_t* color, const uint8_t* palette, uint64_t* counts, const int64_t* labels, uint64_t* M,
                       uint8_t* conf, float* scores, segk_stream_t s);

#define SEGK_CC_TILE_W 64
#define SEGK_CC_TILE_H 32
#define SEGK_CC_MAX_PIXELS (1L << 28)
#define SEGK_CC_WS_INTS(H, W) (16L + 11L * (long)(H) * (long)(W) + 2L * (long)(H))
int segk_cc_label(const uint8_t* mask, int32_t* labels, int32_t* num, int32_t* cls, int32_t* area, int32_t* box,
                  int32_t* first, int32_t* ws, int H, int W, int connectivity, int class_mask, int max_components,
                  segk_stream_t s);
int segk_cc_clean(const uint8_t* mask, uint8_t* out, int32_t* ws, int32_t* kept, int32_t* new_cls, int H, int W,
                  int min_area, int keep_mask, int max_components, segk_stream_t s);
int segk_mask_finish(const uint8_t* mask, uint8_t* color, const uint8_t* palette, uint64_t* counts, const int64_t* labels,
                     uint64_t* M, int C, int H, int W, segk_stream_t s);

int segk_head_fwd(const void* y, const float* w, const float* bias, float* logits, int B, int H, int W, int Cp,
                  int C, int ncls, int dtype, segk_stream_t s);
int segk_head_part_floats(long P, int Cp);
int segk_head_bwd(const float* dlogits, const void* y, const float* w, void* dy, float* part, float* dw, float* db,
                  int B, int H, int W, int Cp, int C, int ncls, int dtype, segk_stream_t s);

int segk_head_bwd_blocks(long P);
int segk_head_bwd_bnstat(const float* dlogits, const void* y, const float* w, void* dy, float* part, float* dw, float* db,
                         int B, int H, int W, int Cp, int C, int ncls, const float* scale, const float* shift,
                         const float* mean, const float* rstd, float* bnpart, int dtype, segk_stream_t s);

int segk_head_fwd_bn(const void* z, const float* scale, const float* shift, const float* w, const float* bias, float* logits,
                     int B, int H, int W, int Cp, int C, int ncls, int dtype, segk_stream_t s);
int segk_head_bwd_bn(const float* dlogits, const void* z, const float* w, void* dy, float* part, float* dw, float* db,
                     int B, int H, int W, int Cp, int C, int ncls, const float* scale, const float* shift,
                     const float* mean, const float* rstd, float* bnpart, int dtype, segk_stream_t s);

int segk_loss_part_floats(long P);
int segk_loss_state_floats(void);
int segk_loss_fwd(const float* logits, const int64_t* labels, const float* class_weights, int N, int C, long HW,
                  int ignore_index, float smooth, float dice_weight, float ce_weight, float* part, float* state,
                  float* loss_out, segk_stream_t s);
int segk_loss_bwd(const float* logits, const int64_t* labels, const float* class_weights, const float* state,
                  const float* grad_out, int N, int C, long HW, int ignore_index, float dice_weight, float ce_weight,
                  float* dlogits, segk_stream_t s);

int segk_prompt_mix_fwd(const float* clip_logits, const float* mask_logit, float* final_probs, int N, long HW,
                        segk_stream_t s);
int segk_prompt_mix_bwd(const float* clip_logits, const float* mask_logit, const float* dfinal, float* dmask_logit, int N,
                        long HW, segk_stream_t s);
int segk_prob_loss_fwd(const float* probs, const int64_t* labels, const float* class_weights, int N, int C, long HW,
                       int ignore_index, float smooth, float dice_weight, float nll_weight, int nll_log, float eps,
                       float* part, float* state, float* loss_out, segk_stream_t s);
int segk_prob_loss_bwd(const float* probs, const int64_t* labels, const float* class_weights, const float* state,
                       const float* grad_out, int N, int C, long HW, int ignore_index, float dice_weight,
                       float nll_weight, int nll_log, float eps, float* dprobs, segk_stream_t s);

int segk_prompt_scores(const int64_t* labels, const uint8_t* lut, const int32_t* centers, const double* w, int nw, int R,
                       double* scores, int32_t* cls, int B, int K, int H, int W, segk_stream_t s);
int segk_prompt_make(const int64_t* labels, const uint8_t* lut, const int32_t* centers, const int32_t* cls, const uint8_t* q,
                     int nq, float* heat, int64_t* target, int32_t* classes, int32_t* out_centers, uint8_t* valid, int B, int K,
                     int per_image, int H, int W, segk_stream_t s);
int segk_prompt_heatmap(const int32_t* points, int P, const uint8_t* q, int nq, float* heat, int H, int W, segk_stream_t s);

#define SEGK_AUG_RESIZE 0
#define SEGK_AUG_CENTER_CROP 1
#define SEGK_AUG_RANDOM_CROP 2
#define SEGK_AUG_ROTATION 3
#define SEGK_AUG_MASKING 4
#define SEGK_AUG_GRAYSCALE 5
#define SEGK_AUG_LAPLACE 6
#define SEGK_AUG_BLUR 7
#define SEGK_AUG_CONTRAST 8
#define SEGK_AUG_LAPLACE_ENTRIES 4096
typedef struct segk_aug_desc {
  const uint8_t* img;
  const uint8_t* lab;
  uint8_t* a_img;
  uint8_t* a_lab;
  int64_t A[6];
  uint64_t seed;
  int32_t H, W, img_c, lab_c;
  int32_t Ha, Wa;
  int32_t op;
  int32_t wy, wx, wh, ww;
  int32_t tab, aux;
  int32_t gh, gw;
  int32_t label_fill;
  int32_t pad_[2];
} segk_aug_desc;
int segk_aug_prefilter(const segk_aug_desc* descs, int n, int max_tiles, segk_stream_t s);
int segk_aug_resample(const segk_aug_desc* descs, int n, int T, const int32_t* cub_idx, const int16_t* cub_coef, int n_cub,
                      const uint8_t* contrast, int n_contrast, const int16_t* laplace, int n_laplace, const uint8_t* label_lut,
                      float* X, uint8_t* X8, int64_t* y, segk_stream_t s);
typedef struct segk_merge_desc {
  const uint8_t* img[2];
  const uint8_t* lab[2];
  int32_t H[2], W[2], img_c[2], lab_c[2];
} segk_merge_desc;
int segk_aug_merge(const segk_merge_desc* descs, const int32_t* tables, int n, int T, const uint8_t* label_lut, float* X,
                   uint8_t* X8, int64_t* y, segk_stream_t s);
int segk_label_hist(const void* labels, long n, int elem_bytes, int num_classes, int has_ignore, long ignore_index,
                    uint64_t* counts, segk_stream_t s);
int segk_rgb_label_to_classes(const uint8_t* rgb, uint8_t* out, long n, segk_stream_t s);

#define SEGK_PERTURB_LUT 0
#define SEGK_PERTURB_GAUSS_NOISE 1
#define SEGK_PERTURB_SALT_PEPPER 2
#define SEGK_PERTURB_OCCLUDE 3
#define SEGK_PERTURB_GAUSS_ENTRIES 4096
#define SEGK_PERTURB_POINT_TILE 4096
#define SEGK_PERTURB_BLUR_TH 32
#define SEGK_PERTURB_BLUR_TW 64
#define SEGK_PERTURB_BLUR_MAX 9
typedef struct segk_perturb_desc {
  const uint8_t* src;
  uint8_t* dst;
  uint64_t seed;
  int32_t H, W, src_c;
  int32_t tile0;
  int32_t p0, p1, p2;
  int32_t pad_;
} segk_perturb_desc;
int segk_perturb_point(const segk_perturb_desc* descs, int n, int total_tiles, int kind, const void* table, segk_stream_t s);
int segk_perturb_blur(const segk_perturb_desc* descs, int n, int total_tiles, int k, segk_stream_t s);

int segk_recon_head_fwd(const void* x, const float* w, const float* bias, float* rec, int B, int H, int W, int Cp, int Cin,
                        int Cout, int dtype, segk_stream_t s);
int segk_recon_sigmoid_bwd(const float* drec, const float* rec, void* dz, int B, int H, int W, int C, int Cp, int dtype,
                           segk_stream_t s);
#define SEGK_MSE_PART_FLOATS 1024
int segk_mse_fwd(const float* a, const float* b, float* part, int part_floats, float* out, long n, int mean, segk_stream_t s);
int segk_mse_bwd(const float* a, const float* b, const float* grad_out, float* da, float* db, long n, int mean,
                 segk_stream_t s);

int segk_clock_probe(uint64_t* out, int blocks, int iters, int shape, segk_stream_t s);
int segk_debug_poison_tickets(uint64_t pattern, segk_stream_t s);

int segk_confusion(const float* logits, const int64_t* labels, int N, int C, long HW, uint64_t* M, segk_stream_t s);

#ifdef __cplusplus
}
#endif
#endif
```

Baseline: 2729 images/sec.

## Fuse BN-ReLU backward into head backward and stem weight-gradient kernels

Adds two fused paths at the network ends. At the output, the head backward no longer writes a dy tensor; the decoder's last BN-ReLU backward recomputes dy from dlogits and the head weights while applying the BN gradient. At the input, the first BN-ReLU backward only computes statistics, and the stem wgrad kernel applies the BN-ReLU backward on the fly instead of reading a materialised dz. Both aim to cut full-resolution activation writes and reads, at the cost of recomputation and more complex kernels.

```diff
diff --git a/image_segmentation_amd/_lib.py b/image_segmentation_amd/_lib.py
--- a/image_segmentation_amd/_lib.py
+++ b/image_segmentation_amd/_lib.py
@@ -5,7 +5,7 @@
 LIB_PATH = os.path.join(_HERE, "csrc", "libsegk.so")
 
 F32, BF16 = 0, 1
-ABI_VERSION = 318
+ABI_VERSION = 319
 MAX_CLASSES = 8
 MAX_VIEWS = 16
 MSE_PART_FLOATS = 1024
@@ -35,6 +35,7 @@
     "segk_stem3x3": (_i, [_fp, _fp, _vp, _vp, _fp, _i, _i, _i, _i, _i, _i, _vp]),
     "segk_stem3x3_wgrad_slabs": (_i, [_i, _i, _i, _i, _i, _i]),
     "segk_stem3x3_wgrad": (_i, [_fp, _vp, _fp, _i, _i, _i, _i, _i, _i, _vp]),
+    "segk_stem3x3_wgrad_bn": (_i, [_fp, _vp, _vp, _fp, _fp, _fp, _fp, _fp, _fp, _i, _i, _i, _i, _i, _i, _vp]),
     "segk_conv1x1": (_i, [_vp, _vp, _fp, _vp, _i, _i, _i, _i, _i, _i, _vp]),
     "segk_convt2x2_fwd": (_i, [_vp, _vp, _fp, _vp, _i, _i, _i, _i, _i, _i, _vp]),
     "segk_convt2x2_dgrad": (_i, [_vp, _vp, _vp, _i, _i, _i, _i, _i, _i, _vp]),
@@ -48,12 +49,15 @@
     "segk_bn_relu_apply_pool": (_i, [_vp, _vp, _vp, _fp, _fp, _i, _i, _i, _i, _i, _vp]),
     "segk_bn_bwd_blocks": (_i, [_l, _i, _i]),
     "segk_bn_relu_bwd": (_i, [_vp, _vp, _vp, _fp, _fp, _fp, _fp, _l, _i, _i, _fp, _fp, _fp, _fp, _i, _vp]),
+    "segk_bn_relu_bwd_stats": (_i, [_vp, _vp, _fp, _fp, _fp, _fp, _l, _i, _i, _fp, _fp, _fp, _fp, _i, _vp]),
     "segk_channel_sum": (_i, [_vp, _l, _i, _i, _fp, _fp, _i, _vp]),
     "segk_maxpool2x2_fwd": (_i, [_vp, _vp, _i, _i, _i, _i, _i, _vp]),
     "segk_maxpool2x2_bwd": (_i, [_vp, _vp, _vp, _i, _i, _i, _i, _i, _i, _vp]),
     "segk_maxpool_bwd_stat_blocks": (_i, [_i, _i, _i, _i, _i]),
     "segk_maxpool2x2_bwd_bnstat": (_i, [_vp, _vp, _vp, _i, _i, _i, _i, _i, _fp, _fp, _fp, _fp, _fp, _vp, _i, _vp]),
     "segk_bn_relu_bwd_from_part": (_i, [_vp, _vp, _vp, _fp, _fp, _fp, _fp, _l, _i, _i, _fp, _i, _fp, _fp, _fp, _i, _vp]),
+    "segk_bn_relu_bwd_from_part_head": (_i, [_fp, _fp, _i, _vp, _vp, _fp, _fp, _fp, _fp, _i, _i, _i, _i, _i, _fp, _i, _fp, _fp, _fp, _i,
+                                              _vp]),
     "segk_bilinear_fwd": (_i, [_vp, _vp, _i, _i, _i, _i, _i, _i, _i, _vp]),
     "segk_bilinear_bwd": (_i, [_vp, _vp, _fp, _i, _i, _i, _i, _i, _i, _i, _vp]),
     "segk_linear": (_i, [_vp, _vp, _fp, _vp, _l, _i, _i, _i, _i, _vp]),
@@ -80,6 +84,7 @@
     "segk_head_fwd": (_i, [_vp, _fp, _fp, _fp, _i, _i, _i, _i, _i, _i, _i, _vp]),
     "segk_head_fwd_bn": (_i, [_vp, _fp, _fp, _fp, _fp, _fp, _i, _i, _i, _i, _i, _i, _i, _vp]),
     "segk_head_bwd_bn": (_i, [_fp, _vp, _fp, _vp, _fp, _fp, _fp, _i, _i, _i, _i, _i, _i, _fp, _fp, _fp, _fp, _fp, _i, _vp]),
+    "segk_head_bwd_bn_nody": (_i, [_fp, _vp, _fp, _fp, _fp, _fp, _i, _i, _i, _i, _i, _i, _fp, _fp, _fp, _fp, _fp, _i, _vp]),
     "segk_head_part_floats": (_i, [_l, _i]),
     "segk_head_bwd": (_i, [_fp, _vp, _fp, _vp, _fp, _fp, _fp, _i, _i, _i, _i, _i, _i, _i, _vp]),
     "segk_head_bwd_blocks": (_i, [_l]),
diff --git a/image_segmentation_amd/build.py b/image_segmentation_amd/build.py
--- a/image_segmentation_amd/build.py
+++ b/image_segmentation_amd/build.py
@@ -4,7 +4,7 @@
 from concurrent.futures import ThreadPoolExecutor
 
 CSRC = os.path.join(os.path.dirname(os.path.abspath(__file__)), "csrc")
-SOURCES = ["api.hip", "conv_igemm.hip", "conv_rs.hip", "convt_stream.hip", "stem.hip", "wgrad.hip", "bn_pool.hip", "pack.hip", "head_loss.hip", "recon.hip", "prompt.hip", "augment.hip", "perturb.hip", "components.hip", "resize.hip", "tiles.hip", "vit.hip", "gemm.hip", "probe.hip"]
+SOURCES = ["api.hip", "conv_igemm.hip", "conv_rs.hip", "convt_stream.hip", "stem.hip", "fused_ends.hip", "wgrad.hip", "bn_pool.hip", "pack.hip", "head_loss.hip", "recon.hip", "prompt.hip", "augment.hip", "perturb.hip", "components.hip", "resize.hip", "tiles.hip", "vit.hip", "gemm.hip", "probe.hip"]
 LIB = os.path.join(CSRC, "libsegk.so")
 FLAGS = ["--offload-arch=gfx950", "-O3", "-fPIC", "-std=c++17", "-ffp-contract=off", "-Wall", "-Wno-unused-function"]
 
diff --git a/image_segmentation_amd/csrc/bn_pool.hip b/image_segmentation_amd/csrc/bn_pool.hip
--- a/image_segmentation_amd/csrc/bn_pool.hip
+++ b/image_segmentation_amd/csrc/bn_pool.hip
@@ -785,6 +785,55 @@
              : bn_bwd_t<float>(dy, z, dz, scale, shift, mean, rstd, P, C, C_real, part, dgamma, dbeta, coef, st);
 }
 
+extern "C" int segk_bn_relu_bwd_stats(const void* dy, const void* z, const float* scale, const float* shift, const float* mean,
+                                      const float* rstd, long P, int C, int C_real, float* part, float* dgamma, float* dbeta,
+                                      float* coef, int dtype, segk_stream_t s) {
+  SEGK_REQUIRE_DTYPE("bn_relu_bwd_stats", dtype);
+  hipStream_t st = (hipStream_t)s;
+  SEGK_REQUIRE(dy && z && scale && shift && mean && rstd && part && dgamma && dbeta && coef, "bn_bwd_stats: null pointer");
+  SEGK_REQUIRE(P > 0 && C > 0 && C % 32 == 0 && C_real > 0 && C_real <= C, "bn_bwd_stats: bad shape");
+  auto run = [&](auto Tc) {
+    using T = decltype(Tc);
+    using E = ET<T>;
+    int cvb, rows, gy;
+    lane_geometry(C, E::VEC, &cvb, &rows, &gy);
+    const int gx = segk_bn_bwd_blocks(P, C, dtype);
+    const size_t lds = (size_t)rows * cvb * 2 * E::VEC * sizeof(float);
+    hipLaunchKernelGGL(bn_bwd_reduce_kernel<T>, dim3(gx, gy), dim3(256), lds, st, (const T*)dy, (const T*)z, scale, shift,
+                       mean, rstd, P, C, cvb, rows, part);
+    SEGK_CHECK_LAUNCH("bn_bwd_reduce");
+    hipLaunchKernelGGL(bn_bwd_finalize_kernel, dim3(C / 32), dim3(1024), 0, st, part, gx, C, C_real, (double)P, dgamma,
+                       dbeta, coef);
+    SEGK_CHECK_LAUNCH("bn_bwd_finalize");
+    return 0;
+  };
+  return dtype == SEGK_DT_BF16 ? run(bf16_t{}) : run(float{});
+}
+
+extern "C" int segk_bn_relu_bwd_from_part_head(const float* dlogits, const float* head_w, int ncls, const void* z, void* dz,
+                                               const float* scale, const float* shift, const float* mean, const float* rstd,
+                                               int B, int H, int W, int C, int C_real, const float* part, int nb, float* dgamma,
+                                               float* dbeta, float* coef, int dtype, segk_stream_t s) {
+  SEGK_REQUIRE_DTYPE("bn_relu_bwd_from_part_head", dtype);
+  hipStream_t st = (hipStream_t)s;
+  SEGK_REQUIRE(dlogits && head_w && z && dz && scale && shift && mean && rstd && part && dgamma && dbeta && coef && nb > 0,
+               "bn_bwd_from_part_head: bad arguments");
+  SEGK_REQUIRE(B > 0 && H > 0 && W > 0 && C > 0 && C % 32 == 0 && C_real > 0 && C_real <= C, "bn_bwd_from_part_head: bad shape");
+  SEGK_REQUIRE(ncls >= 1 && ncls <= SEGK_MAX_CLASSES, "bn_bwd_from_part_head: 1..%d classes supported, got %d", SEGK_MAX_CLASSES,
+               ncls);
+  const long P = (long)B * H * W, HW = (long)H * W;
+  SEGK_REQUIRE(P < (1L << 31), "bn_bwd_from_part_head: pixels are indexed with 32 bits: %ld pixels", P);
+  int cvb, rows, gy;
+  lane_geometry(C, dtype == SEGK_DT_BF16 ? 8 : 4, &cvb, &rows, &gy);
+  hipLaunchKernelGGL(bn_bwd_finalize_kernel, dim3(C / 32), dim3(1024), 0, st, part, nb, C, C_real, (double)P, dgamma,
+                     dbeta, coef);
+  SEGK_CHECK_LAUNCH("bn_bwd_finalize");
+  long ga = (P + rows - 1) / rows;
+  if (ga > 4096) ga = 4096;
+  return segk_bn_apply_head_launch(dlogits, head_w, ncls, z, dz, scale, shift, mean, rstd, coef, P, HW, C, C_real, cvb, rows,
+                                   (int)ga, gy, dtype, st);
+}
+
 extern "C" int segk_maxpool2x2_fwd(const void* x, void* y, int B, int H, int W, int C, int dtype, segk_stream_t s) {
   SEGK_REQUIRE_DTYPE("maxpool2x2_fwd", dtype);
   hipStream_t st = (hipStream_t)s;
diff --git a/image_segmentation_amd/csrc/fused_ends.hip b/image_segmentation_amd/csrc/fused_ends.hip
--- /dev/null
+++ b/image_segmentation_amd/csrc/fused_ends.hip
@@ -0,0 +1,453 @@
+#include <type_traits>
+#include "common.hpp"
+#include "segk_internal.h"
+#include "../../include/segk.h"
+
+namespace {
+
+typedef unsigned u32x4 __attribute__((ext_vector_type(4)));
+constexpr int MAXC = SEGK_MAX_CLASSES;
+constexpr int STEM_WAVES = 8;
+
+struct __attribute__((packed, aligned(4))) F4U { float v[4]; };
+
+__global__ __launch_bounds__(STEM_WAVES * 64, 4) void stem_wgrad_bn_kernel(
+    const float* __restrict__ x, const bf16_t* __restrict__ dy, const bf16_t* __restrict__ z, const float* __restrict__ scale,
+    const float* __restrict__ shift, const float* __restrict__ mean, const float* __restrict__ rstd,
+    const float* __restrict__ coef, float* __restrict__ slabs, int B, int H, int W, int Cin, long nblk) {
+  __shared__ __attribute__((aligned(16))) char lds[4 * 64 * 32 * 4];
+  typedef __attribute__((address_space(3))) s16x4* lds_v4;
+  const int lane = threadIdx.x & 63;
+  const int wave = __builtin_amdgcn_readfirstlane(threadIdx.x >> 6);
+  const int K = Cin * 9;
+  char* const slot = lds + wave * 2048;
+
+  const int j = lane & 31, hh = lane >> 5;
+  const int ci = j / 9, tap = j - ci * 9;
+  const int dyy = tap / 3 - 1, dx = tap % 3 - 1;
+  const bool jok = j < K;
+  const int g = lane >> 4, i16 = lane & 15, q = i16 >> 2, p = i16 & 3;
+  const int coff = (16 * (g & 1) + 4 * p) * 2, xa = 8 * (g >> 1) + q;
+  const int cg = lane & 7, pp = lane >> 3;
+  char* const st0 = slot + (cg >> 2) * 1024 + pp * 64 + (cg & 3) * 16;
+  float sc[8], sh[8], mu[8], rs[8], c1[8], c2[8];
+#pragma unroll
+  for (int e = 0; e < 8; ++e) {
+    const int c = cg * 8 + e;
+    sc[e] = scale[c]; sh[e] = shift[c]; mu[e] = mean[c]; rs[e] = rstd[c];
+    c1[e] = coef[2 * c]; c2[e] = coef[2 * c + 1];
+  }
+  auto apply = [&](const uint4 rz, const uint4 rd) {
+    float fz[8], fd[8];
+    unpack16<bf16_t>(rz, fz);
+    unpack16<bf16_t>(rd, fd);
+#pragma unroll
+    for (int e = 0; e < 8; ++e) {
+      const float gg = (fmaf(fz[e], sc[e], sh[e]) > 0.f) ? fd[e] : 0.f;
+      const float xh = (fz[e] - mu[e]) * rs[e];
+      fd[e] = sc[e] * (gg - c1[e] - xh * c2[e]);
+    }
+    return pack16<bf16_t>(fd);
+  };
+
+  f32x16 acc[2];
+#pragma unroll
+  for (int nh = 0; nh < 2; ++nh)
+#pragma unroll
+    for (int r = 0; r < 16; ++r) acc[nh][r] = 0.f;
+
+  const int W16 = W / 16;
+  const long step = (long)gridDim.x * STEM_WAVES;
+  for (long blk = (long)blockIdx.x * STEM_WAVES + wave; blk < nblk; blk += step) {
+    const long row = blk / W16;
+    const int x0 = (int)(blk - row * W16) * 16;
+    const long b = row / H;
+    const int y = (int)(row - b * H);
+    const size_t e0 = ((size_t)row * W + x0 + pp) * 64 + cg * 8;
+    const uint4 y0 = *(const uint4*)(dy + e0), z0 = *(const uint4*)(z + e0);
+    const uint4 y1 = *(const uint4*)(dy + e0 + 8 * 64), z1 = *(const uint4*)(z + e0 + 8 * 64);
+    float v[8];
+    const int xs = x0 + 8 * hh + dx;
+    const bool rok = jok & ((unsigned)(y + dyy) < (unsigned)H);
+    const float* src = x + ((size_t)(b * Cin + ci) * H + (y + dyy)) * W + xs;
+    if (rok && xs >= 0 && xs + 8 <= W) {
+      const F4U a = *(const F4U*)src, c = *(const F4U*)(src + 4);
+#pragma unroll
+      for (int e = 0; e < 4; ++e) { v[e] = a.v[e]; v[4 + e] = c.v[e]; }
+    } else {
+#pragma unroll
+      for (int e = 0; e < 8; ++e) v[e] = (rok && (unsigned)(xs + e) < (unsigned)W) ? src[e] : 0.f;
+    }
+    *(uint4*)st0 = apply(z0, y0);
+    *(uint4*)(st0 + 8 * 64) = apply(z1, y1);
+    const u32x4 fbv = {cvt_pk_bf16(v[0], v[1]), cvt_pk_bf16(v[2], v[3]), cvt_pk_bf16(v[4], v[5]), cvt_pk_bf16(v[6], v[7])};
+    const bf16x8 fb = __builtin_bit_cast(bf16x8, fbv);
+    __builtin_amdgcn_fence(__ATOMIC_RELEASE, "wavefront");
+#pragma unroll
+    for (int nh = 0; nh < 2; ++nh) {
+      const s16x4 a0 = __builtin_amdgcn_ds_read_tr16_b64_v4i16((lds_v4)(slot + nh * 1024 + xa * 64 + coff));
+      const s16x4 a1 = __builtin_amdgcn_ds_read_tr16_b64_v4i16((lds_v4)(slot + nh * 1024 + (xa + 4) * 64 + coff));
+      const bf16x8 fa = __builtin_bit_cast(bf16x8, __builtin_shufflevector(a0, a1, 0, 1, 2, 3, 4, 5, 6, 7));
+      acc[nh] = __builtin_amdgcn_mfma_f32_32x32x16_bf16(fa, fb, acc[nh], 0, 0, 0);
+    }
+  }
+
+  float* const red = (float*)lds;
+  const int col = lane & 31, lh = lane >> 5;
+  auto put = [&](int slot_i) {
+#pragma unroll
+    for (int nh = 0; nh < 2; ++nh)
+#pragma unroll
+      for (int r = 0; r < 16; ++r) {
+        const int n = 32 * nh + (r & 3) + 8 * (r >> 2) + 4 * lh;
+        red[(slot_i * 64 + n) * 32 + col] = acc[nh][r];
+      }
+  };
+  auto add = [&](int slot_i) {
+#pragma unroll
+    for (int nh = 0; nh < 2; ++nh)
+#pragma unroll
+      for (int r = 0; r < 16; ++r) {
+        const int n = 32 * nh + (r & 3) + 8 * (r >> 2) + 4 * lh;
+        acc[nh][r] += red[(slot_i * 64 + n) * 32 + col];
+      }
+  };
+  __syncthreads();
+  if (wave >= 4) put(wave - 4);
+  __syncthreads();
+  if (wave < 4) add(wave);
+  __syncthreads();
+  if (wave == 2 || wave == 3) put(wave - 2);
+  __syncthreads();
+  if (wave < 2) add(wave);
+  __syncthreads();
+  if (wave == 1) put(0);
+  __syncthreads();
+  if (wave == 0) {
+    add(0);
+    float* const slab = slabs + (size_t)blockIdx.x * 64 * 32;
+#pragma unroll
+    for (int nh = 0; nh < 2; ++nh)
+#pragma unroll
+      for (int r = 0; r < 16; ++r) {
+        const int n = 32 * nh + (r & 3) + 8 * (r >> 2) + 4 * lh;
+        slab[n * 32 + col] = acc[nh][r];
+      }
+  }
+}
+
+__device__ __forceinline__ void split_hw(long p, long HW, long& b, long& r) {
+  const unsigned bb = (unsigned)p / (unsigned)HW;
+  b = (long)bb;
+  r = p - (long)bb * HW;
+}
+
+#ifndef HEAD_BWD_VEC
+#define HEAD_BWD_VEC 4
+#endif
+template <typename T> struct HeadVec;
+template <> struct HeadVec<float> {
+  static constexpr int HV = 4;
+  using Raw = uint4;
+  static __device__ __forceinline__ void unpack(const Raw& v, float* f) { unpack16<float>(v, f); }
+  static __device__ __forceinline__ Raw pack(const float* f) { return pack16<float>(f); }
+};
+template <> struct HeadVec<bf16_t> {
+  static constexpr int HV = HEAD_BWD_VEC;
+  static_assert(HV == 4 || HV == 8, "head backward: 4 or 8 bf16 channels per thread");
+  using Raw = std::conditional_t<HV == 8, uint4, uint2>;
+  static __device__ __forceinline__ void unpack(const uint4& v, float* f) { unpack16<bf16_t>(v, f); }
+  static __device__ __forceinline__ void unpack(const uint2& v, float* f) {
+    f[0] = bf2f(v.x & 0xffffu); f[1] = __uint_as_float(v.x & 0xffff0000u);
+    f[2] = bf2f(v.y & 0xffffu); f[3] = __uint_as_float(v.y & 0xffff0000u);
+  }
+  static __device__ __forceinline__ uint4 pack_n(const float* f, std::integral_constant<int, 8>) { return pack16<bf16_t>(f); }
+  static __device__ __forceinline__ uint2 pack_n(const float* f, std::integral_constant<int, 4>) {
+    return make_uint2(pack_bf16x2(f[0], f[1]), pack_bf16x2(f[2], f[3]));
+  }
+  static __device__ __forceinline__ Raw pack(const float* f) { return pack_n(f, std::integral_constant<int, HV>{}); }
+};
+
+template <typename T, int NC>
+__global__ __launch_bounds__(256) void head_bwd_nody_kernel(const float* __restrict__ dlog, const T* __restrict__ y,
+                                                            const float* __restrict__ w, float* __restrict__ part, long P,
+                                                            long HW, int Cp, int C, int ncls, int cvb, int rows,
+                                                            const float* __restrict__ bn_scale,
+                                                            const float* __restrict__ bn_shift,
+                                                            const float* __restrict__ bn_mean,
+                                                            const float* __restrict__ bn_rstd, float* __restrict__ bnpart) {
+  constexpr int HV = HeadVec<T>::HV;
+  using Raw = typename HeadVec<T>::Raw;
+  extern __shared__ __attribute__((aligned(16))) char smem_raw[];
+  float* red = (float*)smem_raw;
+  float xa[HV], xb[HV], sg[HV], sgx[HV];
+#pragma unroll
+  for (int j = 0; j < HV; ++j) { xa[j] = 0.f; xb[j] = 0.f; sg[j] = 0.f; sgx[j] = 0.f; }
+  constexpr int RW = MAXC * HV + MAXC;
+  const int cx = threadIdx.x % cvb, ry = threadIdx.x / cvb;
+  const int cv = blockIdx.y * cvb + cx;
+  const bool active = cv < Cp / HV && ry < rows;
+  float wr[NC][HV], aw[NC][HV], ab[NC];
+#pragma unroll
+  for (int k = 0; k < NC; ++k) {
+    ab[k] = 0.f;
+#pragma unroll
+    for (int j = 0; j < HV; ++j) {
+      const int c = cv * HV + j;
+      wr[k][j] = (active && k < ncls && c < C) ? w[(size_t)k * C + c] : 0.f;
+      aw[k][j] = 0.f;
+    }
+  }
+  float zc[HV], zh[HV];
+  if (active) {
+#pragma unroll
+    for (int j = 0; j < HV; ++j) {
+      const int c = cv * HV + j;
+      const float rs = bn_rstd[c];
+      zc[j] = bn_scale[c]; zh[j] = bn_shift[c];
+      xa[j] = rs; xb[j] = -bn_mean[c] * rs;
+    }
+  }
+  if (active) {
+    auto pixel = [&](const float (&dl)[NC], const Raw raw) {
+      float f[HV], z[HV], o[HV];
+      HeadVec<T>::unpack(raw, f);
+#pragma unroll
+      for (int j = 0; j < HV; ++j) { z[j] = f[j]; f[j] = fmaxf(fmaf(f[j], zc[j], zh[j]), 0.f); }
+      HeadVec<T>::unpack(HeadVec<T>::pack(f), f);
+#pragma unroll
+      for (int j = 0; j < HV; ++j) o[j] = 0.f;
+#pragma unroll
+      for (int k = 0; k < NC; ++k) {
+        ab[k] += dl[k];
+#pragma unroll
+        for (int j = 0; j < HV; ++j) {
+          o[j] = fmaf(dl[k], wr[k][j], o[j]);
+          aw[k][j] = fmaf(dl[k], f[j], aw[k][j]);
+        }
+      }
+#pragma unroll
+      for (int j = 0; j < HV; ++j) {
+        const float gg = f[j] > 0.f ? o[j] : 0.f;
+        sg[j] += gg;
+        sgx[j] = fmaf(gg, fmaf(z[j], xa[j], xb[j]), sgx[j]);
+      }
+    };
+    auto load_dl = [&](long b, long r, float (&dl)[NC]) {
+#pragma unroll
+      for (int k = 0; k < NC; ++k) {
+        const float v = dlog[(b * ncls + (k < ncls ? k : ncls - 1)) * HW + r];
+        dl[k] = (k < ncls) ? v : 0.f;
+      }
+    };
+    auto advance = [&](long& b, long& r, long d) {
+      r += d;
+      while (r >= HW) { r -= HW; ++b; }
+    };
+#ifndef HEAD_BWD_PIF
+#define HEAD_BWD_PIF 2
+#endif
+    constexpr int PIF = HEAD_BWD_PIF;
+    const long step = (long)gridDim.x * rows;
+    long p = (long)blockIdx.x * rows + ry;
+    long bS[PIF], rS[PIF];
+    bS[0] = 0; rS[0] = 0;
+    if (p < P) split_hw(p, HW, bS[0], rS[0]);
+#pragma unroll
+    for (int u = 1; u < PIF; ++u) { bS[u] = bS[u - 1]; rS[u] = rS[u - 1]; advance(bS[u], rS[u], step); }
+    for (; p + (PIF - 1) * step < P; p += PIF * step) {
+      float dl[PIF][NC];
+      Raw rw[PIF];
+#pragma unroll
+      for (int u = 0; u < PIF; ++u) rw[u] = *(const Raw*)(y + (size_t)(p + u * step) * Cp + cv * HV);
+#pragma unroll
+      for (int u = 0; u < PIF; ++u) load_dl(bS[u], rS[u], dl[u]);
+#pragma unroll
+      for (int u = 0; u < PIF; ++u) pixel(dl[u], rw[u]);
+#pragma unroll
+      for (int u = 0; u < PIF; ++u) advance(bS[u], rS[u], PIF * step);
+    }
+    for (; p < P; p += step) {
+      float dl0[NC];
+      const Raw r0 = *(const Raw*)(y + (size_t)p * Cp + cv * HV);
+      load_dl(bS[0], rS[0], dl0);
+      pixel(dl0, r0);
+      advance(bS[0], rS[0], step);
+    }
+  }
+  if (ry < rows) {
+    float* q = red + ((size_t)ry * cvb + cx) * RW;
+#pragma unroll
+    for (int k = 0; k < NC; ++k) {
+#pragma unroll
+      for (int j = 0; j < HV; ++j) q[k * HV + j] = aw[k][j];
+      q[MAXC * HV + k] = ab[k];
+    }
+  }
+  __syncthreads();
+  if (ry == 0 && cv < Cp / HV) {
+    float* dst = part + (size_t)blockIdx.x * MAXC * (Cp + 1);
+#pragma unroll
+    for (int k = 0; k < NC; ++k) {
+#pragma unroll
+      for (int j = 0; j < HV; ++j) {
+        float s = 0.f;
+        for (int r2 = 0; r2 < rows; ++r2) s += red[((size_t)r2 * cvb + cx) * RW + k * HV + j];
+        dst[k * (Cp + 1) + cv * HV + j] = s;
+      }
+      if (cv == 0) {
+        float s = 0.f;
+        for (int r2 = 0; r2 < rows; ++r2) s += red[((size_t)r2 * cvb + cx) * RW + MAXC * HV + k];
+        dst[k * (Cp + 1) + Cp] = s;
+      }
+    }
+  }
+  __syncthreads();
+  if (ry < rows) {
+    float* q = red + ((size_t)ry * cvb + cx) * RW;
+#pragma unroll
+    for (int j = 0; j < HV; ++j) { q[j] = sg[j]; q[HV + j] = sgx[j]; }
+  }
+  __syncthreads();
+  if (ry == 0 && cv < Cp / HV) {
+#pragma unroll
+    for (int j = 0; j < HV; ++j) {
+      float a = 0.f, b2 = 0.f;
+      for (int r2 = 0; r2 < rows; ++r2) {
+        const float* q = red + ((size_t)r2 * cvb + cx) * RW;
+        a += q[j];
+        b2 += q[HV + j];
+      }
+      ((float2*)bnpart)[(size_t)blockIdx.x * Cp + cv * HV + j] = make_float2(a, b2);
+    }
+  }
+}
+
+template <typename T, int NC>
+__global__ __launch_bounds__(256) void bn_bwd_apply_head_kernel(const float* __restrict__ dlog, const float* __restrict__ w,
+                                                                const T* __restrict__ z, T* __restrict__ dz,
+                                                                const float* scale, const float* shift, const float* mean,
+                                                                const float* rstd, const float* coef, long P, long HW,
+                                                                int C, int C_real, int ncls, int cvb, int rows) {
+  using E = ET<T>;
+  const int cx = threadIdx.x % cvb, ry = threadIdx.x / cvb;
+  const int cv = blockIdx.y * cvb + cx;
+  if (cv >= C / E::VEC || ry >= rows) return;
+  float sc[E::VEC], sh[E::VEC], mu[E::VEC], rs[E::VEC], c1[E::VEC], c2[E::VEC];
+  float wr[NC][E::VEC];
+#pragma unroll
+  for (int j = 0; j < E::VEC; ++j) {
+    const int c = cv * E::VEC + j;
+    sc[j] = scale[c]; sh[j] = shift[c]; mu[j] = mean[c]; rs[j] = rstd[c];
+    c1[j] = coef[2 * c]; c2[j] = coef[2 * c + 1];
+#pragma unroll
+    for (int k = 0; k < NC; ++k) wr[k][j] = (k < ncls && c < C_real) ? w[(size_t)k * C_real + c] : 0.f;
+  }
+  const long step = (long)gridDim.x * rows;
+  const size_t cofs = (size_t)cv * E::VEC;
+  long p = (long)blockIdx.x * rows + ry;
+  long b = 0, r = 0;
+  if (p < P) split_hw(p, HW, b, r);
+  for (; p < P; p += step) {
+    const size_t off = (size_t)p * C + cofs;
+    const uint4 rz = *(const uint4*)(z + off);
+    float dl[NC];
+#pragma unroll
+    for (int k = 0; k < NC; ++k) {
+      const float v = dlog[(b * ncls + (k < ncls ? k : ncls - 1)) * HW + r];
+      dl[k] = (k < ncls) ? v : 0.f;
+    }
+    float fz[E::VEC], fd[E::VEC];
+    unpack16<T>(rz, fz);
+#pragma unroll
+    for (int j = 0; j < E::VEC; ++j) fd[j] = 0.f;
+#pragma unroll
+    for (int k = 0; k < NC; ++k)
+#pragma unroll
+      for (int j = 0; j < E::VEC; ++j) fd[j] = fmaf(dl[k], wr[k][j], fd[j]);
+    unpack16<T>(pack16<T>(fd), fd);
+#pragma unroll
+    for (int j = 0; j < E::VEC; ++j) {
+      const float g = (fmaf(fz[j], sc[j], sh[j]) > 0.f) ? fd[j] : 0.f;
+      const float xh = (fz[j] - mu[j]) * rs[j];
+      fd[j] = sc[j] * (g - c1[j] - xh * c2[j]);
+    }
+    *(uint4*)(dz + off) = pack16<T>(fd);
+    r += step;
+    while (r >= HW) { r -= HW; ++b; }
+  }
+}
+
+template <typename F> int by_classes(int ncls, F&& launch) {
+  return ncls <= 2 ? launch(std::integral_constant<int, 2>{})
+       : ncls == 3 ? launch(std::integral_constant<int, 3>{})
+       : ncls == 4 ? launch(std::integral_constant<int, 4>{})
+                   : launch(std::integral_constant<int, MAXC>{});
+}
+
+template <typename T>
+int head_bwd_nody_t(const float* dlog, const void* z, const float* w, float* part, float* dw, float* db, long P, long HW, int Cp,
+                    int C, int ncls, const float* scale, const float* shift, const float* mean, const float* rstd, float* bnpart,
+                    hipStream_t st) {
+  constexpr int HV = HeadVec<T>::HV;
+  const int cvec = Cp / HV;
+  const int cvb = cvec < 64 ? cvec : 64;
+  const int rows = 256 / cvb, gy = cdiv(cvec, cvb);
+  const int nb = segk_head_bwd_blocks(P);
+  const size_t lds = (size_t)rows * cvb * (MAXC * HV + MAXC) * sizeof(float);
+  const int rc = by_classes(ncls, [&](auto NCc) {
+    return segk_launch_lds<head_bwd_nody_kernel<T, decltype(NCc)::value>>("head_bwd_nody", 96 * 1024, dim3(nb, gy), dim3(256), lds,
+                                                                          st, dlog, (const T*)z, w, part, P, HW, Cp, C, ncls, cvb,
+                                                                          rows, scale, shift, mean, rstd, bnpart);
+  });
+  if (rc) return rc;
+  return segk_head_bwd_finalize_launch(part, nb, Cp, C, ncls, dw, db, st);
+}
+
+}
+
+int segk_bn_apply_head_launch(const float* dlog, const float* w, int ncls, const void* z, void* dz, const float* scale,
+                              const float* shift, const float* mean, const float* rstd, const float* coef, long P, long HW, int C,
+                              int C_real, int cvb, int rows, int gx, int gy, int dtype, hipStream_t st) {
+  SEGK_REQUIRE(ncls >= 1 && ncls <= MAXC, "bn_apply_head: 1..%d classes supported, got %d", MAXC, ncls);
+  SEGK_REQUIRE(P > 0 && HW > 0 && P < (1L << 31), "bn_apply_head: pixels are indexed with 32 bits: %ld pixels", P);
+  auto launch = [&](auto Tc) {
+    using T = decltype(Tc);
+    return by_classes(ncls, [&](auto NCc) {
+      hipLaunchKernelGGL((bn_bwd_apply_head_kernel<T, decltype(NCc)::value>), dim3(gx, gy), dim3(256), 0, st, dlog, w, (const T*)z,
+                         (T*)dz, scale, shift, mean, rstd, coef, P, HW, C, C_real, ncls, cvb, rows);
+      SEGK_CHECK_LAUNCH("bn_bwd_apply_head");
+      return 0;
+    });
+  };
+  return dtype == SEGK_DT_BF16 ? launch(bf16_t{}) : launch(float{});
+}
+
+extern "C" int segk_head_bwd_bn_nody(const float* dlogits, const void* z, const float* w, float* part, float* dw, float* db,
+                                     int B, int H, int W, int Cp, int C, int ncls, const float* scale, const float* shift,
+                                     const float* mean, const float* rstd, float* bnpart, int dtype, segk_stream_t s) {
+  SEGK_REQUIRE_DTYPE("head_bwd_bn_nody", dtype);
+  SEGK_REQUIRE(dlogits && z && w && part && dw && db && B > 0 && H > 0 && W > 0, "head_bwd_bn_nody: bad arguments");
+  SEGK_REQUIRE(ncls >= 1 && ncls <= MAXC && Cp > 0 && Cp % 32 == 0 && C > 0 && C <= Cp, "head_bwd_bn_nody: bad channels/classes");
+  SEGK_REQUIRE(scale && shift && mean && rstd && bnpart, "head_bwd_bn_nody: null BatchNorm vectors or partials");
+  const long P = (long)B * H * W, HW = (long)H * W;
+  SEGK_REQUIRE(P < (1L << 31), "head / loss kernels index pixels with 32 bits: %ld pixels", P);
+  hipStream_t st = (hipStream_t)s;
+  return dtype == SEGK_DT_BF16
+             ? head_bwd_nody_t<bf16_t>(dlogits, z, w, part, dw, db, P, HW, Cp, C, ncls, scale, shift, mean, rstd, bnpart, st)
+             : head_bwd_nody_t<float>(dlogits, z, w, part, dw, db, P, HW, Cp, C, ncls, scale, shift, mean, rstd, bnpart, st);
+}
+
+extern "C" int segk_stem3x3_wgrad_bn(const float* x_nchw, const void* dy, const void* z, const float* scale, const float* shift,
+                                     const float* mean, const float* rstd, const float* coef, float* slabs, int B, int H, int W,
+                                     int Cin, int Cout, int dtype, segk_stream_t s) {
+  SEGK_REQUIRE(dtype == SEGK_DT_BF16, "stem3x3_wgrad_bn: bf16 only (dtype %d)", dtype);
+  SEGK_REQUIRE(x_nchw && dy && z && scale && shift && mean && rstd && coef && slabs, "stem3x3_wgrad_bn: null pointer");
+  const int g = segk_stem_wgrad_slabs(B, H, W, Cin, Cout, SEGK_DT_BF16);
+  SEGK_REQUIRE(g > 0, "stem3x3_wgrad_bn: shape not served (bf16, 1..3 input channels, 64 output channels, W a multiple of 16)");
+  const long nblk = (long)B * H * (W / 16);
+  hipLaunchKernelGGL(stem_wgrad_bn_kernel, dim3(g), dim3(STEM_WAVES * 64), 0, (hipStream_t)s, x_nchw, (const bf16_t*)dy,
+                     (const bf16_t*)z, scale, shift, mean, rstd, coef, slabs, B, H, W, Cin, nblk);
+  SEGK_CHECK_LAUNCH("stem_wgrad_bn");
+  return 0;
+}
diff --git a/image_segmentation_amd/csrc/head_loss.hip b/image_segmentation_amd/csrc/head_loss.hip
--- a/image_segmentation_amd/csrc/head_loss.hip
+++ b/image_segmentation_amd/csrc/head_loss.hip
@@ -629,6 +629,12 @@
                : ncls == 4 ? launch(std::integral_constant<int, 4>{})
                            : launch(std::integral_constant<int, MAXC>{});
   if (rc) return rc;
+  hipLaunchKernelGGL(head_bwd_finalize_kernel, dim3(cdiv(ncls * (C + 1), 4)), dim3(256), 0, st, part, nb, Cp, C, ncls, dw, db);
+  SEGK_CHECK_LAUNCH("head_bwd_finalize");
+  return 0;
+}
+
+int segk_head_bwd_finalize_launch(const float* part, int nb, int Cp, int C, int ncls, float* dw, float* db, hipStream_t st) {
   hipLaunchKernelGGL(head_bwd_finalize_kernel, dim3(cdiv(ncls * (C + 1), 4)), dim3(256), 0, st, part, nb, Cp, C, ncls, dw, db);
   SEGK_CHECK_LAUNCH("head_bwd_finalize");
   return 0;
diff --git a/image_segmentation_amd/csrc/segk_internal.h b/image_segmentation_amd/csrc/segk_internal.h
--- a/image_segmentation_amd/csrc/segk_internal.h
+++ b/image_segmentation_amd/csrc/segk_internal.h
@@ -39,6 +39,10 @@
 int segk_stem_wgrad_slabs(int B, int H, int W, int Cin, int Cout, int dtype);
 int segk_stem_wgrad_launch(const float* x, const void* dz, float* slabs, int B, int H, int W, int Cin, int Cout,
                            hipStream_t st);
+int segk_bn_apply_head_launch(const float* dlog, const float* w, int ncls, const void* z, void* dz, const float* scale,
+                              const float* shift, const float* mean, const float* rstd, const float* coef, long P, long HW, int C,
+                              int C_real, int cvb, int rows, int gx, int gy, int dtype, hipStream_t st);
+int segk_head_bwd_finalize_launch(const float* part, int nb, int Cp, int C, int ncls, float* dw, float* db, hipStream_t st);
 int segk_convt_stream_ok(int B, int H, int W, int Cin, int Cout, int dtype);
 int segk_convt_stream_launch(const void* x, const void* wp, const float* bias4, void* out, int B, int H, int W, int Cin,
                              int Cout, hipStream_t st);
diff --git a/image_segmentation_amd/ops.py b/image_segmentation_amd/ops.py
--- a/image_segmentation_amd/ops.py
+++ b/image_segmentation_amd/ops.py
@@ -115,6 +115,8 @@
 INPLACE_SKIP_GRAD = True
 FUSE_BN_REDUCE = True
 HEAD_ON_Z = os.environ.get("SEGK_HEAD_ON_Z", "1") != "0"
+FUSE_STEM_END = os.environ.get("SEGK_FUSE_STEM_END", "1") != "0"
+FUSE_HEAD_END = os.environ.get("SEGK_FUSE_HEAD_END", "1") != "0"
 _OPT_EPOCH = [0]
 
 
@@ -561,6 +563,31 @@
     return dgamma, dbeta
 
 
+def bn_relu_bwd_stats(dy_ptr, z_ptr, scale, shift, mean, rstd, P, C, dtype, dev):
+    Cp = pad32(C)
+    dgamma, dbeta = _f32(C, dev), _f32(C, dev)
+    nb = _lib.query("segk_bn_bwd_blocks", P, Cp, _DT[dtype])
+    part, coef = _f32(nb * Cp * 2, dev), _f32(2 * Cp, dev)
+    with _span("bn_relu_bwd", 0.0, 2.0 * P * C * _es(dtype)):
+        _lib.call("segk_bn_relu_bwd_stats", dy_ptr, z_ptr, scale.data_ptr(), shift.data_ptr(), mean.data_ptr(),
+                  rstd.data_ptr(), P, Cp, C, part.data_ptr(), dgamma.data_ptr(), dbeta.data_ptr(), coef.data_ptr(),
+                  _DT[dtype], _stream())
+    return dgamma, dbeta, coef
+
+
+def bn_relu_bwd_head(head, z_ptr, dz_ptr, scale, shift, mean, rstd, B, H, W, C, dtype, dev, ready):
+    dl, w2 = head
+    ncls, Cp, P = w2.shape[0], pad32(C), B * H * W
+    dgamma, dbeta = _f32(C, dev), _f32(C, dev)
+    part, nb = ready
+    coef = _f32(2 * Cp, dev)
+    with _span("bn_relu_bwd", 2.0 * P * C * ncls, P * (2.0 * C * _es(dtype) + 4.0 * ncls)):
+        _lib.call("segk_bn_relu_bwd_from_part_head", dl.data_ptr(), w2.data_ptr(), ncls, z_ptr, dz_ptr, scale.data_ptr(),
+                  shift.data_ptr(), mean.data_ptr(), rstd.data_ptr(), B, H, W, Cp, C, part.data_ptr(), nb, dgamma.data_ptr(),
+                  dbeta.data_ptr(), coef.data_ptr(), _DT[dtype], _stream())
+    return dgamma, dbeta
+
+
 def channel_sum(ptr, P, C, dtype, dev):
     Cp = pad32(C)
     nb = _lib.query("segk_bn_bwd_blocks", P, Cp, _DT[dtype])
@@ -685,17 +712,26 @@
     return logits
 
 
-def _head_bwd(dlogits, px, Cp, w, B, C, H, W, dtype, dev, bn=None, on_z=False):
+def _head_bwd(dlogits, px, Cp, w, B, C, H, W, dtype, dev, bn=None, on_z=False, store_dy=True):
     ncls = w.shape[0]
     dl = dlogits
     if dl.dtype != torch.float32 or not dl.is_contiguous():
         dl = dl.float().contiguous()
     w2 = _param_f32(w).reshape(ncls, C)
-    dy = torch.empty((B, H, W, Cp), dtype=dtype, device=dev)
     part = _f32(_lib.query("segk_head_part_floats", B * H * W, Cp), dev)
     dw = _grad_buffer(w, w.shape, dev)
     db = _f32(ncls, dev)
     ready = None
+    if not store_dy:
+        sc, sh, mu, rs = bn
+        nb = _lib.query("segk_head_bwd_blocks", B * H * W)
+        bnpart = _f32(nb * Cp * 2, dev)
+        with _span("head_bwd", 4.0 * B * H * W * C * ncls, B * H * W * (C * _es(dtype) + 4 * ncls)):
+            _lib.call("segk_head_bwd_bn_nody", dl.data_ptr(), px, w2.data_ptr(), part.data_ptr(), dw.data_ptr(), db.data_ptr(),
+                      B, H, W, Cp, C, ncls, sc.data_ptr(), sh.data_ptr(), mu.data_ptr(), rs.data_ptr(), bnpart.data_ptr(),
+                      _DT[dtype], _stream())
+        return (dl, w2), dw, db, (bnpart, nb)
+    dy = torch.empty((B, H, W, Cp), dtype=dtype, device=dev)
     with _span("head_bwd", 4.0 * B * H * W * C * ncls, B * H * W * (2 * C * _es(dtype) + 4 * ncls)):
         if on_z:
             sc, sh, mu, rs = bn
@@ -879,11 +915,16 @@
         ready = None
         d_head_w = d_head_b = None
         keep = None
+        head_dy = None
         if ctx.has_head:
             src = z2 if ctx.head_on_z else y
+            nody = FUSE_HEAD_END and FUSE_BN_REDUCE and ctx.head_on_z and not frozen
             dy_buf, d_head_w, d_head_b, ready = _head_bwd(grads[0], src.data_ptr(), Coutp, head_w, B, Cout, H, W, dtype, dev,
-                                                          bn=(sc2, sh2, mu2, rs2), on_z=ctx.head_on_z)
-            pdy, keep = dy_buf.data_ptr(), dy_buf
+                                                          bn=(sc2, sh2, mu2, rs2), on_z=ctx.head_on_z, store_dy=not nody)
+            if nody:
+                head_dy, pdy = dy_buf, 0
+            else:
+                pdy, keep = dy_buf.data_ptr(), dy_buf
         elif cfg.emit_pool:
             dy, dpool = grads
             rc_skip, rc_pool = sys.getrefcount(dy), sys.getrefcount(dpool)
@@ -919,9 +960,13 @@
             keep, pdy, _ = _raw(grads[0], dtype)
 
         dz2 = torch.empty((B, H, W, Coutp), dtype=dtype, device=dev)
-        dg2, dbe2 = bn_relu_bwd(pdy, z2.data_ptr(), dz2.data_ptr(), sc2, sh2, mu2, rs2, P, Cout, dtype, dev, ready=ready,
-                                frozen=frozen)
-        del keep
+        if head_dy is not None:
+            dg2, dbe2 = bn_relu_bwd_head(head_dy, z2.data_ptr(), dz2.data_ptr(), sc2, sh2, mu2, rs2, B, H, W, Cout, dtype, dev,
+                                         ready)
+        else:
+            dg2, dbe2 = bn_relu_bwd(pdy, z2.data_ptr(), dz2.data_ptr(), sc2, sh2, mu2, rs2, P, Cout, dtype, dev, ready=ready,
+                                    frozen=frozen)
+        del keep, head_dy
         w2d = mod.cache.get(("w2d", dtype), w2, lambda: pack_conv(w2, Cout, 0, dtype, 1))
         da1 = torch.empty((B, H, W, Coutp), dtype=dtype, device=dev)
         conv3x3(dz2, dz2.data_ptr(), Coutp, 0, 0, w2d, da1.data_ptr(), Coutp, 0, 0, B, H, W, dtype, alg=(Cout, Cout))
@@ -934,12 +979,18 @@
         rb = ReduceBatch(dev)
         del slabs, dz2
 
-        dg1, dbe1 = bn_relu_bwd(da1.data_ptr(), z1.data_ptr(), da1.data_ptr(), sc1, sh1, mu1, rs1, P, Cout, dtype, dev,
-                                frozen=frozen)
+        has_up = ctx.up_dims is not None
+        stem_fused = (FUSE_STEM_END and ctx.stem_raw and not frozen and dtype == torch.bfloat16
+                      and not (need[1] or need[2] or has_up))
+        coef1 = None
+        if stem_fused:
+            dg1, dbe1, coef1 = bn_relu_bwd_stats(da1.data_ptr(), z1.data_ptr(), sc1, sh1, mu1, rs1, P, Cout, dtype, dev)
+        else:
+            dg1, dbe1 = bn_relu_bwd(da1.data_ptr(), z1.data_ptr(), da1.data_ptr(), sc1, sh1, mu1, rs1, P, Cout, dtype, dev,
+                                    frozen=frozen)
         dz1 = da1
         dxa = dxb = None
         dxb_buf, chan_sum = None, None
-        has_up = ctx.up_dims is not None
         if need[1] or need[2] or has_up:
             w1d = mod.cache.get(("w1d", dtype), w1, lambda: pack_conv(w1, CA, CB, dtype, 1))
             dxa_buf = torch.empty((B, H, W, CAp), dtype=dtype, device=dev)
@@ -957,9 +1008,15 @@
         if ctx.stem_raw:
             S = _lib.query("segk_stem3x3_wgrad_slabs", B, H, W, CA, Cout, _DT[dtype])
             slabs = _f32(S * 64 * 32, dev)
-            with _span("wgrad3x3", 2.0 * P * 9 * CA * Cout, P * (Cout * _es(dtype) + 4 * CA) + 4.0 * 9 * CA * Cout):
-                _lib.call("segk_stem3x3_wgrad", xa_t.data_ptr(), dz1.data_ptr(), slabs.data_ptr(), B, H, W, CA, Cout,
-                          _DT[dtype], _stream())
+            if stem_fused:
+                with _span("wgrad3x3", 2.0 * P * 9 * CA * Cout, P * (2 * Cout * _es(dtype) + 4 * CA) + 4.0 * 9 * CA * Cout):
+                    _lib.call("segk_stem3x3_wgrad_bn", xa_t.data_ptr(), da1.data_ptr(), z1.data_ptr(), sc1.data_ptr(),
+                              sh1.data_ptr(), mu1.data_ptr(), rs1.data_ptr(), coef1.data_ptr(), slabs.data_ptr(), B, H, W, CA,
+                              Cout, _DT[dtype], _stream())
+            else:
+                with _span("wgrad3x3", 2.0 * P * 9 * CA * Cout, P * (Cout * _es(dtype) + 4 * CA) + 4.0 * 9 * CA * Cout):
+                    _lib.call("segk_stem3x3_wgrad", xa_t.data_ptr(), dz1.data_ptr(), slabs.data_ptr(), B, H, W, CA, Cout,
+                              _DT[dtype], _stream())
             dw1 = wgrad_to_param(slabs, S, w1.shape, Cout, 9 * CA, 0, 1, dev, param=w1)
         else:
             slabs, S = wgrad(dz1.data_ptr(), Coutp, pA, CAp, pB, CBp, B, H, W, 0, dtype, dev, alg=(Cout, CA + CB))
diff --git a/include/segk.h b/include/segk.h
--- a/include/segk.h
+++ b/include/segk.h
@@ -12,8 +12,8 @@
 
 typedef void* segk_stream_t;
 
-#define SEGK_ABI_VERSION 318
-#define SEGK_ENTRY_COUNT 94
+#define SEGK_ABI_VERSION 319
+#define SEGK_ENTRY_COUNT 98
 int segk_version(void);
 int segk_entry_count(void);
 const char* segk_build_id(void);
@@ -41,6 +41,9 @@
 int segk_stem3x3_wgrad_slabs(int B, int H, int W, int Cin, int Cout, int dtype);
 int segk_stem3x3_wgrad(const float* x_nchw, const void* dz, float* slabs, int B, int H, int W, int Cin, int Cout, int dtype,
                        segk_stream_t s);
+int segk_stem3x3_wgrad_bn(const float* x_nchw, const void* dy, const void* z, const float* scale, const float* shift,
+                          const float* mean, const float* rstd, const float* coef, float* slabs, int B, int H, int W, int Cin,
+                          int Cout, int dtype, segk_stream_t s);
 int segk_conv_tiles(int B, int H, int W, int Cin, int Cout, int dtype);
 int segk_bn_stats_floats(int tiles, int Cp);
 int segk_conv3x3(const void* srcA, const void* srcB, const void* wpacked, const float* bias, const float* scale,
@@ -79,6 +82,10 @@
                      const float* mean, const float* rstd, long P, int Cp, int C, float* part, float* dgamma,
                      float* dbeta, float* coef, int dtype, segk_stream_t s);
 
+int segk_bn_relu_bwd_stats(const void* dy, const void* z, const float* scale, const float* shift, const float* mean,
+                           const float* rstd, long P, int Cp, int C, float* part, float* dgamma, float* dbeta, float* coef,
+                           int dtype, segk_stream_t s);
+
 int segk_channel_sum(const void* x, long P, int Cp, int C, float* part, float* out, int dtype, segk_stream_t s);
 
 int segk_maxpool2x2_fwd(const void* x, void* y, int B, int H, int W, int Cp, int dtype, segk_stream_t s);
@@ -92,6 +99,11 @@
 int segk_bn_relu_bwd_from_part(const void* dy, const void* z, void* dz, const float* scale, const float* shift,
                                const float* mean, const float* rstd, long P, int Cp, int C, const float* part, int nb,
                                float* dgamma, float* dbeta, float* coef, int dtype, segk_stream_t s);
+
+int segk_bn_relu_bwd_from_part_head(const float* dlogits, const float* head_w, int ncls, const void* z, void* dz,
+                                    const float* scale, const float* shift, const float* mean, const float* rstd, int B, int H,
+                                    int W, int Cp, int C, const float* part, int nb, float* dgamma, float* dbeta, float* coef,
+                                    int dtype, segk_stream_t s);
 
 int segk_bilinear_fwd(const void* x, void* y, int B, int IH, int IW, int OH, int OW, int Cp, int dtype,
                       segk_stream_t s);
@@ -183,6 +195,10 @@
 int segk_head_bwd_bn(const float* dlogits, const void* z, const float* w, void* dy, float* part, float* dw, float* db,
                      int B, int H, int W, int Cp, int C, int ncls, const float* scale, const float* shift,
                      const float* mean, const float* rstd, float* bnpart, int dtype, segk_stream_t s);
+
+int segk_head_bwd_bn_nody(const float* dlogits, const void* z, const float* w, float* part, float* dw, float* db, int B, int H,
+                          int W, int Cp, int C, int ncls, const float* scale, const float* shift, const float* mean,
+                          const float* rstd, float* bnpart, int dtype, segk_stream_t s);
 
 int segk_loss_part_floats(long P);
 int segk_loss_state_floats(void);
```

Result: no change. 2748 images/sec (median of 6 runs) (+0.7%).
